# hwwang55/GraphGAN

Measured on AMD Instinct MI355X. Metric: sampled_edges_per_sec, higher is better.
Workload: dtype f32

## Files before the change

### graphgan_amd/csrc/gg_api.hip

```cpp
#include <stdarg.h>
#include <stdlib.h>
#include <string.h>
#include <sys/stat.h>
#include <unistd.h>

#include <algorithm>
#include <atomic>
#include <thread>

#include "gg_internal.h"

namespace gg {

thread_local std::string g_last_error;

int fail(gg_ctx *ctx, int code, const char *fmt, ...) {
    char buf[1024];
    va_list ap;
    va_start(ap, fmt);
    vsnprintf(buf, sizeof(buf), fmt, ap);
    va_end(ap);
    g_last_error = buf;
    if (ctx) ctx->err = buf;
    return code;
}

static void free_trees(gg_ctx *ctx) {
    discard_begun_walk(ctx);
    void *ps[] = {ctx->t_root, ctx->t_order, ctx->t_cstart, ctx->t_base, ctx->t_q3, ctx->t_q3off, ctx->t_edge};
    for (void *p : ps)
        if (p) (void)hipFree(p);
    ctx->t_root = ctx->t_order = ctx->t_cstart = ctx->t_edge = nullptr;
    ctx->t_edge_valid = false;
    ctx->t_base = ctx->t_q3off = nullptr;
    ctx->t_q3 = nullptr;
    ctx->t_cap_nodes = ctx->t_cap_roots = ctx->t_cap_q3 = 0;
    ctx->n_tree_roots = 0;
    ctx->tree_nodes = ctx->tree_entries = 0;
    ctx->tree_max_depth = ctx->tree_max_list = 0;
    ctx->t_lazy = false;
    ctx->lz_min_level = 0x7fffffff;
    ctx->h_troot.clear();
    ctx->h_tbase.clear();
    ctx->h_q3off.clear();
}

int alloc_trees(gg_ctx *ctx, const int32_t *roots, int32_t n_roots, const int64_t *node_counts, const int64_t *root_children, int64_t extra_nodes) {
    discard_begun_walk(ctx);
    (void)hipDeviceSynchronize();
    ctx->dc_valid = false;
    ctx->t_lazy = false;
    ctx->lz_min_level = 0x7fffffff;
    ctx->t_edge_valid = false;
    const int n = ctx->n_node;
    if (!node_counts && ctx->h_comp_size.empty()) component_sizes(n, ctx->h_rowptr.data(), ctx->h_col.data(), ctx->h_comp_size);
    ctx->h_tbase.assign(n_roots + 1, 0);
    ctx->h_q3off.assign(n_roots + 1, 0);
    for (int r = 0; r < n_roots; ++r) {
        ctx->h_tbase[r + 1] = ctx->h_tbase[r] + (node_counts ? node_counts[r] : ctx->h_comp_size[roots[r]]);
        const int64_t deg = root_children ? root_children[r] : ctx->h_rowptr[roots[r] + 1] - ctx->h_rowptr[roots[r]];
        ctx->h_q3off[r + 1] = ctx->h_q3off[r] + (deg + 31) / 32;
    }
    const int64_t seg_nodes = ctx->h_tbase[n_roots], q3w = ctx->h_q3off[n_roots];
    const int64_t nodes = seg_nodes + extra_nodes;
    const int nr = std::max(n_roots, 1);
    ctx->arena_next = seg_nodes;
    ctx->arena_end = nodes;
    auto regrow = [&](void **p, size_t bytes) -> hipError_t {
        if (*p) (void)hipFree(*p);
        *p = nullptr;
        return hipMalloc(p, bytes);
    };
    if (nodes > ctx->t_cap_nodes || (ctx->t_cap_nodes > (64 << 20) && nodes < ctx->t_cap_nodes / 4) || nr > ctx->t_cap_roots) {
        const int64_t cn = std::max<int64_t>(nodes, 1), cr = std::max<int64_t>(nr, ctx->t_cap_roots);
        GG_HIP(ctx, regrow((void **)&ctx->t_order, sizeof(int32_t) * (size_t)cn));
        GG_HIP(ctx, regrow((void **)&ctx->t_edge, sizeof(int32_t) * (size_t)cn));
        GG_HIP(ctx, regrow((void **)&ctx->t_cstart, sizeof(int32_t) * (size_t)(cn + 2 * cr + 2)));
        GG_HIP(ctx, regrow((void **)&ctx->t_root, sizeof(int32_t) * (size_t)cr));
        GG_HIP(ctx, regrow((void **)&ctx->t_base, sizeof(int64_t) * (size_t)(cr + 1)));
        GG_HIP(ctx, regrow((void **)&ctx->t_q3off, sizeof(int64_t) * (size_t)(cr + 1)));
        ctx->t_cap_nodes = cn;
        ctx->t_cap_roots = cr;
    }
    if (q3w > ctx->t_cap_q3 || !ctx->t_q3) {
        const int64_t cq = std::max<int64_t>(q3w + q3w / 2, 1);
        GG_HIP(ctx, regrow((void **)&ctx->t_q3, sizeof(uint32_t) * (size_t)cq));
        ctx->t_cap_q3 = cq;
    }
    ctx->tree_max_depth = ctx->tree_max_list = 0;
    GG_HIP(ctx, hipMemcpyAsync(ctx->t_root, roots, sizeof(int32_t) * n_roots, hipMemcpyHostToDevice, ctx->stream));
    GG_HIP(ctx, hipMemcpyAsync(ctx->t_base, ctx->h_tbase.data(), sizeof(int64_t) * (n_roots + 1), hipMemcpyHostToDevice, ctx->stream));
    GG_HIP(ctx, hipMemcpyAsync(ctx->t_q3off, ctx->h_q3off.data(), sizeof(int64_t) * (n_roots + 1), hipMemcpyHostToDevice, ctx->stream));
    GG_HIP(ctx, hipMemsetAsync(ctx->t_q3, 0, sizeof(uint32_t) * (size_t)std::max<int64_t>(q3w, 1), ctx->stream));
    GG_HIP(ctx, hipStreamSynchronize(ctx->stream));
    ctx->n_tree_roots = n_roots;
    ctx->tree_nodes = seg_nodes;
    ctx->tree_entries = 2 * seg_nodes - n_roots;
    ctx->h_troot.assign(roots, roots + n_roots);
    return GG_OK;
}

void generator_changed(gg_ctx *ctx) {
    ctx->dc_valid = false;
    ctx->gs_es_valid = false;
    ctx->es_tick += 256;
    ctx->es_valid_from = ctx->es_tick;
}

static int upload_table(gg_ctx *ctx, float *dst, const float *src) {
    const int n = ctx->n_node, d = ctx->n_emb, ld = ctx->ld;
    if (ld == d) {
        GG_HIP(ctx, hipMemcpy(dst, src, sizeof(float) * (size_t)n * d, hipMemcpyHostToDevice));
    } else {
        GG_HIP(ctx, hipMemset(dst, 0, sizeof(float) * (size_t)n * ld));
        GG_HIP(ctx, hipMemcpy2D(dst, sizeof(float) * ld, src, sizeof(float) * d, sizeof(float) * d, n, hipMemcpyHostToDevice));
    }
    return GG_OK;
}

__global__ __launch_bounds__(256) void table_finite_kernel(const float *E, const float *b, int64_t nE, int64_t nb, unsigned long long *bad) {
    bool any = false;
    const int64_t stride = (int64_t)gridDim.x * blockDim.x;
    for (int64_t i = (int64_t)blockIdx.x * blockDim.x + threadIdx.x; i < nE; i += stride) any |= !__builtin_isfinite(E[i]);
    for (int64_t i = (int64_t)blockIdx.x * blockDim.x + threadIdx.x; i < nb; i += stride) any |= !__builtin_isfinite(b[i]);
    if (any) *bad = 1ull;
}

int rescan_table_finite(gg_ctx *ctx, int which) {
    const Model &M = ctx->model[which];
    unsigned long long *w = ctx->table_bad.as<unsigned long long>() + which;
    GG_HIP(ctx, hipMemsetAsync(w, 0, sizeof(unsigned long long), ctx->stream));
    const int64_t nE = (int64_t)ctx->n_node * ctx->ld;
    hipLaunchKernelGGL(table_finite_kernel, dim3((unsigned)std::min<int64_t>(2048, (nE + 255) / 256)), dim3(256), 0, ctx->stream, M.E, M.b, nE, (int64_t)ctx->n_node, w);
    GG_HIP(ctx, hipGetLastError());
    if (which == 0) ctx->gen_dirty = true;
    return GG_OK;
}

}

using namespace gg;

static int launch_and_join(gg_ctx *ctx, int32_t n_slots, int64_t total, int32_t for_d, uint64_t seed, uint32_t stream, int32_t stride, bool join = true) {
    const bool side = ctx->walk_stream != ctx->stream;
    int rc = launch_walk_sample(ctx, n_slots, total, for_d, seed, stream, stride);
    if (rc != GG_OK) {
        if (side) (void)hipStreamSynchronize(ctx->walk_stream);
        return rc;
    }
    if (side) {
        GG_HIP(ctx, hipEventRecord(ctx->ev_walk_done, ctx->walk_stream));
        if (join) GG_HIP(ctx, hipStreamWaitEvent(ctx->stream, ctx->ev_walk_done, 0));
        if (!for_d) {
            rc = enqueue_path_slots(ctx);
            if (rc != GG_OK) return rc;
        }
    }
    return GG_OK;
}

void gg::discard_begun_walk(gg_ctx *ctx) {
    if (!ctx->g_begun) return;
    (void)hipStreamSynchronize(ctx->stream2);
    ctx->g_begun = false;
    ctx->dc_request = 0;
    ctx->walk_stream = ctx->stream;
    ctx->w_nslots = 0;
    ctx->w_total = 0;
    generator_changed(ctx);
}

int gg::walk_launch_async(gg_ctx *ctx, const int32_t *slots, const int32_t *n_walks, int32_t uniform_walks, int32_t n_slots,
                          int32_t for_d, uint64_t seed, uint32_t stream, int32_t stride, bool side_stream, bool defer_join) {
    discard_begun_walk(ctx);
    GG_CHECK(ctx, ctx->n_tree_roots > 0 || n_slots == 0, GG_EINVAL, "walk: no trees loaded (gg_build_trees / gg_set_trees)");
    GG_CHECK(ctx, n_slots >= 0 && (slots || n_slots == 0), GG_EINVAL, "walk: bad slots");
    GG_CHECK(ctx, stride >= 2, GG_ECAPACITY, "walk: stride %d < 2", stride);
    std::vector<int64_t> &ptr = ctx->h_ptr_new;
    ptr.assign(n_slots + 1, 0);
    for (int i = 0; i < n_slots; ++i) {
        GG_CHECK(ctx, slots[i] >= 0 && slots[i] < ctx->n_tree_roots, GG_EINVAL, "walk: slot %d out of range", slots[i]);
        int64_t nw;
        if (n_walks) nw = n_walks[i];
        else if (uniform_walks >= 0) nw = uniform_walks;
        else {
            GG_CHECK(ctx, !ctx->h_rowptr.empty(), GG_EINVAL, "walk: graph CSR needed for D-mode degrees");
            const int r = ctx->h_troot[slots[i]];
            nw = ctx->h_rowptr[r + 1] - ctx->h_rowptr[r];
        }
        GG_CHECK(ctx, nw >= 0, GG_EINVAL, "walk: negative n_walks");
        ptr[i + 1] = ptr[i] + nw;
    }
    const int64_t total = ptr[n_slots];
    GG_HIP(ctx, hipSetDevice(ctx->device));
    const int mode = for_d ? 1 : 0;
    ctx->w_mode = mode;
    GG_HIP(ctx, ctx->w_slots_m[mode].reserve(sizeof(int32_t) * (n_slots + 1)));
    GG_HIP(ctx, ctx->w_ptr_m[mode].reserve(sizeof(int64_t) * (n_slots + 1)));
    GG_HIP(ctx, ctx->w_status.reserve(sizeof(int32_t) * (n_slots + 1)));
    GG_HIP(ctx, ctx->w_abort.reserve(sizeof(int32_t) * (n_slots + 1)));
    GG_HIP(ctx, ctx->w_samples.reserve(sizeof(int32_t) * (total + 1)));
    GG_HIP(ctx, ctx->w_len.reserve(sizeof(int32_t) * (total + 1)));
    GG_HIP(ctx, ctx->w_first.reserve(sizeof(int32_t) * (total + 1)));
    GG_HIP(ctx, ctx->w_paths.reserve(sizeof(int32_t) * ((size_t)total * stride + 1)));
    ctx->walk_stream = side_stream ? ctx->stream2 : ctx->stream;
    if (side_stream && ctx->gen_dirty) {
        GG_HIP(ctx, hipEventRecord(ctx->ev_main_mark, ctx->stream));
        GG_HIP(ctx, hipStreamWaitEvent(ctx->stream2, ctx->ev_main_mark, 0));
        ctx->gen_dirty = false;
    } else if (side_stream && ctx->gen_pass_recorded) {
        GG_HIP(ctx, hipStreamWaitEvent(ctx->stream2, ctx->ev_gen_pass, 0));
    }
    std::vector<int32_t> &hs = ctx->h_slots_m[mode];
    if (hs.size() != (size_t)n_slots || (n_slots && memcmp(hs.data(), slots, sizeof(int32_t) * n_slots) != 0)) {
        hs.assign(slots, slots + n_slots);
        if (n_slots) GG_HIP(ctx, hipMemcpyAsync(ctx->w_slots_m[mode].p, hs.data(), sizeof(int32_t) * n_slots, hipMemcpyHostToDevice, ctx->walk_stream));
    }
    if (ctx->h_ptr_m[mode] != ptr) {
        ctx->h_ptr_m[mode].swap(ptr);
        GG_HIP(ctx, hipMemcpyAsync(ctx->w_ptr_m[mode].p, ctx->h_ptr_m[mode].data(), sizeof(int64_t) * (n_slots + 1), hipMemcpyHostToDevice, ctx->walk_stream));
    }
    ctx->w_total = total;
    ctx->w_stride = stride;
    ctx->w_nslots = n_slots;
    ctx->w_uniform = (!n_walks && uniform_walks >= 0) ? uniform_walks : -1;
    ctx->w_args = {for_d, seed, stream};
    ctx->g_paths_valid = false;
    if (ctx->g_slots_ready) {
        GG_HIP(ctx, hipStreamWaitEvent(ctx->stream, ctx->ev_slots_done, 0));
        ctx->g_slots_ready = false;
        ctx->g_slots_unused++;
    }
    if (n_slots == 0) {
        ctx->walk_stream = ctx->stream;
        return GG_OK;
    }
    return launch_and_join(ctx, n_slots, total, for_d, seed, stream, stride, !defer_join);
}

int gg::walk_finalize(gg_ctx *ctx, bool *retried) {
    if (retried) *retried = false;
    if (ctx->w_nslots == 0) {
        GG_HIP(ctx, hipStreamSynchronize(ctx->stream));
        return GG_OK;
    }
    const int64_t total = ctx->w_total;
    unsigned long long *c = ctx->h_pin;
    constexpr int CW = gg_ctx::CTR_WORDS;
    GG_HIP(ctx, hipMemcpyAsync(c, ctx->dev_ctr, sizeof(unsigned long long) * 2 * CW, hipMemcpyDeviceToHost, ctx->stream));
    GG_HIP(ctx, hipStreamSynchronize(ctx->stream));
    harvest_timings(ctx);
    for (int attempt = 0; c[3] == 2ull || (c[2] != 0ull && ctx->t_lazy); ++attempt) {
        GG_CHECK(ctx, attempt < 16, GG_EHIP, "walk: the launch was voided %d times in a row", attempt);
        if (c[2] != 0ull && ctx->t_lazy) {
            int rebuilt = 0;
            int rc = lazy_fallback_rebuild(ctx, &rebuilt);
            if (rc == GG_ECAPACITY) rc = lazy_rebuild_whole(ctx);
            if (rc != GG_OK) return rc;
            if (ctx->tree_max_depth + 3 > ctx->w_stride) {
                ctx->w_stride = ctx->tree_max_depth + 3;
                GG_HIP(ctx, ctx->w_paths.reserve(sizeof(int32_t) * ((size_t)total * ctx->w_stride + 1)));
            }
        } else {
            ctx->walk_force_sized = true;
        }
        ctx->ctr.walk_reruns += 1;
        generator_changed(ctx);
        int rc = launch_and_join(ctx, ctx->w_nslots, total, ctx->w_args.for_d, ctx->w_args.seed, ctx->w_args.stream, ctx->w_stride);
        ctx->walk_force_sized = false;
        if (rc != GG_OK) return rc;
        GG_HIP(ctx, hipMemcpyAsync(c, ctx->dev_ctr, sizeof(unsigned long long) * 2 * CW, hipMemcpyDeviceToHost, ctx->stream));
        GG_HIP(ctx, hipStreamSynchronize(ctx->stream));
        if (retried) *retried = true;
    }
    const int n_half = ctx->w_split ? 2 : 1;
    if (n_half == 2)
        for (int i = 8; i < CW; ++i) c[i] += c[CW + i];
    {
        int64_t *prof = ctx->alive_prof[ctx->w_args.for_d ? 1 : 0];
        const int run = ctx->w_levels_run;
        for (int i = 0; i < 64; ++i) prof[i] = i < run ? (int64_t)c[8 + i] : -1;
        if (run > 0 && run < 64 && ctx->w_fin_follows) prof[run] = (int64_t)c[7];
        if (ctx->w_net && c[7] > 2048ull && ctx->lv_levels_learned < ctx->tree_max_depth + 2) ctx->lv_levels_learned += 1;
    }
    unsigned long long hops = c[0], reads = c[1], rows = c[5];
    unsigned long long gathers = 0, nodes = 0;
    for (int i = 0; i < 64; ++i) { hops += c[264 + i]; reads += c[328 + i]; rows += c[200 + i]; gathers += c[520 + i]; nodes += c[584 + i]; }
    ctx->ctr.es_gathers += (int64_t)gathers;
    ctx->ctr.es_nodes += (int64_t)nodes;
    ctx->ctr.hops += (int64_t)hops;
    ctx->ctr.nbr_reads += (int64_t)reads;
    ctx->ctr.rows_scored += (int64_t)rows;
    ctx->ctr.walks += total;
    if (total && ctx->walk_timed) {
        float ms = 0.f;
        GG_HIP(ctx, hipEventElapsedTime(&ms, ctx->ev0, ctx->ev1));
        ctx->ctr.last_kernel_ms = ms;
        ctx->ctr.walk_kernel_ms += ms;
        ctx->ctr.walk_launches += 1;
        for (int i = 0; i < ctx->lv_ev_used; ++i) {
            float lms = 0.f;
            for (int k = 0; k < n_half; ++k) {
                float e = 0.f;
                GG_HIP(ctx, hipEventElapsedTime(&e, ctx->lv_ev[4 * i + 2 * k], ctx->lv_ev[4 * i + 2 * k + 1]));
                lms += e;
            }
            ctx->ctr.score_kernel_ms += lms;
            ctx->ctr.score_launches += n_half;
            ctx->ctr.score_chunks += (int64_t)(c[136 + i] >> 32);
            if (getenv("GG_WALK_DEBUG"))
                fprintf(stderr, "[walk] for_d=%d level %d alive %llu score chunks %llu prefix chunks %llu big %llu small %llu rows %llu score %.1f us\n", ctx->w_args.for_d, i,
                        c[8 + i], c[136 + i] >> 32, c[136 + i] & 0xffffffffull, c[72 + i] & 0xffffffffull, c[72 + i] >> 32, c[456 + i], lms * 1e3);
        }
        if (ctx->lv_ev_used) {
            ctx->ctr.score_rows += (int64_t)(rows - c[5]);
            unsigned long long dists = 0;
            for (int i = 0; i < 64; ++i) dists += c[392 + i];
            ctx->ctr.score_dists += (int64_t)dists;
            ctx->ctr.score_gathers += (int64_t)gathers;
            ctx->ctr.score_nodes += (int64_t)nodes;
        }
    }
    if (c[3] || c[6]) generator_changed(ctx);
    if (c[3]) return fail(ctx, GG_ECAPACITY, "walk: a path needed more than stride=%d entries", ctx->w_stride);
    if (c[6]) return fail(ctx, GG_EINVAL, "walk: non-finite generator scores (a softmax had total weight 0, or the generator's tables hold a non-finite value)");
    return GG_OK;
}

int gg::walk_resident(gg_ctx *ctx, const int32_t *slots, const int32_t *n_walks, int32_t uniform_walks, int32_t n_slots,
                      int32_t for_d, uint64_t seed, uint32_t stream, int32_t stride) {
    int rc = walk_launch_async(ctx, slots, n_walks, uniform_walks, n_slots, for_d, seed, stream, stride);
    if (rc != GG_OK) return rc;
    return walk_finalize(ctx, nullptr);
}

extern "C" {

int gg_abi_version(void) { return GG_ABI_VERSION; }

const char *gg_last_error(const gg_ctx *ctx) { return ctx ? ctx->err.c_str() : g_last_error.c_str(); }

int gg_create(int32_t n_node, int32_t n_emb, const float *emb_gen, const float *emb_dis, const gg_config *cfg,
              gg_ctx **out) {
    if (!out) return fail(nullptr, GG_EINVAL, "gg_create: out is NULL");
    *out = nullptr;
    if (n_node <= 0 || n_emb <= 0 || n_emb > 512 || !emb_gen || !emb_dis || !cfg)
        return fail(nullptr, GG_EINVAL, "gg_create: bad argument (n_node=%d n_emb=%d)", n_node, n_emb);
    int ndev = 0;
    hipError_t e = hipGetDeviceCount(&ndev);
    if (e != hipSuccess || ndev <= 0)
        return fail(nullptr, GG_EHIP, "gg_create: no HIP device (%s); this engine has no CPU fallback",
                    e == hipSuccess ? "count = 0" : hipGetErrorString(e));
    if (cfg->device < 0 || cfg->device >= ndev) return fail(nullptr, GG_EINVAL, "gg_create: device %d of %d", cfg->device, ndev);
    hipDeviceProp_t prop;
    GG_HIP(nullptr, hipGetDeviceProperties(&prop, cfg->device));
    if (strncmp(prop.gcnArchName, "gfx950", 6) != 0)
        return fail(nullptr, GG_EHIP, "gg_create: device %d is %s; kernels are built for gfx950 only", cfg->device, prop.gcnArchName);
    GG_HIP(nullptr, hipSetDevice(cfg->device));

    gg_ctx *ctx = new gg_ctx();
    ctx->n_node = n_node;
    ctx->n_emb = n_emb;
    ctx->ld = (n_emb + 3) / 4 * 4;
    ctx->cfg = *cfg;
    ctx->device = cfg->device;
    ctx->n_cus = prop.multiProcessorCount > 0 ? prop.multiProcessorCount : 256;
    if (const char *lv = getenv("GG_WALK_LEVELS")) ctx->walk_levels = atoi(lv);
    if (const char *pe = getenv("GG_PROFILE_EVERY")) ctx->profile_every = std::max(0, atoi(pe));
    if (const char *fw = getenv("GG_COMM_FAKE_WORLD")) ctx->fake_world = atoi(fw);
    if (const char *ow = getenv("GG_COMM_OWNER")) ctx->owner_exchange = atoi(ow);
    if (const char *bf = getenv("GG_COMM_BF16")) ctx->comm_bf16 = atoi(bf) != 0;
    if (const char *om = getenv("GG_COMM_OWNER_MIN")) ctx->owner_min_bound = atoll(om);
    if (const char *dt = getenv("GG_DETERMINISTIC")) ctx->deterministic = atoi(dt) != 0;
    if (const char *nc = getenv("GG_NO_DIST_CACHE")) ctx->dc_enabled = atoi(nc) == 0;
    if (const char *ft = getenv("GG_FIN_THRESHOLD")) ctx->fin_threshold = std::max(0, atoi(ft));
    if (const char *st = getenv("GG_STAGE_T")) ctx->sg_threshold = std::max(0, atoi(st));
    if (const char *ws = getenv("GG_WALK_SPLIT")) ctx->split_enabled = atoi(ws) != 0;
    if (const char *em = getenv("GG_ES_MODE")) ctx->es_mode = std::min(2, std::max(0, atoi(em)));
    if (const char *er = getenv("GG_ES_RATIO")) ctx->es_ratio_num = std::max(1, atoi(er));
    if (const char *eh = getenv("GG_ES_HUB")) ctx->es_hub = std::max(0, atoi(eh));
    if (const char *wm = getenv("GG_WALK_SPLIT_MIN")) ctx->split_min_walks = std::max(512, atoi(wm));
    for (auto &m : ctx->alive_prof) for (auto &v : m) v = -1;
    if (const char *dr = getenv("GG_COMM_DENSE_RATIO")) ctx->dense_exchange_ratio = (float)atof(dr);
#define GG_TRY(call)                        \
    do {                                    \
        int rc__ = (call);                  \
        if (rc__ != GG_OK) {                \
            g_last_error = ctx->err;        \
            gg_destroy(ctx);                \
            return rc__;                    \
        }                                   \
    } while (0)
    auto body = [&]() -> int {
        GG_HIP(ctx, hipStreamCreateWithFlags(&ctx->stream, hipStreamNonBlocking));
        {
            int lo = 0, hi = 0;
            const char *wp = getenv("GG_WALK_PRIORITY");
            if (wp && atoi(wp) != 0 && hipDeviceGetStreamPriorityRange(&lo, &hi) == hipSuccess && hi != lo)
                GG_HIP(ctx, hipStreamCreateWithPriority(&ctx->stream2, hipStreamNonBlocking, atoi(wp) > 0 ? hi : lo));
            else
                GG_HIP(ctx, hipStreamCreateWithFlags(&ctx->stream2, hipStreamNonBlocking));
        }
        GG_HIP(ctx, hipStreamCreateWithFlags(&ctx->stream3, hipStreamNonBlocking));
        GG_HIP(ctx, hipEventCreateWithFlags(&ctx->ev_fork, hipEventDisableTiming));
        GG_HIP(ctx, hipEventCreateWithFlags(&ctx->ev_join, hipEventDisableTiming));
        GG_HIP(ctx, hipEventCreateWithFlags(&ctx->ev_score[0], hipEventDisableTiming));
        GG_HIP(ctx, hipEventCreateWithFlags(&ctx->ev_score[1], hipEventDisableTiming));
        ctx->walk_stream = ctx->stream;
        GG_HIP(ctx, hipEventCreate(&ctx->ev0));
        GG_HIP(ctx, hipEventCreate(&ctx->ev1));
        GG_HIP(ctx, hipEventCreateWithFlags(&ctx->ev_walk_done, hipEventDisableTiming));
        GG_HIP(ctx, hipEventCreateWithFlags(&ctx->ev_gen_pass, hipEventDisableTiming));
        GG_HIP(ctx, hipEventCreateWithFlags(&ctx->ev_main_mark, hipEventDisableTiming));
        GG_HIP(ctx, hipHostMalloc((void **)&ctx->h_pin, sizeof(unsigned long long) * gg_ctx::PIN_WORDS, hipHostMallocDefault));
        memset(ctx->h_pin, 0, sizeof(unsigned long long) * gg_ctx::PIN_WORDS);
        const size_t tb = sizeof(float) * (size_t)n_node * ctx->ld, vb = sizeof(float) * (size_t)n_node;
        for (int m = 0; m < 2; ++m) {
            Model &M = ctx->model[m];
            GG_HIP(ctx, hipMalloc((void **)&M.E, tb));
            GG_HIP(ctx, hipMalloc((void **)&M.b, vb));
            GG_HIP(ctx, hipMemset(M.b, 0, vb));
            if (cfg->optimizer != GG_OPT_SGD) {
                GG_HIP(ctx, hipMalloc((void **)&M.mE, tb));
                GG_HIP(ctx, hipMalloc((void **)&M.vE, tb));
                GG_HIP(ctx, hipMalloc((void **)&M.mb, vb));
                GG_HIP(ctx, hipMalloc((void **)&M.vb, vb));
                GG_HIP(ctx, hipMemset(M.mE, 0, tb));
                GG_HIP(ctx, hipMemset(M.vE, 0, tb));
                GG_HIP(ctx, hipMemset(M.mb, 0, vb));
                GG_HIP(ctx, hipMemset(M.vb, 0, vb));
            }
            M.b1p = cfg->adam_beta1;
            M.b2p = cfg->adam_beta2;
            M.lr = m == 0 ? cfg->lr_gen : cfg->lr_dis;
            M.lambda = m == 0 ? cfg->lambda_gen : cfg->lambda_dis;
            int rc = upload_table(ctx, M.E, m == 0 ? emb_gen : emb_dis);
            if (rc != GG_OK) return rc;
        }
        GG_HIP(ctx, hipMalloc((void **)&ctx->gradE, tb));
        GG_HIP(ctx, hipMalloc((void **)&ctx->gradb, vb));
        GG_HIP(ctx, hipMemset(ctx->gradE, 0, tb));
        ctx->grad_elems_padded = (size_t)n_node * ctx->ld;
        GG_HIP(ctx, hipMemset(ctx->gradb, 0, vb));
        GG_HIP(ctx, hipMalloc((void **)&ctx->touched, sizeof(int32_t) * n_node));
        GG_HIP(ctx, hipMalloc((void **)&ctx->touched_list, sizeof(int32_t) * n_node));
        GG_HIP(ctx, hipMalloc((void **)&ctx->touched_cnt, sizeof(int32_t) * 4));
        GG_HIP(ctx, hipMemset(ctx->touched, 0, sizeof(int32_t) * n_node));
        GG_HIP(ctx, hipMemset(ctx->touched_cnt, 0, sizeof(int32_t) * 4));
        GG_HIP(ctx, hipMalloc((void **)&ctx->dev_ctr, sizeof(unsigned long long) * gg_ctx::PIN_WORDS));
        GG_HIP(ctx, hipMemset(ctx->dev_ctr, 0, sizeof(unsigned long long) * gg_ctx::PIN_WORDS));
        GG_HIP(ctx, ctx->table_bad.reserve(sizeof(unsigned long long) * 2));
        for (int m = 0; m < 2; ++m) {
            int rc = rescan_table_finite(ctx, m);
            if (rc != GG_OK) return rc;
        }
        GG_HIP(ctx, hipDeviceSynchronize());
        return GG_OK;
    };
    GG_TRY(body());
#undef GG_TRY
    *out = ctx;
    return GG_OK;
}

int gg_destroy(gg_ctx *ctx) {
    if (!ctx) return GG_OK;
    (void)hipSetDevice(ctx->device);
    if (ctx->stream) (void)hipStreamSynchronize(ctx->stream);
    if (ctx->stream2) (void)hipStreamSynchronize(ctx->stream2);
    comm_destroy(ctx);
    for (int m = 0; m < 2; ++m) {
        Model &M = ctx->model[m];
        float *ps[] = {M.E, M.b, M.mE, M.vE, M.mb, M.vb};
        for (float *p : ps)
            if (p) (void)hipFree(p);
    }
    void *ps[] = {ctx->gradE, ctx->gradb, ctx->touched, ctx->touched_list, ctx->touched_cnt, ctx->g_rowptr, ctx->g_col, ctx->dev_ctr,
                  ctx->es, ctx->es_stamp, ctx->g_rev};
    for (void *p : ps)
        if (p) (void)hipFree(p);
    free_trees(ctx);
    DevBuf *bufs[] = {&ctx->w_slots_m[0], &ctx->w_slots_m[1], &ctx->w_ptr_m[0], &ctx->w_ptr_m[1], &ctx->w_samples, &ctx->w_paths, &ctx->w_len, &ctx->w_status,
                      &ctx->w_first, &ctx->w_abort, &ctx->w_scratch, &ctx->d_center, &ctx->d_neighbor, &ctx->d_label, &ctx->d_cnt,
                      &ctx->d_ptr, &ctx->g_node1, &ctx->g_node2, &ctx->g_reward, &ctx->g_cnt, &ctx->g_ptr, &ctx->scan_tmp,
                      &ctx->step_u, &ctx->step_v, &ctx->step_x, &ctx->sg_cnt, &ctx->sg_off, &ctx->sg_slot, &ctx->sg_list, &ctx->sg_rows, &ctx->sg_bias, &ctx->sg_tot, &ctx->sg_key, &ctx->touched_ptr, &ctx->x_cnt, &ctx->x_send_ids, &ctx->x_send_rows,
                      &ctx->x_recv_ids, &ctx->x_recv_rows, &ctx->x_nglob, &ctx->x_own, &ctx->st_item, &ctx->st_item2, &ctx->st_cur, &ctx->st_prev, &ctx->st_len,
                      &ctx->st_alive, &ctx->st_rank, &ctx->bfs_key, &ctx->bfs_bm, &ctx->bfs_misc, &ctx->bfs_sparse, &ctx->bfs_rowptr32, &ctx->lv_pfx, &ctx->dc_keys, &ctx->dc_vals, &ctx->dc_words, &ctx->lv_beg, &ctx->lv_k, &ctx->lv_chunks, &ctx->lv_coff, &ctx->lv_scores, &ctx->lv_chunk_owner, &ctx->lv_prefix, &ctx->lv_big, &ctx->lv_fe, &ctx->fin_list, &ctx->table_bad, &ctx->sgp_cnt, &ctx->sgp_off, &ctx->sgp_slot, &ctx->sgp_list, &ctx->sgp_tot, &ctx->sgp_key, &ctx->sgp_scan, &ctx->sgp_hub, &ctx->sg_hub, &ctx->hub_acc,
                      &ctx->q3_store, &ctx->q3s_off, &ctx->ep_center, &ctx->ep_neighbor, &ctx->ep_label, &ctx->ep_node1, &ctx->ep_node2, &ctx->ep_reward, &ctx->topk_adj,
                      &ctx->gs_es, &ctx->gs_cpre, &ctx->pt_starts, &ctx->pt_paths, &ctx->pt_len, &ctx->pt_cnt, &ctx->pt_ptr, &ctx->pt_noise, &ctx->pt_sample};
    for (DevBuf *b : bufs) b->release();
    for (hipEvent_t e : ctx->lv_ev)
        if (e) (void)hipEventDestroy(e);
    for (auto &tr : ctx->tm_ev)
        for (hipEvent_t e : tr)
            if (e) (void)hipEventDestroy(e);
    for (hipEvent_t e : ctx->pt_ev)
        if (e) (void)hipEventDestroy(e);
    if (ctx->h_pin) (void)hipHostFree(ctx->h_pin);
    for (hipEvent_t e : {ctx->ev_walk_done, ctx->ev_slots_done, ctx->ev_gen_pass, ctx->ev_main_mark, ctx->ev_fork, ctx->ev_join, ctx->ev_score[0], ctx->ev_score[1]})
        if (e) (void)hipEventDestroy(e);
    if (ctx->stream3) {
        (void)hipStreamSynchronize(ctx->stream3);
        (void)hipStreamDestroy(ctx->stream3);
    }
    if (ctx->stream2) {
        (void)hipStreamSynchronize(ctx->stream2);
        (void)hipStreamDestroy(ctx->stream2);
    }
    if (ctx->ev0) (void)hipEventDestroy(ctx->ev0);
    if (ctx->ev1) (void)hipEventDestroy(ctx->ev1);
    if (ctx->stream) (void)hipStreamDestroy(ctx->stream);
    delete ctx;
    return GG_OK;
}

int gg_set_graph_csr(gg_ctx *ctx, const int64_t *rowptr, const int32_t *col) {
    if (!ctx) return fail(nullptr, GG_EINVAL, "ctx is NULL");
    GG_CHECK(ctx, rowptr && rowptr[0] == 0, GG_EINVAL, "gg_set_graph_csr: rowptr[0] must be 0");
    discard_begun_walk(ctx);
    const int n = ctx->n_node;
    const int64_t nnz = rowptr[n];
    GG_CHECK(ctx, nnz >= 0 && (col || nnz == 0), GG_EINVAL, "gg_set_graph_csr: col is NULL");
    for (int v = 0; v < n; ++v) GG_CHECK(ctx, rowptr[v + 1] >= rowptr[v], GG_EINVAL, "gg_set_graph_csr: rowptr not monotone at %d", v);
    for (int64_t e = 0; e < nnz; ++e) GG_CHECK(ctx, col[e] >= 0 && col[e] < n, GG_EINVAL, "gg_set_graph_csr: col[%lld]=%d out of range", (long long)e, col[e]);
    GG_HIP(ctx, hipSetDevice(ctx->device));
    (void)hipDeviceSynchronize();
    for (void *p : {(void *)ctx->g_rowptr, (void *)ctx->g_col, (void *)ctx->es, (void *)ctx->es_stamp, (void *)ctx->g_rev})
        if (p) (void)hipFree(p);
    ctx->g_rowptr = nullptr;
    ctx->g_col = nullptr;
    ctx->es = nullptr;
    ctx->es_stamp = nullptr;
    ctx->g_rev = nullptr;
    ctx->t_edge_valid = false;
    ctx->q3_store_ready = false;
    ctx->bfs_rowptr32_valid = false;
    ctx->topk_adj.release();
    ctx->topk_adj_valid = false;
    ctx->gs_es_valid = ctx->gs_cpre_valid = false;
    ctx->pt_noise_set = false;
    GG_HIP(ctx, hipMalloc((void **)&ctx->g_rowptr, sizeof(int64_t) * (n + 1)));
    GG_HIP(ctx, hipMalloc((void **)&ctx->g_col, sizeof(int32_t) * (std::max<int64_t>(nnz, 1) + 4)));
    GG_HIP(ctx, hipMemcpy(ctx->g_rowptr, rowptr, sizeof(int64_t) * (n + 1), hipMemcpyHostToDevice));
    if (nnz) GG_HIP(ctx, hipMemcpy(ctx->g_col, col, sizeof(int32_t) * nnz, hipMemcpyHostToDevice));
    ctx->g_nnz = nnz;
    ctx->g_max_deg = 0;
    for (int v = 0; v < n; ++v) ctx->g_max_deg = (int32_t)std::min<int64_t>(std::max<int64_t>(ctx->g_max_deg, rowptr[v + 1] - rowptr[v]), 0x7fffffff);
    ctx->g_multi = true;
    ctx->h_rowptr.assign(rowptr, rowptr + n + 1);
    ctx->h_col.assign(col, col + nnz);
    ctx->h_comp_size.clear();
    uint64_t h = 1469598103934665603ull;
    for (int v = 0; v <= n; ++v) h = (h ^ (uint64_t)rowptr[v]) * 1099511628211ull;
    for (int64_t e = 0; e + 1 < nnz; e += 2) h = (h ^ ((uint64_t)(uint32_t)col[e] | ((uint64_t)(uint32_t)col[e + 1] << 32))) * 1099511628211ull;
    if (nnz & 1) h = (h ^ (uint64_t)(uint32_t)col[nnz - 1]) * 1099511628211ull;
    ctx->g_hash = h;
    if (nnz > 0 && nnz < (1ll << 31)) {
        hipError_t e = hipMalloc((void **)&ctx->es, sizeof(float) * (size_t)nnz);
        if (e == hipSuccess) e = hipMalloc((void **)&ctx->es_stamp, sizeof(long long) * (size_t)n);
        if (e == hipSuccess) e = hipMalloc((void **)&ctx->g_rev, sizeof(int32_t) * (size_t)nnz);
        if (e == hipSuccess) e = hipMemset(ctx->es_stamp, 0, sizeof(long long) * (size_t)n);
        generator_changed(ctx);
        int rc = e == hipSuccess ? compute_reverse_edges(ctx) : GG_ENOMEM;
        if (rc != GG_OK) {
            (void)hipGetLastError();
            for (void *p : {(void *)ctx->es, (void *)ctx->es_stamp, (void *)ctx->g_rev})
                if (p) (void)hipFree(p);
            ctx->es = nullptr;
            ctx->es_stamp = nullptr;
            ctx->g_rev = nullptr;
            if (getenv("GG_WALK_DEBUG")) fprintf(stderr, "[graph] edge-score cache not allocated (%s): walks score privately\n", e == hipSuccess ? ctx->err.c_str() : hipGetErrorString(e));
        }
    }
    return GG_OK;
}

int gg_build_trees(gg_ctx *ctx, const int32_t *roots, int32_t n_roots, int32_t n_threads) {
    if (!ctx) return fail(nullptr, GG_EINVAL, "ctx is NULL");
    GG_CHECK(ctx, !ctx->h_rowptr.empty(), GG_EINVAL, "gg_build_trees: call gg_set_graph_csr first");
    GG_CHECK(ctx, n_roots >= 0 && (roots || n_roots == 0), GG_EINVAL, "gg_build_trees: bad roots");
    const int n = ctx->n_node;
    for (int r = 0; r < n_roots; ++r) GG_CHECK(ctx, roots[r] >= 0 && roots[r] < n, GG_EINVAL, "gg_build_trees: root %d out of range", roots[r]);
    GG_HIP(ctx, hipSetDevice(ctx->device));
    if (n_threads <= 0) n_threads = (int)std::max(1u, std::thread::hardware_concurrency());
    int rc = alloc_trees(ctx, roots, n_roots, nullptr, nullptr);
    if (rc != GG_OK) return rc;
    const int64_t budget = 256ll << 20;
    const std::vector<int64_t> &base = ctx->h_tbase;
    int32_t md = 0, ml = 0;
    std::vector<int32_t> order_h, cstart_h;
    for (int r0 = 0; r0 < n_roots;) {
        int r1 = r0 + 1;
        while (r1 < n_roots && base[r1 + 1] - base[r0] <= budget) ++r1;
        order_h.resize((size_t)(base[r1] - base[r0]));
        cstart_h.resize((size_t)(base[r1] - base[r0]) + (r1 - r0));
        const int nt = std::max(1, std::min(n_threads, r1 - r0));
        std::atomic<int> next(r0);
        std::vector<int32_t> tmd(nt, 0), tml(nt, 0);
        auto work = [&](int tid) {
            std::vector<uint32_t> stamp(n, 0u);
            uint32_t epoch = 0;
            for (;;) {
                const int r = next.fetch_add(1);
                if (r >= r1) break;
                int32_t depth = 0, mc = 0;
                (void)host_bfs_order(ctx->h_rowptr.data(), ctx->h_col.data(), roots[r], order_h.data() + (base[r] - base[r0]),
                                     cstart_h.data() + (base[r] - base[r0]) + (r - r0), stamp, epoch, &depth, &mc);
                tmd[tid] = std::max(tmd[tid], depth);
                tml[tid] = std::max(tml[tid], mc + 1);
            }
        };
        std::vector<std::thread> th;
        for (int t = 1; t < nt; ++t) th.emplace_back(work, t);
        work(0);
        for (auto &t : th) t.join();
        for (int t = 0; t < nt; ++t) { md = std::max(md, tmd[t]); ml = std::max(ml, tml[t]); }
        if (!order_h.empty()) GG_HIP(ctx, hipMemcpy(ctx->t_order + base[r0], order_h.data(), sizeof(int32_t) * order_h.size(), hipMemcpyHostToDevice));
        GG_HIP(ctx, hipMemcpy(ctx->t_cstart + base[r0] + r0, cstart_h.data(), sizeof(int32_t) * cstart_h.size(), hipMemcpyHostToDevice));
        r0 = r1;
    }
    ctx->tree_max_depth = md;
    ctx->tree_max_list = ml;
    return derive_tree_edges(ctx);
}

int gg_set_trees(gg_ctx *ctx, const int32_t *roots, int32_t n_roots, const int32_t *off, const int32_t *nbr,
                 const int64_t *nbr_base, int32_t max_depth) {
    if (!ctx) return fail(nullptr, GG_EINVAL, "ctx is NULL");
    GG_CHECK(ctx, n_roots >= 0 && roots && off && nbr_base && (nbr || nbr_base[n_roots] == 0), GG_EINVAL, "gg_set_trees: bad argument");
    const int n = ctx->n_node;
    GG_HIP(ctx, hipSetDevice(ctx->device));
    std::vector<int64_t> counts(n_roots), kids(n_roots);
    for (int r = 0; r < n_roots; ++r) {
        GG_CHECK(ctx, roots[r] >= 0 && roots[r] < n, GG_EINVAL, "gg_set_trees: root out of range");
        const int32_t *o = off + (size_t)r * (n + 1);
        GG_CHECK(ctx, o[0] == 0 && o[n] == nbr_base[r + 1] - nbr_base[r] && o[n] >= 1 && (o[n] & 1), GG_EINVAL,
                 "gg_set_trees: offsets of slot %d inconsistent (a tree over C nodes has 2C - 1 entries)", r);
        for (int v = 0; v < n; ++v) GG_CHECK(ctx, o[v + 1] >= o[v], GG_EINVAL, "gg_set_trees: offsets not monotone");
        counts[r] = (o[n] + 1) / 2;
        kids[r] = o[roots[r] + 1] - o[roots[r]];
    }
    int rc = alloc_trees(ctx, roots, n_roots, counts.data(), kids.data());
    if (rc != GG_OK) return rc;
    const std::vector<int64_t> &base = ctx->h_tbase;
    std::vector<int32_t> order_h((size_t)base[n_roots]), cstart_h((size_t)base[n_roots] + n_roots);
    std::vector<uint32_t> q3_h((size_t)std::max<int64_t>(ctx->h_q3off[n_roots], 1), 0u);
    int32_t md = 0, ml = 0;
    for (int r = 0; r < n_roots; ++r) {
        const int64_t C_expect = base[r + 1] - base[r];
        GG_CHECK(ctx, nbr_base[r + 1] - nbr_base[r] == 2 * C_expect - 1, GG_EINVAL,
                 "gg_set_trees: slot %d has %lld entries, the component of root %d needs %lld", r, (long long)(nbr_base[r + 1] - nbr_base[r]),
                 roots[r], (long long)(2 * C_expect - 1));
// ... 231 lines not shown
        GG_HIP(ctx, hipMemcpy(len.data(), ctx->w_len.p, sizeof(int32_t) * total, hipMemcpyDeviceToHost));
        for (int64_t w = 0; w < total; ++w)
            GG_CHECK(ctx, len[w] <= stride, GG_ECAPACITY, "walk: a path needed %d entries, stride is %d (gg_tree_info reports the depth of the trees as rebuilt)", len[w], stride);
        if (paths) GG_HIP(ctx, hipMemcpy2D(paths, sizeof(int32_t) * (size_t)stride, ctx->w_paths.p, sizeof(int32_t) * (size_t)ctx->w_stride, sizeof(int32_t) * (size_t)stride, (size_t)total, hipMemcpyDeviceToHost));
    }
    if (root_status && n_slots) GG_HIP(ctx, hipMemcpy(root_status, ctx->w_status.p, sizeof(int32_t) * n_slots, hipMemcpyDeviceToHost));
    return GG_OK;
}

int gg_debug_words(gg_ctx *ctx, int32_t first, int32_t n, uint64_t *out) {
    if (!ctx || !out || first < 0 || n < 0 || first + n > gg_ctx::PIN_WORDS) return fail(ctx, GG_EINVAL, "gg_debug_words: bad argument");
    GG_HIP(ctx, hipSetDevice(ctx->device));
    hipStream_t s;
    GG_HIP(ctx, hipStreamCreateWithFlags(&s, hipStreamNonBlocking));
    hipError_t e = hipMemcpyAsync(out, ctx->dev_ctr + first, sizeof(uint64_t) * (size_t)n, hipMemcpyDeviceToHost, s);
    if (e == hipSuccess) e = hipStreamSynchronize(s);
    (void)hipStreamDestroy(s);
    GG_HIP(ctx, e);
    return GG_OK;
}

int gg_set_tree_mode(gg_ctx *ctx, int32_t mode, int64_t node_cap) {
    if (!ctx) return fail(nullptr, GG_EINVAL, "ctx is NULL");
    GG_CHECK(ctx, mode >= -1 && mode <= 1 && node_cap >= 0, GG_EINVAL, "gg_set_tree_mode: mode must be -1 (auto), 0 (whole trees) or 1 (lazy), node_cap >= 0");
    ctx->tree_mode = mode;
    ctx->lz_cap = node_cap;
    return GG_OK;
}

int gg_lazy_stats(gg_ctx *ctx, int64_t *out8) {
    if (!ctx || !out8) return fail(ctx, GG_EINVAL, "gg_lazy_stats: NULL argument");
    GG_HIP(ctx, hipSetDevice(ctx->device));
    for (int i = 0; i < 24; ++i) out8[i] = 0;
    out8[0] = ctx->t_lazy ? 1 : 0;
    out8[1] = ctx->t_lazy ? ctx->lz_min_level : 0;
    out8[2] = ctx->lz_fallback_roots;
    out8[3] = ctx->lz_fallback_rounds;
    if (ctx->t_lazy && ctx->n_tree_roots > 0) {
        GG_HIP(ctx, hipStreamSynchronize(ctx->stream));
        const int R = ctx->n_tree_roots;
        std::vector<int4> info((size_t)R);
        std::vector<int32_t> cur((size_t)R);
        GG_HIP(ctx, hipMemcpy(info.data(), ctx->lz_info.p, sizeof(int4) * (size_t)R, hipMemcpyDeviceToHost));
        GG_HIP(ctx, hipMemcpy(cur.data(), ctx->lz_cursor.p, sizeof(int32_t) * (size_t)R, hipMemcpyDeviceToHost));
        for (int r = 0; r < R; ++r) {
            out8[4] += info[r].y;
            out8[5] += std::max(0, cur[r] - info[r].y);
            out8[6] += info[r].x < info[r].y ? 1 : 0;
            out8[7] = std::max<int64_t>(out8[7], info[r].z);
            if (info[r].x < info[r].y && info[r].z >= 0 && info[r].z < 8) out8[16 + info[r].z] += 1;
        }
        unsigned long long c[8];
        GG_HIP(ctx, hipMemcpy(c, ctx->dev_ctr + 1500, sizeof(c), hipMemcpyDeviceToHost));
        for (int i = 0; i < 8; ++i) out8[8 + i] = (int64_t)c[i];
    }
    return GG_OK;
}

int gg_get_lazy_trees(gg_ctx *ctx, int64_t *n_entries, int32_t *info4, int64_t *base, int32_t *order, int32_t *cstart, int32_t *edge, uint64_t *pair) {
    if (!ctx) return fail(nullptr, GG_EINVAL, "ctx is NULL");
    GG_CHECK(ctx, ctx->t_lazy, GG_EINVAL, "gg_get_lazy_trees: the resident trees are not lazy");
    GG_HIP(ctx, hipSetDevice(ctx->device));
    GG_HIP(ctx, hipDeviceSynchronize());
    const size_t R = (size_t)ctx->n_tree_roots, nodes = (size_t)ctx->arena_end;
    if (n_entries) *n_entries = (int64_t)nodes;
    if (info4) GG_HIP(ctx, hipMemcpy(info4, ctx->lz_info.p, sizeof(int4) * R, hipMemcpyDeviceToHost));
    if (base) GG_HIP(ctx, hipMemcpy(base, ctx->t_base, sizeof(int64_t) * R, hipMemcpyDeviceToHost));
    if (order) GG_HIP(ctx, hipMemcpy(order, ctx->t_order, sizeof(int32_t) * nodes, hipMemcpyDeviceToHost));
    if (cstart) GG_HIP(ctx, hipMemcpy(cstart, ctx->t_cstart, sizeof(int32_t) * (nodes + R), hipMemcpyDeviceToHost));
    if (edge) GG_HIP(ctx, hipMemcpy(edge, ctx->t_edge, sizeof(int32_t) * nodes, hipMemcpyDeviceToHost));
    if (pair) GG_HIP(ctx, hipMemcpy(pair, ctx->lz_pair.p, sizeof(uint64_t) * std::min(nodes, ctx->lz_pair.bytes / sizeof(uint64_t)), hipMemcpyDeviceToHost));
    return GG_OK;
}

int gg_walk_info(const gg_ctx *ctx, int64_t *total_walks, int32_t *stride, int32_t *n_slots) {
    if (!ctx) return fail(nullptr, GG_EINVAL, "ctx is NULL");
    if (total_walks) *total_walks = ctx->w_total;
    if (stride) *stride = ctx->w_stride;
    if (n_slots) *n_slots = ctx->w_nslots;
    return GG_OK;
}

int gg_get_walks(gg_ctx *ctx, int32_t *samples, int32_t *paths, int32_t *path_len, int32_t *root_status) {
    if (!ctx) return fail(nullptr, GG_EINVAL, "ctx is NULL");
    GG_HIP(ctx, hipSetDevice(ctx->device));
    const bool begun = ctx->g_begun;
    discard_begun_walk(ctx);
    GG_CHECK(ctx, !begun, GG_EINVAL, "gg_get_walks: the walks of the last completed launch were overwritten by gg_prepare_g_begin (fetch them before it, or after the gg_prepare_g that adopts it)");
    GG_HIP(ctx, hipStreamSynchronize(ctx->stream));
    const int64_t total = ctx->w_total;
    if (samples && total) GG_HIP(ctx, hipMemcpy(samples, ctx->w_samples.p, sizeof(int32_t) * total, hipMemcpyDeviceToHost));
    if (path_len && total) GG_HIP(ctx, hipMemcpy(path_len, ctx->w_len.p, sizeof(int32_t) * total, hipMemcpyDeviceToHost));
    if (paths && total) GG_HIP(ctx, hipMemcpy(paths, ctx->w_paths.p, sizeof(int32_t) * (size_t)total * ctx->w_stride, hipMemcpyDeviceToHost));
    if (root_status && ctx->w_nslots) GG_HIP(ctx, hipMemcpy(root_status, ctx->w_status.p, sizeof(int32_t) * ctx->w_nslots, hipMemcpyDeviceToHost));
    return GG_OK;
}

static int table_io(gg_ctx *ctx, int32_t which, float *out, const float *in, bool bias) {
    if (!ctx) return fail(nullptr, GG_EINVAL, "ctx is NULL");
    GG_CHECK(ctx, which == 0 || which == 1, GG_EINVAL, "which must be 0 (gen) or 1 (dis)");
    GG_CHECK(ctx, out || in, GG_EINVAL, "buffer is NULL");
    GG_HIP(ctx, hipSetDevice(ctx->device));
    GG_HIP(ctx, hipStreamSynchronize(ctx->stream));
    Model &M = ctx->model[which];
    const int n = ctx->n_node, d = ctx->n_emb, ld = ctx->ld;
    if (in && which == 0) { discard_begun_walk(ctx); generator_changed(ctx); }
    if (bias) {
        if (out) GG_HIP(ctx, hipMemcpy(out, M.b, sizeof(float) * n, hipMemcpyDeviceToHost));
        else GG_HIP(ctx, hipMemcpy(M.b, in, sizeof(float) * n, hipMemcpyHostToDevice));
    } else if (out) {
        GG_HIP(ctx, hipMemcpy2D(out, sizeof(float) * d, M.E, sizeof(float) * ld, sizeof(float) * d, n, hipMemcpyDeviceToHost));
    } else {
        int rc = upload_table(ctx, M.E, in);
        if (rc != GG_OK) return rc;
    }
    if (in) return rescan_table_finite(ctx, which);
    return GG_OK;
}

int gg_get_embeddings(gg_ctx *ctx, int32_t which, float *out) { return table_io(ctx, which, out, nullptr, false); }
int gg_get_bias(gg_ctx *ctx, int32_t which, float *out) { return table_io(ctx, which, out, nullptr, true); }
int gg_set_embeddings(gg_ctx *ctx, int32_t which, const float *emb) { return table_io(ctx, which, nullptr, emb, false); }
int gg_set_bias(gg_ctx *ctx, int32_t which, const float *bias) { return table_io(ctx, which, nullptr, bias, true); }

int gg_get_counters(gg_ctx *ctx, gg_counters *out) {
    if (!ctx || !out) return fail(ctx, GG_EINVAL, "gg_get_counters: NULL argument");
    if (!ctx->tm_pending.empty()) {
        GG_HIP(ctx, hipSetDevice(ctx->device));
        GG_HIP(ctx, hipStreamSynchronize(ctx->stream));
        harvest_timings(ctx);
    }
    *out = ctx->ctr;
    return GG_OK;
}

int gg_set_profiling_solo(gg_ctx *ctx, int32_t solo) {
    if (!ctx) return fail(nullptr, GG_EINVAL, "ctx is NULL");
    ctx->profile_solo = solo != 0;
    return GG_OK;
}

int gg_set_profiling(gg_ctx *ctx, int32_t every_n) {
    if (!ctx) return fail(nullptr, GG_EINVAL, "ctx is NULL");
    GG_CHECK(ctx, every_n >= 0, GG_EINVAL, "gg_set_profiling: every_n < 0");
    ctx->profile_every = every_n;
    ctx->walk_call_index = 0;
    return GG_OK;
}

int gg_synchronize(gg_ctx *ctx) {
    if (!ctx) return fail(nullptr, GG_EINVAL, "ctx is NULL");
    GG_HIP(ctx, hipSetDevice(ctx->device));
    GG_HIP(ctx, hipStreamSynchronize(ctx->stream));
    if (ctx->g_begun) GG_HIP(ctx, hipStreamSynchronize(ctx->stream2));
    harvest_timings(ctx);
    return check_exchange_flag(ctx);
}

}

int gg::check_exchange_flag(gg_ctx *ctx) {
    if (!ctx->comm && ctx->fake_world <= 1) return GG_OK;
    int32_t flag = 0;
    GG_HIP(ctx, hipMemcpy(&flag, ctx->touched_cnt + 2, sizeof(int32_t), hipMemcpyDeviceToHost));
    if (flag) return fail(ctx, GG_ECOMM, "replica exchange: a rank touched more rows than the pack capacity of its step");
    return GG_OK;
}

void gg::harvest_timings(gg_ctx *ctx) {
    size_t keep = 0;
    for (size_t i = 0; i < ctx->tm_pending.size(); ++i) {
        const gg_ctx::PendingTiming t = ctx->tm_pending[i];
        hipEvent_t *ev = ctx->tm_ev[t.slot];
        if (hipEventQuery(ev[2]) != hipSuccess) {
            ctx->tm_pending[keep++] = t;
            continue;
        }
        float a = 0.f, b = 0.f;
        (void)hipEventElapsedTime(&a, ev[0], ev[1]);
        (void)hipEventElapsedTime(&b, ev[1], ev[2]);
        const int64_t rows = t.has_rows ? (int64_t)ctx->h_pin[gg_ctx::H_ROWS + t.slot] : (int64_t)ctx->n_node;
        if (t.kind == 0) {
            ctx->ctr.reward_kernel_ms += a + b;
            ctx->ctr.reward_pairs_timed += t.units;
        } else if (t.kind == 1) {
            ctx->ctr.d_grad_ms += a; ctx->ctr.d_opt_ms += b;
            ctx->ctr.d_pairs_timed += t.units; ctx->ctr.d_rows_timed += rows; ctx->ctr.d_passes_timed += 1;
        } else {
            ctx->ctr.g_grad_ms += a; ctx->ctr.g_opt_ms += b;
            ctx->ctr.g_pairs_timed += t.units; ctx->ctr.g_rows_timed += rows; ctx->ctr.g_passes_timed += 1;
        }
    }
    ctx->tm_pending.resize(keep);
}

int gg::timing_slot(gg_ctx *ctx) {
    for (int s = 0; s < 8; ++s) {
        bool busy = false;
        for (const auto &t : ctx->tm_pending) busy |= t.slot == s;
        if (busy) continue;
        for (int k = 0; k < 3; ++k)
            if (!ctx->tm_ev[s][k] && hipEventCreate(&ctx->tm_ev[s][k]) != hipSuccess) return -1;
        return s;
    }
    return -1;
}

namespace {
struct StateHeader {
    char magic[4];
    int32_t version, n_node, n_emb, ld, optimizer;
};

int io_dev(gg_ctx *ctx, FILE *f, float *dev, size_t count, bool save, std::vector<float> &tmp) {
    tmp.resize(count);
    if (save) {
        GG_HIP(ctx, hipMemcpy(tmp.data(), dev, sizeof(float) * count, hipMemcpyDeviceToHost));
        if (fwrite(tmp.data(), sizeof(float), count, f) != count) return gg::fail(ctx, GG_EIO, "state: short write");
    } else {
        if (fread(tmp.data(), sizeof(float), count, f) != count) return gg::fail(ctx, GG_EIO, "state: short read");
        GG_HIP(ctx, hipMemcpy(dev, tmp.data(), sizeof(float) * count, hipMemcpyHostToDevice));
    }
    return GG_OK;
}

int state_io(gg_ctx *ctx, const char *path, bool save) {
    if (!ctx) return gg::fail(nullptr, GG_EINVAL, "ctx is NULL");
    GG_CHECK(ctx, path, GG_EINVAL, "state: path is NULL");
    GG_HIP(ctx, hipSetDevice(ctx->device));
    GG_HIP(ctx, hipStreamSynchronize(ctx->stream));
    if (!save) discard_begun_walk(ctx);
    const bool slots = ctx->cfg.optimizer != GG_OPT_SGD;
    const size_t ne = (size_t)ctx->n_node * ctx->ld, nb = (size_t)ctx->n_node;
    struct Scalars { int64_t t; float b1p, b2p; };
    const size_t per_model = sizeof(Scalars) + sizeof(float) * (ne + nb) * (slots ? 3 : 1);
    const size_t expect = sizeof(StateHeader) + 2 * per_model;
    const std::string tmp_path = std::string(path) + ".tmp";
    FILE *f = fopen(save ? tmp_path.c_str() : path, save ? "wb" : "rb");
    if (!f) return gg::fail(ctx, GG_EIO, "state: cannot open %s", save ? tmp_path.c_str() : path);
    StateHeader h{{'G', 'G', 'S', 'T'}, 1, ctx->n_node, ctx->n_emb, ctx->ld, ctx->cfg.optimizer};
    int rc = GG_OK;
    if (save) {
        if (fwrite(&h, sizeof(h), 1, f) != 1) rc = gg::fail(ctx, GG_EIO, "state: short write");
    } else {
        StateHeader g;
        if (fread(&g, sizeof(g), 1, f) != 1 || memcmp(g.magic, "GGST", 4) != 0 || g.version != 1)
            rc = gg::fail(ctx, GG_EIO, "state: %s is not a GGST v1 file", path);
        else if (g.n_node != h.n_node || g.n_emb != h.n_emb || g.ld != h.ld || (g.optimizer == GG_OPT_SGD) != (h.optimizer == GG_OPT_SGD))
            rc = gg::fail(ctx, GG_EINVAL, "state: shape/optimizer mismatch (file %dx%d opt %d)", g.n_node, g.n_emb, g.optimizer);
        if (rc == GG_OK) {
            struct stat st;
            if (fstat(fileno(f), &st) != 0 || (size_t)st.st_size != expect)
                rc = gg::fail(ctx, GG_EIO, "state: %s is truncated or has trailing bytes (%lld bytes, expected %zu); nothing was loaded", path,
                              (long long)st.st_size, expect);
        }
    }
    std::vector<float> tmp;
    Scalars loaded[2] = {};
    for (int m = 0; m < 2 && rc == GG_OK; ++m) {
        gg::Model &M = ctx->model[m];
        Scalars sc{M.t, M.b1p, M.b2p};
        if (save) {
            if (fwrite(&sc, sizeof(sc), 1, f) != 1) rc = gg::fail(ctx, GG_EIO, "state: short write");
        } else {
            if (fread(&sc, sizeof(sc), 1, f) != 1) rc = gg::fail(ctx, GG_EIO, "state: short read");
            else loaded[m] = sc;
        }
        if (rc == GG_OK) rc = io_dev(ctx, f, M.E, ne, save, tmp);
        if (rc == GG_OK) rc = io_dev(ctx, f, M.b, nb, save, tmp);
        if (slots) {
            if (rc == GG_OK) rc = io_dev(ctx, f, M.mE, ne, save, tmp);
            if (rc == GG_OK) rc = io_dev(ctx, f, M.vE, ne, save, tmp);
            if (rc == GG_OK) rc = io_dev(ctx, f, M.mb, nb, save, tmp);
            if (rc == GG_OK) rc = io_dev(ctx, f, M.vb, nb, save, tmp);
        }
    }
    if (save) {
        if (rc == GG_OK && (fflush(f) != 0 || fsync(fileno(f)) != 0)) rc = gg::fail(ctx, GG_EIO, "state: cannot flush %s", tmp_path.c_str());
        fclose(f);
        if (rc == GG_OK && rename(tmp_path.c_str(), path) != 0) rc = gg::fail(ctx, GG_EIO, "state: cannot rename %s to %s", tmp_path.c_str(), path);
        if (rc != GG_OK) (void)remove(tmp_path.c_str());
        return rc;
    }
    fclose(f);
    generator_changed(ctx);
    for (int m = 0; m < 2; ++m) {
        const int rs = gg::rescan_table_finite(ctx, m);
        if (rc == GG_OK) rc = rs;
    }
    if (rc == GG_OK)
        for (int m = 0; m < 2; ++m) { ctx->model[m].t = loaded[m].t; ctx->model[m].b1p = loaded[m].b1p; ctx->model[m].b2p = loaded[m].b2p; }
    return rc;
}
}

extern "C" int gg_save_state(gg_ctx *ctx, const char *path) { return state_io(ctx, path, true); }
extern "C" int gg_load_state(gg_ctx *ctx, const char *path) { return state_io(ctx, path, false); }
```

### graphgan_amd/csrc/gg_internal.h

```cpp
#pragma once
#include <hip/hip_runtime.h>
#include <stdint.h>
#include <stdio.h>
#include <string>
#include <vector>

#include "../../include/graphgan_hip.h"

namespace gg {

struct DevBuf {
    void *p = nullptr;
    size_t bytes = 0;
    hipError_t reserve(size_t need) {
        if (need <= bytes) return hipSuccess;
        if (p) {
            (void)hipDeviceSynchronize();
            (void)hipFree(p);
        }
        p = nullptr;
        bytes = 0;
        size_t want = need + need / 4 + 256;
        hipError_t e = hipMalloc(&p, want);
        if (e == hipSuccess) bytes = want;
        return e;
    }
    void release() {
        if (p) (void)hipFree(p);
        p = nullptr;
        bytes = 0;
    }
    template <class T> T *as() const { return (T *)p; }
};

struct Model {
    float *E = nullptr, *b = nullptr;
    float *mE = nullptr, *vE = nullptr;
    float *mb = nullptr, *vb = nullptr;
    float b1p = 0.9f, b2p = 0.999f;
    int64_t t = 0;
    float lr = 1e-3f, lambda = 1e-5f;
};

}

struct gg_ctx {
    int32_t n_node = 0, n_emb = 0, ld = 0;
    gg_config cfg{};
    int device = 0;
    hipStream_t stream = nullptr;
    hipEvent_t ev0 = nullptr, ev1 = nullptr;
    hipStream_t stream2 = nullptr;
    hipStream_t walk_stream = nullptr;
    hipEvent_t ev_walk_done = nullptr;
    hipEvent_t ev_gen_pass = nullptr;
    hipEvent_t ev_main_mark = nullptr;
    bool gen_pass_recorded = false;
    bool gen_dirty = false;
    hipEvent_t lv_ev[256] = {};
    hipStream_t stream3 = nullptr;
    hipEvent_t ev_fork = nullptr, ev_join = nullptr, ev_score[2] = {nullptr, nullptr};
    bool split_enabled = false;
    int64_t split_min_walks = 32768;
    bool w_split = false;
    gg::DevBuf fin_list;
    gg::DevBuf table_bad;
    int lv_ev_used = 0;
    gg::Model model[2];

    float *gradE = nullptr, *gradb = nullptr;
    int32_t *touched = nullptr;
    int32_t *touched_list = nullptr;
    int32_t *touched_cnt = nullptr;

    int64_t *g_rowptr = nullptr;
    int32_t *g_col = nullptr;
    int64_t g_nnz = 0;
    uint64_t g_hash = 0;
    std::vector<int64_t> h_rowptr;
    std::vector<int32_t> h_col;
    float *es = nullptr;
    long long *es_stamp = nullptr;
    int32_t *g_rev = nullptr;
    long long es_tick = 256;
    long long es_valid_from = 256;
    int32_t es_mode = 1;
    int32_t es_ratio_num = 2;
    int32_t es_hub = 0;

    int32_t n_tree_roots = 0, tree_max_depth = 0, tree_max_list = 0;
    int64_t tree_nodes = 0;
    int64_t t_cap_nodes = 0, t_cap_roots = 0, t_cap_q3 = 0;
    int64_t tree_entries = 0;
    int32_t *t_root = nullptr;
    int32_t *t_order = nullptr;
    int32_t *t_cstart = nullptr;
    int32_t *t_edge = nullptr;
    bool t_edge_valid = false;
    int64_t *t_base = nullptr;
    uint32_t *t_q3 = nullptr;
    int64_t *t_q3off = nullptr;
    std::vector<int32_t> h_troot;
    std::vector<int64_t> h_tbase, h_q3off;
    std::vector<int32_t> h_comp_size;

    int32_t tree_mode = -1;
    int64_t lz_cap = 0;
    bool t_lazy = false;
    bool lz_force_whole = false;
    int32_t lz_min_level = 0x7fffffff;
    uint32_t lz_stamp = 0;
    gg::DevBuf lz_info, lz_pair, lz_rank, lz_bm, lz_cursor, lz_flag, lz_limit, lz_expect, lz_list, lz_scratch, lz_fb_scratch;
    int64_t arena_next = 0, arena_end = 0;
    int64_t lz_fallback_roots = 0, lz_fallback_rounds = 0, lz_resolved = 0;
    bool g_multi = true;
    int32_t g_max_deg = 0;

    gg::DevBuf w_slots_m[2], w_ptr_m[2];
    std::vector<int32_t> h_slots_m[2];
    std::vector<int64_t> h_ptr_m[2], h_ptr_new;
    int w_mode = 0;
    int64_t alive_prof[2][64];
    int64_t fin_threshold = 0;
    int w_levels_run = 0;
    bool w_fin_follows = false;
    bool w_net = false;
    const gg::DevBuf &w_slots_buf() const { return w_slots_m[w_mode]; }
    const gg::DevBuf &w_ptr_buf() const { return w_ptr_m[w_mode]; }
    gg::DevBuf w_samples, w_paths, w_len, w_status, w_first, w_abort, w_scratch;
    gg::DevBuf st_cur, st_prev, st_len, st_alive, st_rank, st_item, st_item2, lv_beg, lv_k, lv_chunks, lv_coff, lv_scores, lv_chunk_owner, lv_prefix, lv_big, lv_fe;
    gg::DevBuf lv_pfx, dc_keys, dc_vals, dc_words;
    size_t dc_size = 0;
    int32_t dc_request = 0;
    bool dc_valid = false;
    bool dc_enabled = true;
    int64_t lv_cap_total = 0;
    int32_t lv_levels_learned = 0;
    int64_t lv_cap_chunks = 0;
    bool walk_force_sized = false;
    bool walk_used_speculation = false;
    int32_t walk_levels = 64;
    int64_t w_total = 0;
    int32_t w_stride = 0, w_nslots = 0;
    int32_t w_uniform = -1;
    struct { int32_t for_d; uint64_t seed; uint32_t stream; } w_args{};

    static constexpr int CTR_WORDS = 720;
    static constexpr int PIN_WORDS = 2048;
    static constexpr int H_TOTAL = 1960;
    static constexpr int H_ROWS = 1940;
    unsigned long long *h_pin = nullptr;
    int32_t profile_every = 1;
    int64_t walk_call_index = 0;
    bool walk_timed = false;
    bool profile_solo = true;
    struct PendingTiming { int kind; int64_t units; int slot; bool has_rows; };
    hipEvent_t tm_ev[8][3] = {};
    std::vector<PendingTiming> tm_pending;
    int64_t pass_call_index[2] = {0, 0};
    int tm_cur = -1;

    gg::DevBuf d_center, d_neighbor, d_label, d_cnt, d_ptr;
    int64_t d_rows = 0;
    gg::DevBuf g_node1, g_node2, g_reward, g_cnt, g_ptr;
    int64_t g_pairs = 0;
    bool g_paths_valid = false;
    bool g_begun = false;
    struct { int32_t n_slots = 0, n_sample = 0; uint64_t seed = 0; uint32_t stream = 0; } g_begun_args;
    gg::DevBuf touched_ptr;
    gg::DevBuf bfs_key, bfs_bm, bfs_misc, bfs_sparse, bfs_rowptr32;
    bool bfs_rowptr32_valid = false;
    gg::DevBuf q3_store, q3s_off;
    int64_t q3_words = 0;
    bool q3_store_ready = false;
    gg::DevBuf ep_center, ep_neighbor, ep_label, ep_node1, ep_node2, ep_reward;
    int64_t ep_rows = 0, ep_pairs = 0;
    std::vector<int32_t> ep_slots;
    bool in_epoch_add = false;
    int n_cus = 256;
    gg::DevBuf scan_tmp, step_u, step_v, step_x;
    gg::DevBuf sg_cnt, sg_off, sg_slot, sg_list, sg_rows, sg_bias, sg_tot, sg_key;
    bool g_pairs_filled = false;
    bool sg_cnt_dirty = false;
    gg::DevBuf sgp_cnt, sgp_off, sgp_slot, sgp_list, sgp_tot, sgp_key, sgp_scan, sgp_hub;
    gg::DevBuf sg_hub, hub_acc;
    int64_t hub_cap = 0;
    hipEvent_t ev_slots_done = nullptr;
    bool g_slots_ready = false;
    bool sgp_cnt_clean = false;
    int g_slots_unused = 0;
    int64_t g_slots_walks = 0;
    int32_t g_slots_stride = 0;
    int32_t *sg_cnt_active = nullptr;
    bool sg_active = false;
    int sg_threshold = 64;

    unsigned long long *dev_ctr = nullptr;
    gg_counters ctr{};

    void *comm = nullptr;
    bool comm_rsag = true;
    size_t grad_elems_padded = 0;
    int64_t d_rows_max = 0, g_pairs_max = 0;
    int64_t step_bound = 0;
    int64_t comm_steps_sparse = 0, comm_steps_dense = 0, comm_bytes_sent = 0;
    int32_t rank = 0, world = 1;
    bool deterministic = true;
    float dense_exchange_ratio = 1.5f;
    int32_t fake_world = 0;
    gg::DevBuf x_cnt, x_send_ids, x_send_rows, x_recv_ids, x_recv_rows;
    gg::DevBuf x_nglob;
    gg::DevBuf x_own;
    int32_t owner_exchange = 1;
    bool comm_bf16 = false;
    int64_t owner_min_bound = 4096;
    int64_t comm_steps_owner = 0;

    gg::DevBuf topk_adj;
    bool topk_adj_valid = false;

    gg::DevBuf gs_es, gs_cpre;
    int64_t gs_chunks = 0;
    bool gs_es_valid = false, gs_cpre_valid = false;

    gg::DevBuf pt_starts, pt_paths, pt_len, pt_cnt, pt_ptr, pt_noise, pt_sample;
    bool pt_noise_set = false;
    uint64_t pt_noise_total = 0;
    int32_t pt_sample_n = 0, pt_sample_stride = 1;
    hipEvent_t pt_ev[4] = {};
    bool ep_d_open = false;

    std::string err;
};

namespace gg {

extern thread_local std::string g_last_error;

int fail(gg_ctx *ctx, int code, const char *fmt, ...);

#define GG_HIP(ctx, call)                                                                      \
    do {                                                                                       \
        hipError_t e__ = (call);                                                               \
        if (e__ != hipSuccess)                                                                 \
            return gg::fail(ctx, GG_EHIP, "%s:%d %s -> %s", __FILE__, __LINE__, #call,         \
                            hipGetErrorString(e__));                                           \
    } while (0)

#define GG_CHECK(ctx, cond, code, ...)                        \
    do {                                                      \
        if (!(cond)) return gg::fail(ctx, code, __VA_ARGS__); \
    } while (0)

int device_exclusive_scan(gg_ctx *ctx, const int32_t *cnt, int64_t *ptr, int64_t n);
int ensure_g_pairs(gg_ctx *ctx);
int device_compact_flags(gg_ctx *ctx, const int32_t *flag, int64_t n, int32_t *list, int64_t *total_out);
int device_segment_rows(gg_ctx *ctx, const int32_t *cnt, int64_t n, int T, int32_t *off, int4 *list, int64_t *totals, hipStream_t stream = nullptr,
                        DevBuf *scratch = nullptr);

int alloc_trees(gg_ctx *ctx, const int32_t *roots, int32_t n_roots, const int64_t *node_counts, const int64_t *root_children, int64_t extra_nodes = 0);
bool lazy_build_wanted(const gg_ctx *ctx);
int lazy_rebuild_whole(gg_ctx *ctx);
int lazy_fallback_rebuild(gg_ctx *ctx, int *n_out);
void component_sizes(int n, const int64_t *rowptr, const int32_t *col, std::vector<int32_t> &comp_size);
int32_t host_bfs_order(const int64_t *rowptr, const int32_t *col, int32_t root, int32_t *order, int32_t *cstart,
                       std::vector<uint32_t> &stamp, uint32_t &epoch, int32_t *depth_out, int32_t *max_children_out);
void order_to_lists(int32_t n, int32_t C, const int32_t *order, const int32_t *cstart, const uint32_t *q3, int32_t *off, int32_t *nbr);
int32_t lists_to_order(int32_t n, int32_t root, const int32_t *off, const int32_t *nbr, int32_t *order, int32_t *cstart,
                       uint32_t *q3, int32_t q3_words, int32_t *depth_out, int32_t *max_children_out);

int walk_launch_async(gg_ctx *ctx, const int32_t *slots, const int32_t *n_walks, int32_t uniform_walks, int32_t n_slots,
                      int32_t for_d, uint64_t seed, uint32_t stream, int32_t stride, bool side_stream = false, bool defer_join = false);
void discard_begun_walk(gg_ctx *ctx);
int walk_finalize(gg_ctx *ctx, bool *retried);
int timing_slot(gg_ctx *ctx);
int check_exchange_flag(gg_ctx *ctx);
void harvest_timings(gg_ctx *ctx);
int derive_tree_edges(gg_ctx *ctx);
int compute_reverse_edges(gg_ctx *ctx);
int rescan_table_finite(gg_ctx *ctx, int which);
int enqueue_path_slots(gg_ctx *ctx);
void generator_changed(gg_ctx *ctx);
int walk_resident(gg_ctx *ctx, const int32_t *slots, const int32_t *n_walks, int32_t uniform_walks, int32_t n_slots,
                  int32_t for_d, uint64_t seed, uint32_t stream, int32_t stride);
int launch_walk_sample(gg_ctx *ctx, int32_t n_slots, int64_t total_walks, int for_d, uint64_t seed, uint32_t stream,
                       int32_t stride);
int run_step(gg_ctx *ctx, int which, const int32_t *d_u, const int32_t *d_v, const float *d_x, int32_t n);
int comm_allreduce_grads(gg_ctx *ctx);
int comm_allreduce_flags(gg_ctx *ctx);
int comm_allreduce_i64(gg_ctx *ctx, int64_t *buf, size_t count);
int comm_allreduce_max_i64(gg_ctx *ctx, int64_t *buf, size_t count);
size_t comm_dense_bytes(const gg_ctx *ctx);
int exchange_count_max(gg_ctx *ctx, int64_t local, int64_t *max_out);
int comm_allgather(gg_ctx *ctx, const void *send, void *recv, size_t count, int elem_bytes);
bool comm_has_p2p(const gg_ctx *ctx);
int comm_exchange_v(gg_ctx *ctx, const float *send, const int64_t *send_off, const int64_t *send_cnt, float *recv, const int64_t *recv_off,
                    const int64_t *recv_cnt);
void comm_destroy(gg_ctx *ctx);

static inline int cdiv(int64_t a, int64_t b) { return (int)((a + b - 1) / b); }

}
```

### graphgan_amd/csrc/prepare.hip

```cpp
#include <algorithm>

#include <cstring>

#include "gg_internal.h"

namespace gg {

constexpr int SCAN_THREADS = 256;
constexpr int SCAN_ITEMS = 8;
constexpr int SCAN_TILE = SCAN_THREADS * SCAN_ITEMS;

__device__ __forceinline__ int64_t block_excl_scan(int64_t v, int64_t *total, int64_t *sh ) {
    const int lane = threadIdx.x & 63, wv = threadIdx.x >> 6;
    int64_t inc = v;
#pragma unroll
    for (int off = 1; off < 64; off <<= 1) {
        const int64_t o = __shfl_up(inc, off, 64);
        if (lane >= off) inc += o;
    }
    if (lane == 63) sh[wv] = inc;
    __syncthreads();
    int64_t base = 0, tot = 0;
#pragma unroll
    for (int i = 0; i < SCAN_THREADS / 64; ++i) {
        if (i < wv) base += sh[i];
        tot += sh[i];
    }
    __syncthreads();
    *total = tot;
    return base + inc - v;
}

__global__ __launch_bounds__(SCAN_THREADS) void scan_tile_sums(const int32_t *cnt, int64_t n, int64_t *tile_sum) {
    __shared__ int64_t sh[SCAN_THREADS / 64];
    const int64_t base = (int64_t)blockIdx.x * SCAN_TILE + (int64_t)threadIdx.x * SCAN_ITEMS;
    int64_t s = 0;
#pragma unroll
    for (int i = 0; i < SCAN_ITEMS; ++i)
        if (base + i < n) s += cnt[base + i];
    int64_t tot;
    (void)block_excl_scan(s, &tot, sh);
    if (threadIdx.x == 0) tile_sum[blockIdx.x] = tot;
}

__global__ __launch_bounds__(SCAN_THREADS) void scan_tile_offsets(int64_t *tile_sum, int64_t n_tiles, int64_t *total_out) {
    __shared__ int64_t sh[SCAN_THREADS / 64];
    int64_t carry = 0;
    for (int64_t t0 = 0; t0 < n_tiles; t0 += SCAN_THREADS) {
        const int64_t i = t0 + threadIdx.x;
        const int64_t v = i < n_tiles ? tile_sum[i] : 0;
        int64_t tot;
        const int64_t ex = block_excl_scan(v, &tot, sh);
        if (i < n_tiles) tile_sum[i] = carry + ex;
        carry += tot;
    }
    if (threadIdx.x == 0) *total_out = carry;
}

__global__ __launch_bounds__(SCAN_THREADS) void scan_tile_offsets2(int64_t *tile_sum_a, int64_t *tile_sum_b, int64_t n_tiles, int64_t *total_a, int64_t *total_b) {
    __shared__ int64_t sh[SCAN_THREADS / 64];
    int64_t *const tile_sum = blockIdx.x == 0 ? tile_sum_a : tile_sum_b;
    int64_t carry = 0;
    for (int64_t t0 = 0; t0 < n_tiles; t0 += SCAN_THREADS) {
        const int64_t i = t0 + threadIdx.x;
        const int64_t v = i < n_tiles ? tile_sum[i] : 0;
        int64_t tot;
        const int64_t ex = block_excl_scan(v, &tot, sh);
        if (i < n_tiles) tile_sum[i] = carry + ex;
        carry += tot;
    }
    if (threadIdx.x == 0) *(blockIdx.x == 0 ? total_a : total_b) = carry;
}

__global__ __launch_bounds__(SCAN_THREADS) void scan_apply(const int32_t *cnt, int64_t n, const int64_t *tile_off, int64_t *ptr) {
    __shared__ int64_t sh[SCAN_THREADS / 64];
    const int64_t base = (int64_t)blockIdx.x * SCAN_TILE + (int64_t)threadIdx.x * SCAN_ITEMS;
    int64_t v[SCAN_ITEMS], s = 0;
#pragma unroll
    for (int i = 0; i < SCAN_ITEMS; ++i) {
        v[i] = base + i < n ? cnt[base + i] : 0;
        s += v[i];
    }
    int64_t tot;
    int64_t run = tile_off[blockIdx.x] + block_excl_scan(s, &tot, sh);
#pragma unroll
    for (int i = 0; i < SCAN_ITEMS; ++i) {
        if (base + i < n) ptr[base + i] = run;
        run += v[i];
    }
}

int device_exclusive_scan(gg_ctx *ctx, const int32_t *cnt, int64_t *ptr, int64_t n) {
    const int64_t tiles = (n + SCAN_TILE - 1) / SCAN_TILE;
    GG_HIP(ctx, ctx->scan_tmp.reserve(sizeof(int64_t) * (tiles + 2)));
    int64_t *ts = ctx->scan_tmp.as<int64_t>();
    if (n == 0) {
        GG_HIP(ctx, hipMemsetAsync(ptr, 0, sizeof(int64_t), ctx->stream));
        return GG_OK;
    }
    hipLaunchKernelGGL(scan_tile_sums, dim3((unsigned)tiles), dim3(SCAN_THREADS), 0, ctx->stream, cnt, n, ts);
    hipLaunchKernelGGL(scan_tile_offsets, dim3(1), dim3(SCAN_THREADS), 0, ctx->stream, ts, tiles, ptr + n);
    hipLaunchKernelGGL(scan_apply, dim3((unsigned)tiles), dim3(SCAN_THREADS), 0, ctx->stream, cnt, n, ts, ptr);
    GG_HIP(ctx, hipGetLastError());
    return GG_OK;
}

__global__ __launch_bounds__(SCAN_THREADS) void flag_tile_sums(const int32_t *flag, int64_t n, int64_t *tile_sum) {
    __shared__ int64_t sh[SCAN_THREADS / 64];
    const int64_t base = (int64_t)blockIdx.x * SCAN_TILE + (int64_t)threadIdx.x * SCAN_ITEMS;
    int64_t s = 0;
#pragma unroll
    for (int i = 0; i < SCAN_ITEMS; ++i)
        if (base + i < n) s += flag[base + i] > 0 ? 1 : 0;
    int64_t tot;
    (void)block_excl_scan(s, &tot, sh);
    if (threadIdx.x == 0) tile_sum[blockIdx.x] = tot;
}

__global__ __launch_bounds__(SCAN_THREADS) void flag_compact(const int32_t *flag, int64_t n, const int64_t *tile_off, int32_t *list) {
    __shared__ int64_t sh[SCAN_THREADS / 64];
    const int64_t base = (int64_t)blockIdx.x * SCAN_TILE + (int64_t)threadIdx.x * SCAN_ITEMS;
    bool v[SCAN_ITEMS];
    int64_t s = 0;
#pragma unroll
    for (int i = 0; i < SCAN_ITEMS; ++i) {
        v[i] = base + i < n && flag[base + i] > 0;
        s += v[i] ? 1 : 0;
    }
    int64_t tot;
    int64_t run = tile_off[blockIdx.x] + block_excl_scan(s, &tot, sh);
#pragma unroll
    for (int i = 0; i < SCAN_ITEMS; ++i)
        if (v[i]) list[run++] = (int32_t)(base + i);
}

int device_compact_flags(gg_ctx *ctx, const int32_t *flag, int64_t n, int32_t *list, int64_t *total_out) {
    const int64_t tiles = (n + SCAN_TILE - 1) / SCAN_TILE;
    GG_HIP(ctx, ctx->scan_tmp.reserve(sizeof(int64_t) * (tiles + 2)));
    int64_t *ts = ctx->scan_tmp.as<int64_t>();
    if (n == 0) {
        GG_HIP(ctx, hipMemsetAsync(total_out, 0, sizeof(int64_t), ctx->stream));
        return GG_OK;
    }
    hipLaunchKernelGGL(flag_tile_sums, dim3((unsigned)tiles), dim3(SCAN_THREADS), 0, ctx->stream, flag, n, ts);
    hipLaunchKernelGGL(scan_tile_offsets, dim3(1), dim3(SCAN_THREADS), 0, ctx->stream, ts, tiles, total_out);
    hipLaunchKernelGGL(flag_compact, dim3((unsigned)tiles), dim3(SCAN_THREADS), 0, ctx->stream, flag, n, ts, list);
    GG_HIP(ctx, hipGetLastError());
    return GG_OK;
}

__global__ __launch_bounds__(SCAN_THREADS) void seg_tile_sums(const int32_t *cnt, int64_t n, int T, int64_t *tile_rows, int64_t *tile_occ) {
    __shared__ int64_t sh[SCAN_THREADS / 64];
    const int64_t base = (int64_t)blockIdx.x * SCAN_TILE + (int64_t)threadIdx.x * SCAN_ITEMS;
    int64_t rows = 0, occ = 0;
#pragma unroll
    for (int i = 0; i < SCAN_ITEMS; ++i)
        if (base + i < n) {
            const int c = cnt[base + i];
            if (c > 0 && c <= T) { rows += 1; occ += c; }
        }
    int64_t tot;
    (void)block_excl_scan(rows, &tot, sh);
    if (threadIdx.x == 0) tile_rows[blockIdx.x] = tot;
    (void)block_excl_scan(occ, &tot, sh);
    if (threadIdx.x == 0) tile_occ[blockIdx.x] = tot;
}

__global__ __launch_bounds__(SCAN_THREADS) void seg_apply(const int32_t *cnt, int64_t n, int T, const int64_t *tile_rows, const int64_t *tile_occ,
                                                          int32_t *off, int4 *list) {
    __shared__ int64_t sh[SCAN_THREADS / 64];
    const int64_t base = (int64_t)blockIdx.x * SCAN_TILE + (int64_t)threadIdx.x * SCAN_ITEMS;
    int c[SCAN_ITEMS];
    int64_t rows = 0, occ = 0;
#pragma unroll
    for (int i = 0; i < SCAN_ITEMS; ++i) {
        const int v = base + i < n ? cnt[base + i] : 0;
        c[i] = (v > 0 && v <= T) ? v : 0;
        rows += c[i] ? 1 : 0;
        occ += c[i];
    }
    int64_t tot;
    int64_t rrun = tile_rows[blockIdx.x] + block_excl_scan(rows, &tot, sh);
    int64_t orun = tile_occ[blockIdx.x] + block_excl_scan(occ, &tot, sh);
#pragma unroll
    for (int i = 0; i < SCAN_ITEMS; ++i)
        if (c[i]) {
            list[rrun++] = make_int4((int32_t)(base + i), (int32_t)orun, c[i], 0);
            off[base + i] = (int32_t)orun;
            orun += c[i];
        }
}

int device_segment_rows(gg_ctx *ctx, const int32_t *cnt, int64_t n, int T, int32_t *off, int4 *list, int64_t *totals, hipStream_t stream, DevBuf *scratch) {
    const int64_t tiles = (n + SCAN_TILE - 1) / SCAN_TILE;
    if (!scratch) scratch = &ctx->scan_tmp;
    if (!stream) stream = ctx->stream;
    GG_HIP(ctx, scratch->reserve(sizeof(int64_t) * (2 * tiles + 4)));
    int64_t *tr = scratch->as<int64_t>(), *to = tr + tiles + 1;
    hipLaunchKernelGGL(seg_tile_sums, dim3((unsigned)tiles), dim3(SCAN_THREADS), 0, stream, cnt, n, T, tr, to);
    hipLaunchKernelGGL(scan_tile_offsets2, dim3(2), dim3(SCAN_THREADS), 0, stream, tr, to, tiles, totals, totals + 1);
    hipLaunchKernelGGL(seg_apply, dim3((unsigned)tiles), dim3(SCAN_THREADS), 0, stream, cnt, n, T, tr, to, off, list);
    GG_HIP(ctx, hipGetLastError());
    return GG_OK;
}

__global__ void pair_count_kernel(const int32_t *path_len, int64_t n_walks, int window, int32_t *cnt, const unsigned long long *flag) {
    const int64_t w = (int64_t)blockIdx.x * blockDim.x + threadIdx.x;
    if (w >= n_walks) return;
    if (*flag == 2ull) { cnt[w] = 0; return; }
    const int L = path_len[w] - 1;
    int c = 0;
    for (int i = 0; i < L; ++i) {
        const int lo = max(i - window, 0), hi = min(i + window + 1, L);
        c += hi - lo - 1;
    }
    cnt[w] = L > 0 ? c : 0;
}

__global__ void pair_fill_kernel(const int32_t *paths, const int32_t *path_len, int stride, int64_t n_walks, int window,
                                 const int64_t *ptr, int32_t *node1, int32_t *node2, const unsigned long long *flag) {
    const int64_t w = (int64_t)blockIdx.x * blockDim.x + threadIdx.x;
    if (w >= n_walks || *flag == 2ull) return;
    const int L = path_len[w] - 1;
    const int32_t *p = paths + w * (int64_t)stride;
    int64_t o = ptr[w];
    for (int i = 0; i < L; ++i) {
        const int lo = max(i - window, 0), hi = min(i + window + 1, L);
        const int c = p[i];
        for (int j = lo; j < hi; ++j) {
            if (j == i) continue;
            node1[o] = c;
            node2[o] = p[j];
            ++o;
        }
    }
}

__global__ __launch_bounds__(256) void pair_reward_kernel(const float *E, const float *bias, int ld, const int32_t *u,
                                                          const int32_t *v, int64_t n_host, const int64_t *n_dev, float *out) {
    const int64_t n = n_dev ? *n_dev : n_host;
    const int t = threadIdx.x & 15;
    const int64_t g0 = ((int64_t)blockIdx.x * blockDim.x + threadIdx.x) >> 4;
    const int64_t ng = ((int64_t)gridDim.x * blockDim.x) >> 4;
    const int nchunk = ld >> 2;
    for (int64_t p = g0; p < n; p += ng) {
        const int a = u[p], b = v[p];
        const float4 *ra = (const float4 *)(E + (int64_t)a * ld);
        const float4 *rb = (const float4 *)(E + (int64_t)b * ld);
        float acc = 0.f;
        for (int c = t; c < nchunk; c += 16) {
            const float4 x = ra[c], y = rb[c];
            acc = __builtin_fmaf(x.x, y.x, acc);
            acc = __builtin_fmaf(x.y, y.y, acc);
            acc = __builtin_fmaf(x.z, y.z, acc);
            acc = __builtin_fmaf(x.w, y.w, acc);
        }
        acc += __shfl_xor(acc, 8, 64);
        acc += __shfl_xor(acc, 4, 64);
        acc += __shfl_xor(acc, 2, 64);
        acc += __shfl_xor(acc, 1, 64);
        if (t == 0) {
            float s = acc + bias[b];
            s = fminf(fmaxf(s, -10.0f), 10.0f);
            out[p] = logf(1.0f + expf(s));
        }
    }
}

template <int NCH>
__global__ __launch_bounds__(256) void path_reward_kernel(const float *E, const float *bias, int ld, const int32_t *paths,
                                                          const int32_t *path_len, int stride, int64_t n_walks, int window,
                                                          const int64_t *ptr, float *out, const unsigned long long *flag) {
    const int t = threadIdx.x & 15;
    const int64_t w = ((int64_t)blockIdx.x * blockDim.x + threadIdx.x) >> 4;
    if (w >= n_walks || *flag == 2ull) return;
    const int L = path_len[w] - 1;
    if (L <= 1) return;
    const int32_t *p = paths + w * (int64_t)stride;
    const int nchunk = ld >> 2;
    const int64_t pi0 = ptr[w];
    float4 R[3][NCH];
    float bv[3];
    bool have[3];
    auto fetch = [&](int pos, float4 (&row)[NCH], float &b, bool &ok) {
        ok = pos >= 0 && pos < L;
        const int nd = ok ? p[pos] : 0;
        b = ok ? bias[nd] : 0.f;
        const float4 *r = (const float4 *)(E + (int64_t)nd * ld);
#pragma unroll
        for (int i = 0; i < NCH; ++i) {
            const int c = t + 16 * i;
            row[i] = (ok && c < nchunk) ? r[c] : make_float4(0.f, 0.f, 0.f, 0.f);
        }
    };
    fetch(0, R[0], bv[0], have[0]);
    fetch(1, R[1], bv[1], have[1]);
    fetch(2, R[2], bv[2], have[2]);
    auto n_pairs_of = [&](int i) { return min(i, window) + min(L - 1 - i, window); };
    int base = 0;
    for (int c = 0; c < L; ++c) {
        float4 Rn[NCH];
        float nb;
        bool nh;
        fetch(c + 3, Rn, nb, nh);
        const int back_c = min(c, window);
        int base_d = base + n_pairs_of(c);
        float myval = 0.f;
        int myidx = -1;
#pragma unroll
        for (int d = 1; d <= 2; ++d) {
            if (d <= window && have[d]) {
                float acc = 0.f;
#pragma unroll
                for (int i = 0; i < NCH; ++i) {
                    acc = __builtin_fmaf(R[0][i].x, R[d][i].x, acc);
                    acc = __builtin_fmaf(R[0][i].y, R[d][i].y, acc);
                    acc = __builtin_fmaf(R[0][i].z, R[d][i].z, acc);
                    acc = __builtin_fmaf(R[0][i].w, R[d][i].w, acc);
                }
                acc += __shfl_xor(acc, 8, 64);
                acc += __shfl_xor(acc, 4, 64);
                acc += __shfl_xor(acc, 2, 64);
                acc += __shfl_xor(acc, 1, 64);
                if (t == 2 * d - 2) { myval = acc + bv[d]; myidx = base + back_c + (d - 1); }
                if (t == 2 * d - 1) { myval = acc + bv[0]; myidx = base_d + (c - max(c + d - window, 0)); }
            }
            base_d += n_pairs_of(c + d);
        }
        if (myidx >= 0) {
            const float sc = fminf(fmaxf(myval, -10.0f), 10.0f);
            out[pi0 + myidx] = logf(1.0f + expf(sc));
        }
        base += n_pairs_of(c);
#pragma unroll
        for (int i = 0; i < NCH; ++i) { R[0][i] = R[1][i]; R[1][i] = R[2][i]; R[2][i] = Rn[i]; }
        have[0] = have[1]; have[1] = have[2]; have[2] = nh;
        bv[0] = bv[1]; bv[1] = bv[2]; bv[2] = nb;
    }
}

__global__ __launch_bounds__(256) void edge_dot_f64_kernel(const float *E, int ld, const int32_t *u, const int32_t *v, int64_t n, double *out) {
    const int t = threadIdx.x & 15;
    const int64_t g0 = ((int64_t)blockIdx.x * blockDim.x + threadIdx.x) >> 4, ng = ((int64_t)gridDim.x * blockDim.x) >> 4;
    for (int64_t p = g0; p < n; p += ng) {
        const float *ra = E + (int64_t)u[p] * ld, *rb = E + (int64_t)v[p] * ld;
        double acc = 0.0;
        for (int k = t; k < ld; k += 16) acc = fma((double)ra[k], (double)rb[k], acc);
        acc += __shfl_xor(acc, 8, 64);
        acc += __shfl_xor(acc, 4, 64);
        acc += __shfl_xor(acc, 2, 64);
        acc += __shfl_xor(acc, 1, 64);
        if (t == 0) out[p] = acc;
    }
}

int launch_pair_reward(gg_ctx *ctx, const int32_t *d_u, const int32_t *d_v, int64_t n, float *d_out) {
    if (n == 0) return GG_OK;
    const Model &D = ctx->model[1];
    int64_t blocks = (n * 16 + 255) / 256;
    if (blocks > 256 * 16) blocks = 256 * 16;
    hipLaunchKernelGGL(pair_reward_kernel, dim3((unsigned)blocks), dim3(256), 0, ctx->stream, D.E, D.b, ctx->ld, d_u, d_v, n,
                       (const int64_t *)nullptr, d_out);
    GG_HIP(ctx, hipGetLastError());
    ctx->ctr.reward_pairs += n;
    return GG_OK;
}

__global__ void d_count_kernel(const int32_t *status, const int64_t *walk_ptr, int n_slots, int32_t *cnt, const unsigned long long *flag) {
    const int i = blockIdx.x * blockDim.x + threadIdx.x;
    if (i >= n_slots) return;
    if (*flag == 2ull) { cnt[i] = 0; return; }
    const int64_t deg = walk_ptr[i + 1] - walk_ptr[i];
    cnt[i] = (status[i] == GG_ROOT_OK && deg > 0) ? (int32_t)(2 * deg) : 0;
}

__global__ __launch_bounds__(256) void d_fill_kernel(const int32_t *slots, const int32_t *t_root, const int64_t *g_rowptr,
                                                     const int32_t *g_col, const int32_t *samples, const int64_t *walk_ptr,
                                                     const int64_t *row_ptr, int n_slots, int32_t *center, int32_t *neighbor,
                                                     float *label, const unsigned long long *flag) {
    const int lane = threadIdx.x & 63;
    const int i = (blockIdx.x * blockDim.x + threadIdx.x) >> 6;
    if (i >= n_slots || *flag == 2ull) return;
    const int64_t o = row_ptr[i], rows = row_ptr[i + 1] - o;
    if (rows == 0) return;
    const int64_t deg = rows / 2;
    const int root = t_root[slots[i]];
    const int64_t e0 = g_rowptr[root], w0 = walk_ptr[i];
    for (int64_t e = lane; e < deg; e += 64) {
        center[o + e] = root;
        neighbor[o + e] = g_col[e0 + e];
        label[o + e] = 1.0f;
        center[o + deg + e] = root;
        neighbor[o + deg + e] = samples[w0 + e];
        label[o + deg + e] = 0.0f;
    }
}

static int fill_g_pairs(gg_ctx *ctx) {
    const int64_t nw = ctx->w_total;
    hipLaunchKernelGGL(pair_fill_kernel, dim3(cdiv(nw, 256)), dim3(256), 0, ctx->stream, ctx->w_paths.as<int32_t>(),
                       ctx->w_len.as<int32_t>(), ctx->w_stride, nw, ctx->cfg.window_size, ctx->g_ptr.as<int64_t>(),
                       ctx->g_node1.as<int32_t>(), ctx->g_node2.as<int32_t>(), ctx->dev_ctr + 3);
    GG_HIP(ctx, hipGetLastError());
    ctx->g_pairs_filled = true;
    return GG_OK;
}

int ensure_g_pairs(gg_ctx *ctx) {
    if (ctx->g_pairs_filled || ctx->g_pairs == 0) return GG_OK;
    GG_CHECK(ctx, ctx->g_paths_valid, GG_EINVAL,
             "the walks of the last gg_prepare_g were overwritten by a later walk launch before its pairs were read: fetch the pairs "
             "(gg_get_g_data) or run the minibatch passes before the next prepare call");
    return fill_g_pairs(ctx);
}

}

using namespace gg;

extern "C" {

static int enqueue_d_rows(gg_ctx *ctx, int32_t n_slots) {
    hipLaunchKernelGGL(d_count_kernel, dim3(cdiv(n_slots, 256)), dim3(256), 0, ctx->stream, ctx->w_status.as<int32_t>(),
                       ctx->w_ptr_buf().as<int64_t>(), n_slots, ctx->d_cnt.as<int32_t>(), ctx->dev_ctr + 3);
    int rc = device_exclusive_scan(ctx, ctx->d_cnt.as<int32_t>(), ctx->d_ptr.as<int64_t>(), n_slots);
    if (rc != GG_OK) return rc;
    hipLaunchKernelGGL(d_fill_kernel, dim3(cdiv((int64_t)n_slots * 64, 256)), dim3(256), 0, ctx->stream,
                       ctx->w_slots_buf().as<int32_t>(), ctx->t_root, ctx->g_rowptr, ctx->g_col, ctx->w_samples.as<int32_t>(),
                       ctx->w_ptr_buf().as<int64_t>(), ctx->d_ptr.as<int64_t>(), n_slots, ctx->d_center.as<int32_t>(),
                       ctx->d_neighbor.as<int32_t>(), ctx->d_label.as<float>(), ctx->dev_ctr + 3);
    GG_HIP(ctx, hipMemcpyAsync(ctx->h_pin + gg_ctx::H_TOTAL, ctx->d_ptr.as<int64_t>() + n_slots, sizeof(int64_t), hipMemcpyDeviceToHost, ctx->stream));
    GG_HIP(ctx, hipGetLastError());
    return GG_OK;
}

int gg_prepare_d(gg_ctx *ctx, const int32_t *slots, int32_t n_slots, uint64_t seed, uint32_t stream, int64_t *n_rows_out,
                 int32_t *root_status) {
    if (!ctx) return fail(nullptr, GG_EINVAL, "ctx is NULL");
    GG_CHECK(ctx, ctx->g_rowptr, GG_EINVAL, "gg_prepare_d: call gg_set_graph_csr first");
    const int stride = ctx->tree_max_depth + 3;
    ctx->d_rows = 0;
    ctx->dc_valid = false;
    discard_begun_walk(ctx);
    ctx->dc_request = ctx->dc_enabled ? 1 : 0;
    int rc = walk_launch_async(ctx, slots, nullptr, -1, n_slots, 1, seed, stream, stride);
    if (rc != GG_OK) { ctx->dc_request = 0; return rc; }
    if (n_slots > 0) {
        const int64_t cap = 2 * ctx->w_total;
        GG_HIP(ctx, ctx->d_cnt.reserve(sizeof(int32_t) * n_slots));
        GG_HIP(ctx, ctx->d_ptr.reserve(sizeof(int64_t) * (n_slots + 1)));
        GG_HIP(ctx, ctx->d_center.reserve(sizeof(int32_t) * (cap + 1)));
        GG_HIP(ctx, ctx->d_neighbor.reserve(sizeof(int32_t) * (cap + 1)));
        GG_HIP(ctx, ctx->d_label.reserve(sizeof(float) * (cap + 1)));
        rc = enqueue_d_rows(ctx, n_slots);
        if (rc != GG_OK) return rc;
    }
    bool retried = false;
    rc = walk_finalize(ctx, &retried);
    ctx->dc_request = 0;
    if (rc != GG_OK) return rc;
    if (n_slots > 0) {
        if (retried) {
            rc = enqueue_d_rows(ctx, n_slots);
            if (rc != GG_OK) return rc;
            GG_HIP(ctx, hipStreamSynchronize(ctx->stream));
        }
        ctx->d_rows = (int64_t)ctx->h_pin[gg_ctx::H_TOTAL];
        ctx->dc_valid = ctx->dc_enabled && ctx->walk_levels > 0;
        if (root_status) GG_HIP(ctx, hipMemcpy(root_status, ctx->w_status.p, sizeof(int32_t) * n_slots, hipMemcpyDeviceToHost));
    }
    if (!ctx->in_epoch_add) {
        rc = exchange_count_max(ctx, ctx->d_rows, &ctx->d_rows_max);
        if (rc != GG_OK) return rc;
    }
    if (n_rows_out) *n_rows_out = ctx->d_rows;
    return GG_OK;
}

int gg_get_d_data(gg_ctx *ctx, int32_t *center, int32_t *neighbor, float *label) {
    if (!ctx) return fail(nullptr, GG_EINVAL, "ctx is NULL");
    const int64_t n = ctx->d_rows;
    if (n == 0) return GG_OK;
    GG_HIP(ctx, hipSetDevice(ctx->device));
    GG_HIP(ctx, hipStreamSynchronize(ctx->stream));
    if (center) GG_HIP(ctx, hipMemcpy(center, ctx->d_center.p, sizeof(int32_t) * n, hipMemcpyDeviceToHost));
    if (neighbor) GG_HIP(ctx, hipMemcpy(neighbor, ctx->d_neighbor.p, sizeof(int32_t) * n, hipMemcpyDeviceToHost));
    if (label) GG_HIP(ctx, hipMemcpy(label, ctx->d_label.p, sizeof(float) * n, hipMemcpyDeviceToHost));
    return GG_OK;
}

static int enqueue_g_pairs(gg_ctx *ctx, int64_t nw, int64_t cap) {
    const int window = ctx->cfg.window_size;
    hipLaunchKernelGGL(pair_count_kernel, dim3(cdiv(nw, 256)), dim3(256), 0, ctx->stream, ctx->w_len.as<int32_t>(), nw, window,
                       ctx->g_cnt.as<int32_t>(), ctx->dev_ctr + 3);
    int rc = device_exclusive_scan(ctx, ctx->g_cnt.as<int32_t>(), ctx->g_ptr.as<int64_t>(), nw);
    if (rc != GG_OK) return rc;
    const int nch = (ctx->ld / 4 + 15) / 16;
    const bool path_reward = window <= 2 && nch <= 4 && ctx->ld % 4 == 0 && !getenv("GG_NO_PATH_REWARD");
    ctx->g_pairs_filled = false;
    if (!path_reward) {
        rc = fill_g_pairs(ctx);
        if (rc != GG_OK) return rc;
    }
    const Model &D = ctx->model[1];
    const int ts = ctx->walk_timed ? timing_slot(ctx) : -1;
    if (ts >= 0) GG_HIP(ctx, hipEventRecord(ctx->tm_ev[ts][0], ctx->stream));
    if (path_reward) {
        const dim3 grid(cdiv(nw * 16, 256)), blk(256);
#define GG_PATH_REWARD(N)                                                                                                              \
    hipLaunchKernelGGL(path_reward_kernel<N>, grid, blk, 0, ctx->stream, D.E, D.b, ctx->ld, ctx->w_paths.as<int32_t>(),                 \
                       ctx->w_len.as<int32_t>(), ctx->w_stride, nw, window, ctx->g_ptr.as<int64_t>(), ctx->g_reward.as<float>(), ctx->dev_ctr + 3)
        if (nch <= 1) GG_PATH_REWARD(1);
        else if (nch == 2) GG_PATH_REWARD(2);
        else GG_PATH_REWARD(4);
#undef GG_PATH_REWARD
    } else {
        hipLaunchKernelGGL(pair_reward_kernel, dim3(256 * 16), dim3(256), 0, ctx->stream, D.E, D.b, ctx->ld, ctx->g_node1.as<int32_t>(),
                           ctx->g_node2.as<int32_t>(), (int64_t)-1, ctx->g_ptr.as<int64_t>() + nw, ctx->g_reward.as<float>());
    }
    if (ts >= 0) {
        GG_HIP(ctx, hipEventRecord(ctx->tm_ev[ts][1], ctx->stream));
        GG_HIP(ctx, hipEventRecord(ctx->tm_ev[ts][2], ctx->stream));
        ctx->tm_pending.push_back({0, 0, ts, false});
    }
    GG_HIP(ctx, hipMemcpyAsync(ctx->h_pin + gg_ctx::H_TOTAL, ctx->g_ptr.as<int64_t>() + nw, sizeof(int64_t), hipMemcpyDeviceToHost, ctx->stream));
    GG_HIP(ctx, hipGetLastError());
    (void)cap;
    return GG_OK;
}

int gg_prepare_g_begin(gg_ctx *ctx, const int32_t *slots, int32_t n_slots, int32_t n_sample, uint64_t seed, uint32_t stream) {
    if (!ctx) return fail(nullptr, GG_EINVAL, "ctx is NULL");
    GG_CHECK(ctx, n_sample >= 0, GG_EINVAL, "gg_prepare_g_begin: n_sample < 0");
    const int stride = ctx->tree_max_depth + 3;
    discard_begun_walk(ctx);
    ctx->dc_request = ctx->dc_valid ? 2 : 0;
    int rc = walk_launch_async(ctx, slots, nullptr, n_sample, n_slots, 0, seed, stream, stride, true, true);
    if (rc != GG_OK) { ctx->dc_request = 0; return rc; }
    if (n_slots == 0) { ctx->dc_request = 0; return GG_OK; }
    ctx->g_begun = true;
    ctx->g_begun_args.n_slots = n_slots;
    ctx->g_begun_args.n_sample = n_sample;
    ctx->g_begun_args.seed = seed;
    ctx->g_begun_args.stream = stream;
    return GG_OK;
}

int gg_prepare_g(gg_ctx *ctx, const int32_t *slots, int32_t n_slots, int32_t n_sample, uint64_t seed, uint32_t stream,
                 int64_t *n_pairs_out, int32_t *root_status) {
    if (!ctx) return fail(nullptr, GG_EINVAL, "ctx is NULL");
    GG_CHECK(ctx, n_sample >= 0, GG_EINVAL, "gg_prepare_g: n_sample < 0");
    const int stride = ctx->tree_max_depth + 3;
    ctx->g_pairs = 0;
    int rc;
    const bool adopt = ctx->g_begun && ctx->g_begun_args.n_slots == n_slots && ctx->g_begun_args.n_sample == n_sample &&
                       ctx->g_begun_args.seed == seed && ctx->g_begun_args.stream == stream && slots &&
                       ctx->h_slots_m[0].size() == (size_t)n_slots && memcmp(ctx->h_slots_m[0].data(), slots, sizeof(int32_t) * n_slots) == 0;
    if (adopt) {
        ctx->g_begun = false;
        GG_HIP(ctx, hipSetDevice(ctx->device));
        GG_HIP(ctx, hipStreamWaitEvent(ctx->stream, ctx->ev_walk_done, 0));
    } else {
        discard_begun_walk(ctx);
        ctx->dc_request = ctx->dc_valid ? 2 : 0;
        rc = walk_launch_async(ctx, slots, nullptr, n_sample, n_slots, 0, seed, stream, stride, true);
        if (rc != GG_OK) { ctx->dc_request = 0; return rc; }
    }
    const int64_t nw = ctx->w_total;
    const int64_t cap = nw * 2 * ctx->cfg.window_size * (stride - 1);
    if (nw > 0) {
        GG_HIP(ctx, ctx->g_cnt.reserve(sizeof(int32_t) * nw));
        GG_HIP(ctx, ctx->g_ptr.reserve(sizeof(int64_t) * (nw + 1)));
        GG_HIP(ctx, ctx->g_node1.reserve(sizeof(int32_t) * (cap + 1)));
        GG_HIP(ctx, ctx->g_node2.reserve(sizeof(int32_t) * (cap + 1)));
        GG_HIP(ctx, ctx->g_reward.reserve(sizeof(float) * (cap + 1)));
        rc = enqueue_g_pairs(ctx, nw, cap);
        if (rc != GG_OK) return rc;
    }
    bool retried = false;
    const int64_t hops_before = ctx->ctr.hops;
    rc = walk_finalize(ctx, &retried);
    ctx->dc_request = 0;
    if (rc != GG_OK) return rc;
    if (nw > 0) {
        if (retried) {
            const int64_t cap2 = std::max<int64_t>(cap, nw * 2 * ctx->cfg.window_size * (ctx->w_stride - 1));
            GG_HIP(ctx, ctx->g_node1.reserve(sizeof(int32_t) * (cap2 + 1)));
            GG_HIP(ctx, ctx->g_node2.reserve(sizeof(int32_t) * (cap2 + 1)));
            GG_HIP(ctx, ctx->g_reward.reserve(sizeof(float) * (cap2 + 1)));
            rc = enqueue_g_pairs(ctx, nw, cap2);
            if (rc != GG_OK) return rc;
            GG_HIP(ctx, hipStreamSynchronize(ctx->stream));
        }
        ctx->g_pairs = (int64_t)ctx->h_pin[gg_ctx::H_TOTAL];
        ctx->ctr.reward_pairs += ctx->g_pairs;
        if (ctx->walk_timed) {
            ctx->ctr.reward_pairs_timed += ctx->g_pairs;
            ctx->ctr.g_walk_nodes_timed += ctx->ctr.hops - hops_before;
        }
        ctx->g_paths_valid = true;
    }
    if (root_status && n_slots) GG_HIP(ctx, hipMemcpy(root_status, ctx->w_status.p, sizeof(int32_t) * n_slots, hipMemcpyDeviceToHost));
    if (!ctx->in_epoch_add) {
        rc = exchange_count_max(ctx, ctx->g_pairs, &ctx->g_pairs_max);
        if (rc != GG_OK) return rc;
    }
    if (n_pairs_out) *n_pairs_out = ctx->g_pairs;
    return GG_OK;
}

int gg_get_g_data(gg_ctx *ctx, int32_t *node_1, int32_t *node_2, float *reward) {
    if (!ctx) return fail(nullptr, GG_EINVAL, "ctx is NULL");
    discard_begun_walk(ctx);
    const int64_t n = ctx->g_pairs;
    if (n == 0) return GG_OK;
    GG_HIP(ctx, hipSetDevice(ctx->device));
    if (node_1 || node_2) {
        int rc = ensure_g_pairs(ctx);
        if (rc != GG_OK) return rc;
    }
    GG_HIP(ctx, hipStreamSynchronize(ctx->stream));
    if (node_1) GG_HIP(ctx, hipMemcpy(node_1, ctx->g_node1.p, sizeof(int32_t) * n, hipMemcpyDeviceToHost));
    if (node_2) GG_HIP(ctx, hipMemcpy(node_2, ctx->g_node2.p, sizeof(int32_t) * n, hipMemcpyDeviceToHost));
    if (reward) GG_HIP(ctx, hipMemcpy(reward, ctx->g_reward.p, sizeof(float) * n, hipMemcpyDeviceToHost));
    return GG_OK;
}

int gg_pair_reward(gg_ctx *ctx, const int32_t *u, const int32_t *v, int64_t n, float *out) {
    if (!ctx) return fail(nullptr, GG_EINVAL, "ctx is NULL");
    GG_CHECK(ctx, n >= 0 && (n == 0 || (u && v && out)), GG_EINVAL, "gg_pair_reward: bad argument");
    if (n == 0) return GG_OK;
    for (int64_t i = 0; i < n; ++i)
        GG_CHECK(ctx, u[i] >= 0 && u[i] < ctx->n_node && v[i] >= 0 && v[i] < ctx->n_node, GG_EINVAL, "gg_pair_reward: id out of range at %lld", (long long)i);
    GG_HIP(ctx, hipSetDevice(ctx->device));
    GG_HIP(ctx, ctx->step_u.reserve(sizeof(int32_t) * n));
    GG_HIP(ctx, ctx->step_v.reserve(sizeof(int32_t) * n));
    GG_HIP(ctx, ctx->step_x.reserve(sizeof(float) * n));
    GG_HIP(ctx, hipMemcpyAsync(ctx->step_u.p, u, sizeof(int32_t) * n, hipMemcpyHostToDevice, ctx->stream));
    GG_HIP(ctx, hipMemcpyAsync(ctx->step_v.p, v, sizeof(int32_t) * n, hipMemcpyHostToDevice, ctx->stream));
    int rc = launch_pair_reward(ctx, ctx->step_u.as<int32_t>(), ctx->step_v.as<int32_t>(), n, ctx->step_x.as<float>());
    if (rc != GG_OK) return rc;
    GG_HIP(ctx, hipMemcpyAsync(out, ctx->step_x.p, sizeof(float) * n, hipMemcpyDeviceToHost, ctx->stream));
    GG_HIP(ctx, hipStreamSynchronize(ctx->stream));
    return GG_OK;
}

}

extern "C" int gg_edge_scores(gg_ctx *ctx, int32_t which, const int32_t *u, const int32_t *v, int64_t n, double *out) {
    if (!ctx) return fail(nullptr, GG_EINVAL, "ctx is NULL");
    GG_CHECK(ctx, (which == 0 || which == 1) && n >= 0 && (n == 0 || (u && v && out)), GG_EINVAL, "gg_edge_scores: bad argument");
    if (n == 0) return GG_OK;
    for (int64_t i = 0; i < n; ++i)
        GG_CHECK(ctx, u[i] >= 0 && u[i] < ctx->n_node && v[i] >= 0 && v[i] < ctx->n_node, GG_EINVAL, "gg_edge_scores: id out of range at %lld", (long long)i);
    GG_HIP(ctx, hipSetDevice(ctx->device));
    GG_HIP(ctx, ctx->step_u.reserve(sizeof(int32_t) * n));
    GG_HIP(ctx, ctx->step_v.reserve(sizeof(int32_t) * n));
    GG_HIP(ctx, ctx->step_x.reserve(sizeof(double) * n));
    GG_HIP(ctx, hipMemcpyAsync(ctx->step_u.p, u, sizeof(int32_t) * n, hipMemcpyHostToDevice, ctx->stream));
    GG_HIP(ctx, hipMemcpyAsync(ctx->step_v.p, v, sizeof(int32_t) * n, hipMemcpyHostToDevice, ctx->stream));
    int64_t blocks = std::min<int64_t>((n * 16 + 255) / 256, 4096);
    hipLaunchKernelGGL(edge_dot_f64_kernel, dim3((unsigned)blocks), dim3(256), 0, ctx->stream, ctx->model[which].E, ctx->ld,
                       ctx->step_u.as<int32_t>(), ctx->step_v.as<int32_t>(), n, ctx->step_x.as<double>());
    GG_HIP(ctx, hipGetLastError());
    GG_HIP(ctx, hipMemcpyAsync(out, ctx->step_x.p, sizeof(double) * n, hipMemcpyDeviceToHost, ctx->stream));
    GG_HIP(ctx, hipStreamSynchronize(ctx->stream));
    return GG_OK;
}
```

### graphgan_amd/csrc/steps.hip

```cpp
#include <stdlib.h>

#include <algorithm>
#include <cmath>
#include <vector>

#include "gg_internal.h"

namespace gg {

struct HubAcc {
    unsigned long long *acc;
    int64_t cap;
    float scale;
};
__device__ __forceinline__ unsigned long long *hub_row(const HubAcc &h, int slot, int ld) {
    const int64_t k = -3 - (int64_t)slot;
    return (slot <= -3 && k < h.cap) ? h.acc + k * (ld + 1) : nullptr;
}
__device__ __forceinline__ void hub_add(unsigned long long *p, float x, float scale) {
    atomicAdd(p, (unsigned long long)__float2ll_rn(x * scale));
}

struct StepArgs {
    float *E, *b;
// ... 1624 lines not shown
            if (bf16) hipLaunchKernelGGL(set_rows_kernel<true>, dim3(nbg), dim3(256), 0, ctx->stream, ctx->gradE, ctx->gradb, ctx->touched, ctx->x_recv_ids.as<int32_t>() + (size_t)r * cap,
                                         ctx->x_recv_rows.as<float>() + (size_t)r * cap * row_f, (int64_t)cap, ld);
            else hipLaunchKernelGGL(set_rows_kernel<false>, dim3(nbg), dim3(256), 0, ctx->stream, ctx->gradE, ctx->gradb, ctx->touched, ctx->x_recv_ids.as<int32_t>() + (size_t)r * cap,
                                    ctx->x_recv_rows.as<float>() + (size_t)r * cap * row_f, (int64_t)cap, ld);
        }
        bytes += (long long)(world - 1) * (long long)cap * (long long)(row_f + 1) * 4;
    } else {
        hipLaunchKernelGGL(owner_count_owned_kernel, dim3(256), dim3(256), 0, ctx->stream, ctx->touched_list, o.touched_total, bf16 ? 1 : world, 0, own);
        GG_HIP(ctx, hipMemcpyAsync(&umax, own, sizeof(long long), hipMemcpyDeviceToHost, ctx->stream));
        GG_HIP(ctx, hipStreamSynchronize(ctx->stream));
        const size_t cap = (size_t)std::max<long long>(umax, 1);
        GG_HIP(ctx, ctx->x_send_ids.reserve(sizeof(int32_t) * cap));
        GG_HIP(ctx, ctx->x_send_rows.reserve(sizeof(float) * cap * row_f));
        hipLaunchKernelGGL(fill_ids_kernel, dim3(256), dim3(256), 0, ctx->stream, ctx->x_send_ids.as<int32_t>(), (int64_t)cap, -1);
        GG_HIP(ctx, hipMemsetAsync(own + 1, 0, sizeof(long long), ctx->stream));
        int nbg = cdiv((int64_t)cap * 16, 256);
        if (nbg > 4096) nbg = 4096;
        const int wsim = bf16 ? 1 : world;
        if (bf16) {
            hipLaunchKernelGGL(owner_gather_pack_kernel<true>, dim3(nbg), dim3(256), 0, ctx->stream, ctx->gradE, ctx->gradb, ctx->touched_list, o.touched_total, wsim, 0, own + 1,
                               (int64_t)cap, ld, ctx->x_send_ids.as<int32_t>(), ctx->x_send_rows.as<float>());
            hipLaunchKernelGGL(set_rows_kernel<true>, dim3(nbg), dim3(256), 0, ctx->stream, ctx->gradE, ctx->gradb, ctx->touched, ctx->x_send_ids.as<int32_t>(),
                               ctx->x_send_rows.as<float>(), (int64_t)cap, ld);
        } else {
            hipLaunchKernelGGL(owner_gather_pack_kernel<false>, dim3(nbg), dim3(256), 0, ctx->stream, ctx->gradE, ctx->gradb, ctx->touched_list, o.touched_total, wsim, 0, own + 1,
                               (int64_t)cap, ld, ctx->x_send_ids.as<int32_t>(), ctx->x_send_rows.as<float>());
            hipLaunchKernelGGL(set_rows_kernel<false>, dim3(nbg), dim3(256), 0, ctx->stream, ctx->gradE, ctx->gradb, ctx->touched, ctx->x_send_ids.as<int32_t>(),
                               ctx->x_send_rows.as<float>(), (int64_t)cap, ld);
        }
    }
    GG_HIP(ctx, hipGetLastError());
    ctx->comm_steps_sparse += 1;
    ctx->comm_steps_owner += 1;
    if (ctx->comm) ctx->comm_bytes_sent += bytes;
    *taken = true;
    return GG_OK;
}

static int exchange_sparse(gg_ctx *ctx, OptArgs &o, int world, int64_t bound) {
    const int n = ctx->n_node, ld = ctx->ld;
    const int64_t cap = std::min<int64_t>(n, 2 * std::max<int64_t>(bound, 0));
    if (cap == 0) return GG_OK;
    if ((double)world * (double)cap >= (double)ctx->dense_exchange_ratio * n) {
        if (bound >= ctx->owner_min_bound) {
            bool taken = false;
            int rc = exchange_owner(ctx, o, world, &taken);
            if (rc != GG_OK) return rc;
            if (taken) return GG_OK;
        }
        if (ctx->comm) {
            int rc = comm_allreduce_grads(ctx);
            if (rc == GG_OK) rc = comm_allreduce_flags(ctx);
            if (rc != GG_OK) return rc;
            ctx->comm_bytes_sent += (int64_t)comm_dense_bytes(ctx) + (int64_t)(2.0 * 4.0 * n * (world - 1) / world);
        } else {
            hipLaunchKernelGGL(scale_grads_kernel, dim3(2048), dim3(256), 0, ctx->stream, ctx->gradE, ctx->gradb, (int64_t)n * ld, n, (float)world);
        }
        hipLaunchKernelGGL(normalize_flags_kernel, dim3(cdiv(n, 256)), dim3(256), 0, ctx->stream, ctx->touched, n);
        GG_HIP(ctx, hipGetLastError());
        ctx->comm_steps_dense += 1;
        return GG_OK;
    }
    int rc = device_compact_flags(ctx, ctx->touched, n, ctx->touched_list, ctx->touched_ptr.as<int64_t>() + n);
    if (rc != GG_OK) return rc;
    const size_t row_f = (size_t)ld + 1;
    GG_HIP(ctx, ctx->x_send_ids.reserve(sizeof(int32_t) * cap));
    GG_HIP(ctx, ctx->x_send_rows.reserve(sizeof(float) * cap * row_f));
    GG_HIP(ctx, ctx->x_recv_ids.reserve(sizeof(int32_t) * cap * world));
    GG_HIP(ctx, ctx->x_recv_rows.reserve(sizeof(float) * cap * row_f * world));
    int nb = cdiv(cap * 16, 256);
    if (nb > 4096) nb = 4096;
    hipLaunchKernelGGL(pack_rows_kernel, dim3(nb), dim3(256), 0, ctx->stream, ctx->gradE, ctx->gradb, ctx->touched, ctx->touched_list,
                       o.touched_total, cap, ld, ctx->x_send_ids.as<int32_t>(), ctx->x_send_rows.as<float>(), ctx->touched_cnt + 2);
    rc = comm_allgather(ctx, ctx->x_send_ids.p, ctx->x_recv_ids.p, (size_t)cap, 4);
    if (rc != GG_OK) return rc;
    rc = comm_allgather(ctx, ctx->x_send_rows.p, ctx->x_recv_rows.p, (size_t)cap * row_f, 4);
    if (rc != GG_OK) return rc;
    for (int r = 0; r < world; ++r)
        hipLaunchKernelGGL(add_rows_kernel<false>, dim3(nb), dim3(256), 0, ctx->stream, ctx->gradE, ctx->gradb, ctx->touched,
                           ctx->x_recv_ids.as<int32_t>() + (size_t)r * cap, ctx->x_recv_rows.as<float>() + (size_t)r * cap * row_f, cap, ld);
    GG_HIP(ctx, hipGetLastError());
    ctx->comm_steps_sparse += 1;
    if (ctx->comm) ctx->comm_bytes_sent += (int64_t)((world - 1) * cap * (row_f + 1) * 4);
    return GG_OK;
}

int exchange_count_max(gg_ctx *ctx, int64_t local, int64_t *max_out) {
    *max_out = local;
    if (!ctx->comm || ctx->world <= 1) return GG_OK;
    GG_HIP(ctx, ctx->x_nglob.reserve(sizeof(int64_t) * 4));
    int64_t *w = ctx->x_nglob.as<int64_t>() + 2;
    ctx->h_pin[gg_ctx::H_TOTAL + 2] = (unsigned long long)local;
    GG_HIP(ctx, hipMemcpyAsync(w, ctx->h_pin + gg_ctx::H_TOTAL + 2, sizeof(int64_t), hipMemcpyHostToDevice, ctx->stream));
    int rc = comm_allreduce_max_i64(ctx, w, 1);
    if (rc != GG_OK) return rc;
    GG_HIP(ctx, hipMemcpyAsync(ctx->h_pin + gg_ctx::H_TOTAL + 1, w, sizeof(int64_t), hipMemcpyDeviceToHost, ctx->stream));
    GG_HIP(ctx, hipStreamSynchronize(ctx->stream));
    *max_out = (int64_t)ctx->h_pin[gg_ctx::H_TOTAL + 1];
    return GG_OK;
}

int apply_optimizer(gg_ctx *ctx, int which, int64_t n) {
    const int opt = ctx->cfg.optimizer;
    int rc = GG_OK;
    if (opt == GG_OPT_ADAM_DENSE) {
        rc = comm_allreduce_grads(ctx);
        if (ctx->comm && ctx->world > 1) { ctx->comm_steps_dense += 1; ctx->comm_bytes_sent += (int64_t)comm_dense_bytes(ctx); }
    }
    if (rc != GG_OK) return rc;

    OptArgs o = make_opt_args(ctx, which);
    if (ctx->sg_active) o.sg_cnt = ctx->sg_cnt_active;
    if (opt == GG_OPT_ADAM_DENSE) {
        int64_t nb = (o.nE / 4 + 255) / 256;
        if (nb > 2048) nb = 2048;
        if (nb < 1) nb = 1;
        hipLaunchKernelGGL(adam_dense_kernel, dim3((unsigned)nb), dim3(256), 0, ctx->stream, o);
    } else {
        GG_HIP(ctx, ctx->touched_ptr.reserve(sizeof(int64_t) * ((size_t)ctx->n_node + 1)));
        o.touched_ptr = ctx->touched_ptr.as<int64_t>();
        o.touched_total = o.touched_ptr + ctx->n_node;
        const int world = ctx->comm ? ctx->world : ctx->fake_world;
        if (world > 1 || (ctx->comm && ctx->world == 1)) {
            rc = exchange_sparse(ctx, o, world < 1 ? 1 : world, ctx->step_bound > 0 ? ctx->step_bound : n);
            if (rc != GG_OK) return rc;
        }
        rc = device_compact_flags(ctx, ctx->touched, ctx->n_node, ctx->touched_list, ctx->touched_ptr.as<int64_t>() + ctx->n_node);
        if (rc != GG_OK) return rc;
        int nb = cdiv((int64_t)std::min<int64_t>(2ll * n * ctx->world, ctx->n_node) * 16, 256);
        if (nb > 4096) nb = 4096;
        if (nb < 1) nb = 1;
        if (opt == GG_OPT_SGD) hipLaunchKernelGGL(sparse_opt_kernel<1>, dim3(nb), dim3(256), 0, ctx->stream, o);
        else hipLaunchKernelGGL(sparse_opt_kernel<0>, dim3(nb), dim3(256), 0, ctx->stream, o);
    }
    GG_HIP(ctx, hipGetLastError());
    step_done(ctx, which, n);
    return GG_OK;
}

void step_done(gg_ctx *ctx, int which, int64_t n) {
    Model &M = ctx->model[which];
    if (which == 0) { ctx->gen_dirty = true; generator_changed(ctx); }
    M.t += 1;
    M.b1p = M.b1p * ctx->cfg.adam_beta1;
    M.b2p = M.b2p * ctx->cfg.adam_beta2;
    if (which == 1) { ctx->ctr.d_pairs += n; ctx->ctr.d_steps += 1; }
    else { ctx->ctr.g_pairs += n; ctx->ctr.g_steps += 1; }
}

}

using namespace gg;

static int host_step(gg_ctx *ctx, int which, const int32_t *u, const int32_t *v, const float *x, int32_t n) {
    if (!ctx) return fail(nullptr, GG_EINVAL, "ctx is NULL");
    if (which == 0) discard_begun_walk(ctx);
    GG_CHECK(ctx, n >= 0 && (n == 0 || (u && v && x)), GG_EINVAL, "step: bad argument");
    if (n == 0) return GG_OK;
    for (int i = 0; i < n; ++i)
        GG_CHECK(ctx, u[i] >= 0 && u[i] < ctx->n_node && v[i] >= 0 && v[i] < ctx->n_node, GG_EINVAL, "step: id out of range at %d", i);
    GG_HIP(ctx, hipSetDevice(ctx->device));
    GG_HIP(ctx, ctx->step_u.reserve(sizeof(int32_t) * n));
    GG_HIP(ctx, ctx->step_v.reserve(sizeof(int32_t) * n));
    GG_HIP(ctx, ctx->step_x.reserve(sizeof(float) * n));
    GG_HIP(ctx, hipMemcpyAsync(ctx->step_u.p, u, sizeof(int32_t) * n, hipMemcpyHostToDevice, ctx->stream));
    GG_HIP(ctx, hipMemcpyAsync(ctx->step_v.p, v, sizeof(int32_t) * n, hipMemcpyHostToDevice, ctx->stream));
    GG_HIP(ctx, hipMemcpyAsync(ctx->step_x.p, x, sizeof(float) * n, hipMemcpyHostToDevice, ctx->stream));
    ctx->step_bound = n;
    if (ctx->comm && ctx->world > 1 && ctx->cfg.optimizer != GG_OPT_ADAM_DENSE) {
        GG_HIP(ctx, ctx->x_nglob.reserve(sizeof(int64_t) * 4));
        int64_t *w = ctx->x_nglob.as<int64_t>() + 3;
        const int64_t mine = n;
        GG_HIP(ctx, hipMemcpyAsync(w, &mine, sizeof(int64_t), hipMemcpyHostToDevice, ctx->stream));
        int rc0 = comm_allreduce_max_i64(ctx, w, 1);
        if (rc0 != GG_OK) return rc0;
        int64_t mx = n;
        GG_HIP(ctx, hipMemcpyAsync(&mx, w, sizeof(int64_t), hipMemcpyDeviceToHost, ctx->stream));
        GG_HIP(ctx, hipStreamSynchronize(ctx->stream));
        ctx->step_bound = mx;
    }
    int rc = run_step(ctx, which, ctx->step_u.as<int32_t>(), ctx->step_v.as<int32_t>(), ctx->step_x.as<float>(), n);
    if (rc != GG_OK) return rc;
    GG_HIP(ctx, hipStreamSynchronize(ctx->stream));
    return GG_OK;
}

static int run_pass(gg_ctx *ctx, int which, const int64_t *starts, int64_t n_batches, int32_t batch_size) {
    if (!ctx) return fail(nullptr, GG_EINVAL, "ctx is NULL");
    if (which == 0) discard_begun_walk(ctx);
    GG_CHECK(ctx, batch_size > 0 && n_batches >= 0 && (starts || n_batches == 0), GG_EINVAL, "pass: bad argument");
    const int64_t rows = which == 1 ? ctx->d_rows : ctx->g_pairs;
    const int32_t *u = which == 1 ? ctx->d_center.as<int32_t>() : ctx->g_node1.as<int32_t>();
    const int32_t *v = which == 1 ? ctx->d_neighbor.as<int32_t>() : ctx->g_node2.as<int32_t>();
    const float *x = which == 1 ? ctx->d_label.as<float>() : ctx->g_reward.as<float>();
    GG_HIP(ctx, hipSetDevice(ctx->device));
    const int64_t rows_max = std::max(rows, which == 1 ? ctx->d_rows_max : ctx->g_pairs_max);
    auto empty_step = [&]() -> int {
        if (!ctx->comm) return GG_OK;
        if (which == 0) {
            const int64_t *unused = nullptr;
            int rc = global_pair_count(ctx, 0, &unused);
            if (rc != GG_OK) return rc;
        }
        return apply_optimizer(ctx, which, 0);
    };
    if (rows == 0) {
        ctx->step_bound = std::min<int64_t>(batch_size, rows_max);
        for (int64_t k = 0; k < n_batches; ++k) {
            int rc = empty_step();
            if (rc != GG_OK) return rc;
        }
        if (ctx->comm && n_batches > 0) GG_HIP(ctx, hipStreamSynchronize(ctx->stream));
        return GG_OK;
    }
    const bool timed = ctx->profile_every == 1;
    if (timed) GG_HIP(ctx, hipEventRecord(ctx->ev0, ctx->stream));
    const bool whole = n_batches == 1 && starts[0] == 0 && batch_size >= rows && rows > 0;
    ctx->tm_cur = -1;
    if (whole && ctx->profile_every > 0 && (ctx->pass_call_index[which]++ % ctx->profile_every) == 0 && !(ctx->deterministic && rows <= DET_MAX_PAIRS)) {
        ctx->tm_cur = timing_slot(ctx);
        if (ctx->tm_cur >= 0) GG_HIP(ctx, hipEventRecord(ctx->tm_ev[ctx->tm_cur][0], ctx->stream));
    }
    ctx->step_bound = std::min<int64_t>(batch_size, rows_max);
    if (which == 0 && whole && ctx->g_paths_valid && ctx->cfg.window_size <= 2 && ctx->ld <= 256 && !getenv("GG_NO_PATH_GRAD")) {
        int rc = run_path_step(ctx);
        if (rc != GG_OK) { ctx->tm_cur = -1; return rc; }
    } else {
        if (which == 0) {
            int rc = ensure_g_pairs(ctx);
            if (rc != GG_OK) { ctx->tm_cur = -1; return rc; }
        }
        for (int64_t k = 0; k < n_batches; ++k) {
            const int64_t s = starts[k];
            if (s < 0) {
                int rc = empty_step();
                if (rc != GG_OK) return rc;
                continue;
            }
            GG_CHECK(ctx, s < rows, GG_EINVAL, "pass: start %lld outside the %lld prepared rows", (long long)s, (long long)rows);
            const int32_t n = (int32_t)std::min<int64_t>(batch_size, rows - s);
            int rc = run_step(ctx, which, u + s, v + s, x + s, n);
            if (rc != GG_OK) return rc;
        }
    }
    if (ctx->tm_cur >= 0) {
        const int ts = ctx->tm_cur;
        ctx->tm_cur = -1;
        GG_HIP(ctx, hipEventRecord(ctx->tm_ev[ts][2], ctx->stream));
        const bool has_rows = ctx->cfg.optimizer != GG_OPT_ADAM_DENSE;
        if (has_rows)
            GG_HIP(ctx, hipMemcpyAsync(ctx->h_pin + gg_ctx::H_ROWS + ts, ctx->touched_ptr.as<int64_t>() + ctx->n_node, sizeof(int64_t),
                                       hipMemcpyDeviceToHost, ctx->stream));
        ctx->tm_pending.push_back({which == 1 ? 1 : 2, rows, ts, has_rows});
    }
    if (which == 0) {
        GG_HIP(ctx, hipEventRecord(ctx->ev_gen_pass, ctx->stream));
        ctx->gen_pass_recorded = true;
        ctx->gen_dirty = false;
    }
    if (timed) {
        GG_HIP(ctx, hipEventRecord(ctx->ev1, ctx->stream));
        GG_HIP(ctx, hipStreamSynchronize(ctx->stream));
        harvest_timings(ctx);
        float ms = 0.f;
        GG_HIP(ctx, hipEventElapsedTime(&ms, ctx->ev0, ctx->ev1));
        ctx->ctr.last_kernel_ms = ms;
    }
    return GG_OK;
}

extern "C" {

int gg_d_step(gg_ctx *ctx, const int32_t *u, const int32_t *v, const float *label, int32_t n) { return host_step(ctx, 1, u, v, label, n); }
int gg_g_step(gg_ctx *ctx, const int32_t *u, const int32_t *v, const float *reward, int32_t n) { return host_step(ctx, 0, u, v, reward, n); }
int gg_d_pass(gg_ctx *ctx, const int64_t *starts, int64_t n_batches, int32_t batch_size) { return run_pass(ctx, 1, starts, n_batches, batch_size); }
int gg_g_pass(gg_ctx *ctx, const int64_t *starts, int64_t n_batches, int32_t batch_size) { return run_pass(ctx, 0, starts, n_batches, batch_size); }

}
```

### graphgan_amd/csrc/walk_sample.hip

```cpp
#include <algorithm>

#include "gg_arith.h"
#include "gg_internal.h"

namespace gg {

constexpr int WAVES_PER_BLOCK = 4;
constexpr int SCORE_CAP = 1024;
constexpr int CHUNK = 16;

struct WalkArgs {
    const float *E;
    const float *bias;
    int32_t n_node, ld, nchunk;
    const int32_t *t_root;
    const int32_t *t_order;
    const int32_t *t_cstart;
    const int64_t *t_base;
    uint32_t *t_q3;
    const int64_t *t_q3off;
    const int32_t *slots;
    const int64_t *walk_ptr;
    int32_t n_slots;
    int64_t total_walks;
// ... 1422 lines not shown

                const uint64_t m53 = uniform53(a.seed, a.stream, (uint32_t)root, j, hop);
                int idx = sample_index([&](int jj) { return sbuf[jj]; }, k, mx, m53, lane);
                __builtin_amdgcn_wave_barrier();
                if (idx < 0) {
                    if (lane == 0) a.ctr[CTR_NONFINITE] = 1ull;
                    idx = 0;
                }
                const bool back = hf && idx == 0;
                const int nxt = back ? prev : ids[idx];
                my_hops += 1;
                my_reads += (unsigned long long)k;
                if (len >= a.stride) { overflow = true; break; }
                if (lane == 0) path[len] = nxt;
                len += 1;
                hop += 1;
                if (back) break;
                prev = cur;
                cur = nxt;
                rank = cbeg + idx - hf;
            }

            if (lane == 0) {
                if (overflow) {
                    a.ctr[3] = 1ull;
                    a.path_len[w] = 0;
                    a.samples[w] = -1;
                } else if (aborted) {
                    a.path_len[w] = 0;
                    a.samples[w] = -1;
                    if (!a.for_d) a.status[item] = GG_ROOT_ABORTED;
                    else if (hop == 0) atomicMin(&a.abort_walk[item], 0);
                } else {
                    a.path_len[w] = len;
                    a.samples[w] = cur;
                }
            }
        }
        unsigned long long nw = 0;
        if (lane == 0) nw = atomicAdd(&a.ctr[4], 1ull);
        it = n_waves + (int64_t)__shfl(nw, 0, 64);
    }

    if (lane == 0) {
        atomicAdd(&blk_ctr[0], my_hops);
        atomicAdd(&blk_ctr[1], my_reads);
    }
    __syncthreads();
    if (threadIdx.x == 0) {
        if (blk_ctr[0]) atomicAdd(&a.ctr[0], blk_ctr[0]);
        if (blk_ctr[1]) {
            atomicAdd(&a.ctr[1], blk_ctr[1]);
            atomicAdd(&a.ctr[5], blk_ctr[1]);
        }
    }
}

__global__ void walk_d_postpass_kernel(const WalkArgs a) {
    const int64_t w = (int64_t)blockIdx.x * blockDim.x + threadIdx.x;
    if (w >= a.total_walks || a.ctr[3] == 2ull || a.ctr[CTR_LZ_FB] != 0ull) return;
    const int item = find_item(a.walk_ptr, a.n_slots, w);
    const int j = (int)(w - a.walk_ptr[item]);
    const int ab = a.abort_walk[item];
    const int slot = a.slots[item];
    if (j < ab) {
        const int c = a.first_child[w];
        if (c >= 1) atomicOr(&a.t_q3[a.t_q3off[slot] + ((c - 1) >> 5)], 1u << ((c - 1) & 31));
    }
    if (ab != 0x7fffffff) {
        a.samples[w] = -1;
        a.path_len[w] = 0;
        if (j == 0) a.status[item] = GG_ROOT_ABORTED;
    }
}

__global__ void walk_reset_kernel(unsigned long long *ctr, int n_words, int64_t *dc_words, int append, int split, int64_t S, const unsigned long long *gen_bad) {
    const int i = blockIdx.x * blockDim.x + threadIdx.x;
    if (i < n_words && i != CTR_BASE && i != CTR_WORDS + CTR_BASE) ctr[i] = (i == CTR_NONFINITE) ? (*gen_bad ? 1ull : 0ull) : 0ull;
    if (i == 0) {
        if (!append) dc_words[1] = dc_words[3] = 0;
        const int64_t e0 = dc_words[1], e1 = dc_words[3];
        if (split) {
            dc_words[0] = append ? e0 : 0;
            dc_words[2] = (append && e1 > S) ? e1 : S;
        } else {
            dc_words[0] = append ? (e0 > e1 ? e0 : e1) : 0;
        }
        ctr[CTR_BASE] = (unsigned long long)dc_words[0];
        ctr[CTR_WORDS + CTR_BASE] = (unsigned long long)(split ? dc_words[2] : 0);
    }
}

__global__ void walk_init_status_kernel(const WalkArgs a) {
    const int i = blockIdx.x * blockDim.x + threadIdx.x;
    if (i >= a.n_slots) return;
    a.status[i] = (a.walk_ptr[i + 1] == a.walk_ptr[i]) ? GG_ROOT_EMPTY : GG_ROOT_OK;
    a.abort_walk[i] = 0x7fffffff;
}

static int reserve_level_buffers(gg_ctx *ctx, WalkArgs &a, int64_t chunks) {
    GG_HIP(ctx, ctx->lv_scores.reserve(sizeof(float) * CHUNK * (size_t)chunks + 256));
    GG_HIP(ctx, ctx->lv_chunk_owner.reserve(sizeof(int4) * 2 * (size_t)chunks + 256));
    a.lv_scores = ctx->lv_scores.as<float>();
    a.lv_chunk_desc = ctx->lv_chunk_owner.as<int4>();
    return GG_OK;
}

static int reserve_prefix(gg_ctx *ctx, WalkArgs &a, int64_t chunks, bool keep) {
    const size_t need = sizeof(uint64_t) * CHUNK * (size_t)chunks + 256;
    if (need > ctx->lv_prefix.bytes) {
        if (keep && ctx->lv_prefix.p) {
            DevBuf bigger;
            GG_HIP(ctx, bigger.reserve(need));
            GG_HIP(ctx, hipMemcpyAsync(bigger.p, ctx->lv_prefix.p, ctx->lv_prefix.bytes, hipMemcpyDeviceToDevice, ctx->walk_stream));
            GG_HIP(ctx, hipStreamSynchronize(ctx->walk_stream));
            ctx->lv_prefix.release();
            ctx->lv_prefix = bigger;
        } else {
            GG_HIP(ctx, ctx->lv_prefix.reserve(need));
        }
    }
    a.lv_prefix = ctx->lv_prefix.as<uint64_t>();
    a.cap_total = (int64_t)((ctx->lv_prefix.bytes - 256) / (sizeof(uint64_t) * CHUNK));
    return GG_OK;
}

__global__ __launch_bounds__(256) void fill_ones_kernel(uint4 *p, int64_t n16) {
    const uint4 v = make_uint4(~0u, ~0u, ~0u, ~0u);
    for (int64_t i = (int64_t)blockIdx.x * 256 + threadIdx.x; i < n16; i += (int64_t)gridDim.x * 256) p[i] = v;
}

__global__ void dc_finish_kernel(const WalkArgs a, int64_t *words, int n_levels) {
    if (a.ctr[3] == 2ull || a.ctr[CTR_LZ_FB] != 0ull) { words[1] = 0; return; }
    words[1] = (int64_t)a.lc[CTR_BASE + n_levels];
}


static void launch_lazy_resolve(gg_ctx *ctx, const WalkArgs &x, hipStream_t st) {
    const size_t lds = sizeof(uint32_t) * (size_t)x.lz_words;
    const bool no_lds = getenv("GG_LZ_NO_LDS") != nullptr;
    const size_t lds_static = sizeof(LzWork) * (LZ_T / 64) + 2 * sizeof(int32_t) * LZ_LIST + sizeof(LzCoop) + 256;
    if (!no_lds && lds + lds_static <= 160 * 1024) {
        static bool attr_set = false;
        if (!attr_set) {
            if (hipFuncSetAttribute((const void *)lazy_resolve_kernel<true>, hipFuncAttributeMaxDynamicSharedMemorySize, (int)(160 * 1024 - lds_static)) != hipSuccess) (void)hipGetLastError();
            attr_set = true;
        }
        hipLaunchKernelGGL(lazy_resolve_kernel<true>, dim3((unsigned)std::min<int64_t>(x.n_slots, ctx->n_cus)), dim3(LZ_T), lds, st, x);
    } else {
        hipLaunchKernelGGL(lazy_resolve_kernel<false>, dim3((unsigned)std::min<int64_t>(x.n_slots, 2 * ctx->n_cus)), dim3(LZ_T), 0, st, x);
    }
}

template <int NCH>
static int run_levels(gg_ctx *ctx, WalkArgs &a, int64_t total_walks, int n_levels, bool sized, bool finisher_follows, bool *any_alive) {
    const dim3 blk(WAVES_PER_BLOCK * 64);
    int64_t cap = sized ? 0 : ctx->lv_cap_chunks;
    const bool keep = a.dc_mode != 0;
    int64_t base_host = 0, cum = 0;
    const bool split = ctx->w_split;
    const int n_half = split ? 2 : 1;
    const int64_t S = ctx->lv_cap_total;
    if (!sized) {
        int rc = reserve_level_buffers(ctx, a, cap * n_half);
        if (rc == GG_OK) rc = reserve_prefix(ctx, a, std::max<int64_t>(S, cap) * n_half, keep);
        if (rc != GG_OK) return rc;
    } else {
        if (a.dc_mode == 2) {
            GG_HIP(ctx, hipMemcpyAsync(&base_host, a.dc_words, sizeof(int64_t), hipMemcpyDeviceToHost, ctx->walk_stream));
            GG_HIP(ctx, hipStreamSynchronize(ctx->walk_stream));
        }
        int rc = reserve_prefix(ctx, a, std::max<int64_t>(base_host, 1), keep);
        if (rc != GG_OK) return rc;
    }
    WalkArgs h[2] = {a, a};
    hipStream_t hs[2] = {ctx->walk_stream, ctx->stream3};
    if (split) {
        const int64_t mid = ((total_walks / 2 + 255) / 256) * 256;
        h[0].w0 = 0; h[0].w_end = mid;
        h[1].w0 = mid; h[1].w_end = total_walks;
        for (int k = 0; k < 2; ++k) {
            h[k].lc = ctx->dev_ctr + (size_t)k * CTR_WORDS;
            h[k].lv_big = a.lv_big + h[k].w0;
            h[k].lv_big_cap = h[k].w_end - h[k].w0;
            h[k].lv_scores = a.lv_scores + (size_t)k * cap * CHUNK;
            h[k].lv_chunk_desc = a.lv_chunk_desc + (size_t)2 * k * cap;
            h[k].dc_words = a.dc_words + 2 * k;
            h[k].cap_total = std::min<int64_t>((k + 1) * S, a.cap_total);
        }
        GG_HIP(ctx, hipEventRecord(ctx->ev_fork, hs[0]));
        GG_HIP(ctx, hipStreamWaitEvent(hs[1], ctx->ev_fork, 0));
    }
    const bool all_levels = n_levels >= ctx->tree_max_depth + 2;
    if (!sized && all_levels && !finisher_follows && ctx->lv_levels_learned > 0) n_levels = std::min(n_levels, ctx->lv_levels_learned);
    *any_alive = true;
    ctx->lv_ev_used = 0;
    int level = 0;
    for (; level < n_levels; ++level) {
        for (int k = 0; k < n_half; ++k) {
            WalkArgs &x = h[k];
            x.level = level;
            x.es_now = a.es_now + 2 * level + k;
            const unsigned wblocks = (unsigned)cdiv(x.w_end - x.w0, 256);
            if (!a.lazy) {
                hipLaunchKernelGGL(level_advance_kernel<false>, dim3(wblocks), dim3(256), 0, hs[k], x, level > 0 ? 1 : 0, 1, sized ? 0 : 1, cap);
            } else if (level == 0 || level < ctx->lz_min_level) {
                hipLaunchKernelGGL(level_advance_kernel<true>, dim3(wblocks), dim3(256), 0, hs[k], x, level > 0 ? 1 : 0, 1, sized ? 0 : 1, cap);
            } else {
                hipLaunchKernelGGL(level_advance_kernel<true>, dim3(wblocks), dim3(256), 0, hs[k], x, 1, 0, 0, cap);
                launch_lazy_resolve(ctx, x, hs[k]);
                hipLaunchKernelGGL(level_advance_kernel<true>, dim3(wblocks), dim3(256), 0, hs[k], x, 2, 1, sized ? 0 : 1, cap);
            }
            if (sized) {
                unsigned long long total_chunks = 0, alive = 0;
                GG_HIP(ctx, hipMemcpyAsync(&total_chunks, ctx->dev_ctr + CTR_CHUNKS + level, sizeof(total_chunks), hipMemcpyDeviceToHost, ctx->walk_stream));
                GG_HIP(ctx, hipMemcpyAsync(&alive, ctx->dev_ctr + CTR_ALIVE + level, sizeof(alive), hipMemcpyDeviceToHost, ctx->walk_stream));
                GG_HIP(ctx, hipStreamSynchronize(ctx->walk_stream));
                if (alive == 0) {
                    *any_alive = false;
                    ctx->w_levels_run = level + 1;
                    if (a.dc_mode == 1) hipLaunchKernelGGL(dc_finish_kernel, dim3(1), dim3(1), 0, ctx->walk_stream, x, ctx->dc_words.as<int64_t>(), level);
                    return GG_OK;
                }
                if (level + 1 > ctx->lv_levels_learned) ctx->lv_levels_learned = level + 1;
                const int64_t pch = (int64_t)(total_chunks & 0xffffffffull);
                cap = (int64_t)(total_chunks >> 32);
                const int64_t need = std::max(cap, pch);
                if (need + need / 2 + 4096 > ctx->lv_cap_chunks) ctx->lv_cap_chunks = need + need / 2 + 4096;
                int rc = reserve_level_buffers(ctx, x, cap);
                if (rc == GG_OK) rc = reserve_prefix(ctx, x, base_host + cum + pch, true);
                if (rc != GG_OK) return rc;
                cum += pch;
                if (base_host + cum + (base_host + cum) / 4 + 4096 > ctx->lv_cap_total) ctx->lv_cap_total = base_host + cum + (base_host + cum) / 4 + 4096;
                hipLaunchKernelGGL(level_expand_kernel, dim3(wblocks), dim3(256), 0, ctx->walk_stream, x);
            }
            int64_t blocks = sized ? (cap + WAVES_PER_BLOCK * 4 - 1) / (WAVES_PER_BLOCK * 4) : score_blocks();
            if (blocks > score_blocks()) blocks = score_blocks();
            if (blocks >= 8) blocks -= blocks % 8;
            if (blocks < 1) blocks = 1;
            if (split && (level > 0 || k == 1)) GG_HIP(ctx, hipStreamWaitEvent(hs[k], ctx->ev_score[1 - k], 0));
            hipEvent_t *ev = ctx->lv_ev + 4 * level + 2 * k;
            if (ctx->walk_timed) {
                if (!ev[0]) {
                    GG_HIP(ctx, hipEventCreate(&ev[0]));
                    GG_HIP(ctx, hipEventCreate(&ev[1]));
                }
                GG_HIP(ctx, hipEventRecord(ev[0], hs[k]));
            }
            hipLaunchKernelGGL(level_score_kernel<NCH>, dim3((unsigned)blocks), blk, 0, hs[k], x, cap);
            if (ctx->walk_timed) {
                GG_HIP(ctx, hipEventRecord(ev[1], hs[k]));
                ctx->lv_ev_used = level + 1;
            }
            if (split) GG_HIP(ctx, hipEventRecord(ctx->ev_score[k], hs[k]));
            const int64_t half_walks = x.w_end - x.w0;
            hipLaunchKernelGGL(level_weights_kernel, dim3((unsigned)(BIG_BLOCKS + std::min<int64_t>(SMALL_BLOCKS, cdiv(half_walks * 16, 256)))), dim3(256), 0, hs[k], x, cap);
        }
    }
    for (int k = 0; k < n_half; ++k) {
        WalkArgs &x = h[k];
        x.level = level;
        const unsigned wblocks = (unsigned)cdiv(x.w_end - x.w0, 256);
        const int wd_last = (!sized && all_levels && !finisher_follows) ? 2 : 0;
        if (!a.lazy) {
            hipLaunchKernelGGL(level_advance_kernel<false>, dim3(wblocks), dim3(256), 0, hs[k], x, 1, 2, wd_last, 0);
        } else if (level < ctx->lz_min_level) {
            hipLaunchKernelGGL(level_advance_kernel<true>, dim3(wblocks), dim3(256), 0, hs[k], x, 1, 2, wd_last, 0);
        } else {
            hipLaunchKernelGGL(level_advance_kernel<true>, dim3(wblocks), dim3(256), 0, hs[k], x, 1, 0, 0, 0);
            launch_lazy_resolve(ctx, x, hs[k]);
            hipLaunchKernelGGL(level_advance_kernel<true>, dim3(wblocks), dim3(256), 0, hs[k], x, 2, 2, wd_last, 0);
        }
        if (a.dc_mode == 1) hipLaunchKernelGGL(dc_finish_kernel, dim3(1), dim3(1), 0, hs[k], x, ctx->dc_words.as<int64_t>() + 2 * k, level);
    }
    if (split) {
        GG_HIP(ctx, hipEventRecord(ctx->ev_join, hs[1]));
        GG_HIP(ctx, hipStreamWaitEvent(hs[0], ctx->ev_join, 0));
    }
    a = h[0];
    a.w0 = 0; a.w_end = total_walks;
    ctx->w_levels_run = level;
    GG_HIP(ctx, hipGetLastError());
    return GG_OK;
}

template <int NCH>
static int run_levels_and_finish(gg_ctx *ctx, WalkArgs &a, int64_t total_walks) {
    const dim3 blk(WAVES_PER_BLOCK * 64);
    int n_levels = ctx->walk_levels < 0 ? 0 : ctx->walk_levels;
    const bool all_levels = n_levels >= ctx->tree_max_depth + 2;
    if (all_levels) n_levels = ctx->tree_max_depth + 2;
    if (n_levels > MAX_LEVELS) n_levels = MAX_LEVELS;
    bool any_alive = true, small_finisher = false;
    ctx->lv_ev_used = 0;
    ctx->w_levels_run = 0;
    ctx->w_fin_follows = true;
    ctx->w_net = false;
    if (n_levels > 0) {
        GG_HIP(ctx, ctx->st_cur.reserve(sizeof(int32_t) * total_walks));
        GG_HIP(ctx, ctx->st_prev.reserve(sizeof(int32_t) * total_walks));
        GG_HIP(ctx, ctx->st_len.reserve(sizeof(int32_t) * total_walks));
        GG_HIP(ctx, ctx->st_alive.reserve(sizeof(int32_t) * total_walks));
        GG_HIP(ctx, ctx->st_rank.reserve(sizeof(int32_t) * total_walks));
        GG_HIP(ctx, ctx->lv_beg.reserve(sizeof(int64_t) * total_walks));
        GG_HIP(ctx, ctx->lv_k.reserve(sizeof(int32_t) * total_walks));
        GG_HIP(ctx, ctx->lv_chunks.reserve(sizeof(int32_t) * total_walks));
        GG_HIP(ctx, ctx->lv_big.reserve(sizeof(int32_t) * total_walks));
        GG_HIP(ctx, ctx->lv_fe.reserve(sizeof(int32_t) * total_walks));
        GG_HIP(ctx, ctx->lv_coff.reserve(sizeof(int64_t) * (total_walks + 1)));
        GG_HIP(ctx, ctx->lv_pfx.reserve(sizeof(int64_t) * (total_walks + 1)));
        GG_HIP(ctx, ctx->st_item.reserve(sizeof(int4) * total_walks));
        GG_HIP(ctx, ctx->st_item2.reserve(sizeof(int4) * total_walks));
        a.st_cur = ctx->st_cur.as<int32_t>();
        a.st_prev = ctx->st_prev.as<int32_t>();
        a.st_len = ctx->st_len.as<int32_t>();
        a.st_alive = ctx->st_alive.as<int32_t>();
        a.st_rank = ctx->st_rank.as<int32_t>();
        a.st_const = ctx->st_item.as<int4>();
        a.st_const2 = ctx->st_item2.as<int4>();
        a.lv_beg = ctx->lv_beg.as<int64_t>();
        a.lv_k = ctx->lv_k.as<int32_t>();
        a.lv_chunks = ctx->lv_chunks.as<int32_t>();
        a.lv_big = ctx->lv_big.as<int32_t>();
        a.lv_fe = ctx->lv_fe.as<int32_t>();
        a.lv_coff = ctx->lv_coff.as<int64_t>();
        a.lv_pfx = ctx->lv_pfx.as<int64_t>();
        const bool sized = ctx->lv_cap_chunks == 0 || ctx->walk_force_sized;
        bool early = false;
        if (all_levels && !sized && ctx->fin_threshold > 0) {
            const int64_t *prof = ctx->alive_prof[a.for_d ? 1 : 0];
            for (int l = 1; l < n_levels && l < MAX_LEVELS; ++l)
                if (prof[l] >= 0 && prof[l] < ctx->fin_threshold) { n_levels = l; early = true; break; }
        }
        bool net = false;
        if (all_levels && !sized && !early && ctx->lv_levels_learned > 0 && ctx->lv_levels_learned < n_levels && !getenv("GG_WALK_NO_NET")) {
            n_levels = ctx->lv_levels_learned;
            net = true;
        }
        ctx->w_net = net;
        ctx->w_fin_follows = early || !all_levels || net;
        int rc = run_levels<NCH>(ctx, a, total_walks, n_levels, sized, early || net, &any_alive);
        if (rc != GG_OK) return rc;
        ctx->walk_used_speculation = !sized;
        if (all_levels && !early && !net) any_alive = false;
        if (net) small_finisher = true;
    }
    if (any_alive) {
        a.level = n_levels;
        int64_t blocks = (total_walks + WAVES_PER_BLOCK - 1) / WAVES_PER_BLOCK;
        const int64_t max_blocks = small_finisher ? 256 : 256 * 8;
        if (blocks > max_blocks) blocks = max_blocks;
        if (blocks >= 8) blocks -= blocks % 8;
        const int64_t need_stride = ctx->tree_max_list > SCORE_CAP ? ((ctx->tree_max_list + 63) / 64 * 64) : 0;
        GG_HIP(ctx, ctx->w_scratch.reserve((size_t)need_stride * blocks * WAVES_PER_BLOCK * sizeof(float) + 16));
        a.scratch = ctx->w_scratch.as<float>();
        a.scratch_stride = need_stride;
        if (a.lazy) hipLaunchKernelGGL((walk_sample_kernel<NCH, true>), dim3((unsigned)blocks), blk, 0, ctx->walk_stream, a);
        else hipLaunchKernelGGL((walk_sample_kernel<NCH, false>), dim3((unsigned)blocks), blk, 0, ctx->walk_stream, a);
    }
    GG_HIP(ctx, hipGetLastError());
    return GG_OK;
}

int launch_walk_sample(gg_ctx *ctx, int32_t n_slots, int64_t total_walks, int for_d, uint64_t seed, uint32_t stream,
                       int32_t stride) {
    WalkArgs a{};
    a.E = ctx->model[0].E;
    a.bias = ctx->model[0].b;
    a.n_node = ctx->n_node;
    a.ld = ctx->ld;
    a.nchunk = ctx->ld / 4;
    a.t_root = ctx->t_root;
    a.t_order = ctx->t_order;
    a.t_cstart = ctx->t_cstart;
    a.t_base = ctx->t_base;
    a.t_q3 = ctx->t_q3;
    a.t_q3off = ctx->t_q3off;
    a.slots = ctx->w_slots_buf().as<int32_t>();
    a.walk_ptr = ctx->w_ptr_buf().as<int64_t>();
    a.n_slots = n_slots;
    a.total_walks = total_walks;
    a.for_d = for_d;
    a.seed = seed;
    a.stream = stream;
    a.samples = ctx->w_samples.as<int32_t>();
    a.paths = ctx->w_paths.as<int32_t>();
    a.path_len = ctx->w_len.as<int32_t>();
    a.stride = stride;
    a.status = ctx->w_status.as<int32_t>();
    a.first_child = ctx->w_first.as<int32_t>();
    a.abort_walk = ctx->w_abort.as<int32_t>();
    a.ctr = ctx->dev_ctr;
    a.lc = ctx->dev_ctr;
    a.rowptr = ctx->g_rowptr;
    a.col = ctx->g_col;
    a.t_edge = ctx->t_edge;
    a.rev = ctx->g_rev;
    a.es = ctx->es;
    a.es_stamp = ctx->es_stamp;
    a.es_valid_from = ctx->es_valid_from;
    a.es_now = ctx->es_tick;
    ctx->es_tick += 256;
    a.es_ratio = ctx->es_ratio_num;
    a.es_hub = ctx->es_hub;
    a.es_mode = 0;
    {
        static const int exp_env = getenv("GG_WALK_EXPERIMENT") ? atoi(getenv("GG_WALK_EXPERIMENT")) : 0;
        a.exp = exp_env;
    }
    a.w0 = 0;
    a.w_end = total_walks;
    a.lv_big_cap = total_walks;
    a.lazy = ctx->t_lazy ? 1 : 0;
    a.t_order_w = ctx->t_order;
    a.t_edge_w = ctx->t_edge;
    if (a.lazy) {
        if (ctx->lz_list.bytes < sizeof(int32_t) * 2 * (size_t)n_slots) {
            GG_HIP(ctx, ctx->lz_list.reserve(sizeof(int32_t) * 2 * (size_t)n_slots));
            GG_HIP(ctx, hipMemset(ctx->lz_list.p, 0, ctx->lz_list.bytes));
        }
        a.lz_info = ctx->lz_info.as<int4>();
        a.lz_pair = ctx->lz_pair.as<unsigned long long>();
        a.lz_rank = ctx->lz_rank.as<int32_t>();
        a.lz_bm = ctx->lz_bm.as<uint2>();
        a.lz_words = (ctx->n_node + 31) / 32;
        a.lz_cursor = ctx->lz_cursor.as<int32_t>();
        a.lz_flag = ctx->lz_flag.as<int32_t>();
        a.lz_stamp = ctx->lz_stamp;
        a.g_multi = ctx->g_multi ? 1 : 0;
        a.lz_list = ctx->lz_list.as<int32_t>();
        {
            const bool stats_env = getenv("GG_LZ_STATS") != nullptr;
            a.lz_ctr = stats_env ? ctx->dev_ctr + 1500 : nullptr;
        }
        {
            static const int budget_env = getenv("GG_LZ_BUDGET") ? atoi(getenv("GG_LZ_BUDGET")) : 2048;
            a.lz_budget = budget_env > 0 ? budget_env : 0x7fffffff;
            const int coop_env = getenv("GG_LZ_COOP_MIN") ? atoi(getenv("GG_LZ_COOP_MIN")) : LZ_COOP_MIN;
            a.lz_coop_min = std::max(64, coop_env);
        }
    }
    GG_HIP(ctx, ctx->fin_list.reserve(sizeof(int32_t) * (size_t)(total_walks + 1)));
    a.fin_list = ctx->fin_list.as<int32_t>();
    GG_HIP(ctx, ctx->dc_words.reserve(sizeof(int64_t) * 8));
    a.dc_words = ctx->dc_words.as<int64_t>();
    a.dc_mode = (ctx->walk_levels > 0 && total_walks > 0) ? ctx->dc_request : 0;
    if (a.dc_mode == 1) {
        size_t want = 1u << 16;
        while (want < (size_t)total_walks * 8 && want < (1u << 24)) want <<= 1;
        if (want > ctx->dc_size) {
            GG_HIP(ctx, ctx->dc_keys.reserve(sizeof(ulonglong2) * want));
            ctx->dc_size = want;
        }
        hipLaunchKernelGGL(fill_ones_kernel, dim3(1024), dim3(256), 0, ctx->walk_stream, (uint4 *)ctx->dc_keys.p, (int64_t)ctx->dc_size);
    }
    a.dc_tab = ctx->dc_keys.as<ulonglong2>();
    a.dc_mask = (uint32_t)(ctx->dc_size ? ctx->dc_size - 1 : 0);
    const bool will_size = ctx->lv_cap_chunks == 0 || ctx->walk_force_sized;
    ctx->w_split = ctx->split_enabled && ctx->walk_levels > 0 && !will_size && total_walks >= ctx->split_min_walks && !ctx->t_lazy;
    if (ctx->es && ctx->es_stamp && ctx->g_rev && ctx->t_edge_valid && ctx->walk_levels > 0) a.es_mode = ctx->es_mode;
    hipLaunchKernelGGL(walk_reset_kernel, dim3(cdiv(2 * CTR_WORDS, 256)), dim3(256), 0, ctx->walk_stream, ctx->dev_ctr, 2 * (int)CTR_WORDS,
                       ctx->dc_words.as<int64_t>(), a.dc_mode == 2 ? 1 : 0, ctx->w_split ? 1 : 0, ctx->lv_cap_total, ctx->table_bad.as<unsigned long long>());
    if (!ctx->walk_force_sized) ctx->walk_timed = ctx->profile_every > 0 && (ctx->walk_call_index++ % ctx->profile_every) == 0;
    if (ctx->walk_timed && ctx->walk_stream != ctx->stream && ctx->profile_solo) {
        GG_HIP(ctx, hipEventRecord(ctx->ev_main_mark, ctx->stream));
        GG_HIP(ctx, hipStreamWaitEvent(ctx->walk_stream, ctx->ev_main_mark, 0));
    }
    hipLaunchKernelGGL(walk_init_status_kernel, dim3(cdiv(n_slots, 256)), dim3(256), 0, ctx->walk_stream, a);
    if (total_walks == 0) return GG_OK;

    const int nch = (a.nchunk + 15) / 16;
    if (ctx->walk_timed) GG_HIP(ctx, hipEventRecord(ctx->ev0, ctx->walk_stream));
    int rc;
    if (nch <= 1) rc = run_levels_and_finish<1>(ctx, a, total_walks);
    else if (nch == 2) rc = run_levels_and_finish<2>(ctx, a, total_walks);
    else if (nch <= 4) rc = run_levels_and_finish<4>(ctx, a, total_walks);
    else if (nch <= 8) rc = run_levels_and_finish<8>(ctx, a, total_walks);
    else return fail(ctx, GG_EINVAL, "n_emb %d not supported (max 512)", ctx->n_emb);
    if (rc != GG_OK) return rc;
    if (ctx->walk_timed) GG_HIP(ctx, hipEventRecord(ctx->ev1, ctx->walk_stream));
    if (for_d)
        hipLaunchKernelGGL(walk_d_postpass_kernel, dim3(cdiv(total_walks, 256)), dim3(256), 0, ctx->walk_stream, a);
    GG_HIP(ctx, hipGetLastError());
    return GG_OK;
}

}
```

Measured before the change: 664.0 million.

## Defer walk level launches and enqueue early counter/count readbacks on side stream

Adds a deferred-walk continuation that launches only the first few level kernels and resumes the rest after the training pass, so host launch work interleaves with the main stream. It also enqueues the counter and pair-count readbacks on the walk stream with events, letting finalize wait on events instead of a full stream sync. It adds a single-block scan kernel for small inputs and moves the generator pair count and scan onto the side stream. This cuts host-side sync and launch serialization, at the cost of more state machine complexity and possible ordering bugs.

```diff
diff --git a/graphgan_amd/csrc/gg_api.hip b/graphgan_amd/csrc/gg_api.hip
--- a/graphgan_amd/csrc/gg_api.hip
+++ b/graphgan_amd/csrc/gg_api.hip
@@ -141,28 +141,77 @@
 
 using namespace gg;
 
-static int launch_and_join(gg_ctx *ctx, int32_t n_slots, int64_t total, int32_t for_d, uint64_t seed, uint32_t stream, int32_t stride, bool join = true) {
+int gg::enqueue_ctr_readback(gg_ctx *ctx, hipStream_t stream) {
+    GG_HIP(ctx, hipMemcpyAsync(ctx->h_pin, ctx->dev_ctr, sizeof(unsigned long long) * 2 * gg_ctx::CTR_WORDS, hipMemcpyDeviceToHost, stream));
+    GG_HIP(ctx, hipEventRecord(ctx->ev_ctr, stream));
+    ctx->ctr_copied = true;
+    return GG_OK;
+}
+
+int gg::enqueue_count_readback(gg_ctx *ctx, const int64_t *count, hipStream_t stream) {
+    GG_HIP(ctx, hipMemcpyAsync(ctx->h_pin + gg_ctx::H_TOTAL, count, sizeof(int64_t), hipMemcpyDeviceToHost, stream));
+    GG_HIP(ctx, hipEventRecord(ctx->ev_count, stream));
+    ctx->count_copied = true;
+    return GG_OK;
+}
+
+static int side_launch_tail(gg_ctx *ctx, int32_t for_d, bool join, bool early_tail) {
+    hipStream_t st = ctx->walk_stream;
+    GG_HIP(ctx, hipEventRecord(ctx->ev_walk_done, st));
+    ctx->g_count_early = false;
+    if (early_tail && !for_d && ctx->w_total > 0 && !ctx->in_epoch_add) {
+        const bool early = env_on("GG_EARLY_COUNT");
+        if (early) {
+            int rc = enqueue_ctr_readback(ctx, st);
+            if (rc != GG_OK) return rc;
+        }
+        if (env_on("GG_SIDE_PAIRS")) {
+            int rc = enqueue_g_pair_count(ctx, st, &ctx->sgp_scan, early);
+            if (rc != GG_OK) return rc;
+            GG_HIP(ctx, hipEventRecord(ctx->ev_pairs_done, st));
+            ctx->g_count_early = true;
+        }
+    }
+    if (join) GG_HIP(ctx, hipStreamWaitEvent(ctx->stream, ctx->g_count_early ? ctx->ev_pairs_done : ctx->ev_walk_done, 0));
+    if (!for_d) return enqueue_path_slots(ctx);
+    return GG_OK;
+}
+
+static int launch_and_join(gg_ctx *ctx, int32_t n_slots, int64_t total, int32_t for_d, uint64_t seed, uint32_t stream, int32_t stride, bool join = true,
+                           bool early_tail = false) {
     const bool side = ctx->walk_stream != ctx->stream;
+    ctx->ctr_copied = ctx->count_copied = false;
+    ctx->g_count_early = false;
     int rc = launch_walk_sample(ctx, n_slots, total, for_d, seed, stream, stride);
     if (rc != GG_OK) {
+        ctx->walk_cont_pending = false;
         if (side) (void)hipStreamSynchronize(ctx->walk_stream);
         return rc;
     }
-    if (side) {
-        GG_HIP(ctx, hipEventRecord(ctx->ev_walk_done, ctx->walk_stream));
-        if (join) GG_HIP(ctx, hipStreamWaitEvent(ctx->stream, ctx->ev_walk_done, 0));
-        if (!for_d) {
-            rc = enqueue_path_slots(ctx);
-            if (rc != GG_OK) return rc;
-        }
-    }
-    return GG_OK;
+    if (ctx->walk_cont_pending) return GG_OK;
+    if (side) return side_launch_tail(ctx, for_d, join, early_tail);
+    return GG_OK;
+}
+
+int gg::flush_begun_walk(gg_ctx *ctx) {
+    if (!ctx->walk_cont_pending) return GG_OK;
+    ctx->walk_cont_pending = false;
+    GG_HIP(ctx, hipSetDevice(ctx->device));
+    int rc = walk_resume(ctx);
+    if (rc != GG_OK) {
+        (void)hipStreamSynchronize(ctx->walk_stream);
+        return rc;
+    }
+    return side_launch_tail(ctx, 0, false, true);
 }
 
 void gg::discard_begun_walk(gg_ctx *ctx) {
-    if (!ctx->g_begun) return;
+    if (!ctx->g_begun) { ctx->walk_cont_pending = false; return; }
+    (void)flush_begun_walk(ctx);
     (void)hipStreamSynchronize(ctx->stream2);
     ctx->g_begun = false;
+    ctx->ctr_copied = ctx->count_copied = false;
+    ctx->g_count_early = false;
     ctx->dc_request = 0;
     ctx->walk_stream = ctx->stream;
     ctx->w_nslots = 0;
@@ -211,6 +260,10 @@
     } else if (side_stream && ctx->gen_pass_recorded) {
         GG_HIP(ctx, hipStreamWaitEvent(ctx->stream2, ctx->ev_gen_pass, 0));
     }
+    if (ctx->fill_pending) {
+        if (side_stream) GG_HIP(ctx, hipStreamWaitEvent(ctx->stream2, ctx->ev_fill, 0));
+        ctx->fill_pending = false;
+    }
     std::vector<int32_t> &hs = ctx->h_slots_m[mode];
     if (hs.size() != (size_t)n_slots || (n_slots && memcmp(hs.data(), slots, sizeof(int32_t) * n_slots) != 0)) {
         hs.assign(slots, slots + n_slots);
@@ -235,20 +288,30 @@
         ctx->walk_stream = ctx->stream;
         return GG_OK;
     }
-    return launch_and_join(ctx, n_slots, total, for_d, seed, stream, stride, !defer_join);
+    ctx->walk_defer_req = defer_join && side_stream && env_on("GG_DEFER_WALK");
+    const int rc = launch_and_join(ctx, n_slots, total, for_d, seed, stream, stride, !defer_join, true);
+    ctx->walk_defer_req = false;
+    return rc;
 }
 
 int gg::walk_finalize(gg_ctx *ctx, bool *retried) {
     if (retried) *retried = false;
     if (ctx->w_nslots == 0) {
+        ctx->ctr_copied = ctx->count_copied = false;
         GG_HIP(ctx, hipStreamSynchronize(ctx->stream));
         return GG_OK;
     }
     const int64_t total = ctx->w_total;
     unsigned long long *c = ctx->h_pin;
     constexpr int CW = gg_ctx::CTR_WORDS;
-    GG_HIP(ctx, hipMemcpyAsync(c, ctx->dev_ctr, sizeof(unsigned long long) * 2 * CW, hipMemcpyDeviceToHost, ctx->stream));
-    GG_HIP(ctx, hipStreamSynchronize(ctx->stream));
+    if (ctx->ctr_copied && ctx->count_copied) {
+        GG_HIP(ctx, hipEventSynchronize(ctx->ev_ctr));
+        GG_HIP(ctx, hipEventSynchronize(ctx->ev_count));
+    } else {
+        if (!ctx->ctr_copied) GG_HIP(ctx, hipMemcpyAsync(c, ctx->dev_ctr, sizeof(unsigned long long) * 2 * CW, hipMemcpyDeviceToHost, ctx->stream));
+        GG_HIP(ctx, hipStreamSynchronize(ctx->stream));
+    }
+    ctx->ctr_copied = ctx->count_copied = false;
     harvest_timings(ctx);
     for (int attempt = 0; c[3] == 2ull || (c[2] != 0ull && ctx->t_lazy); ++attempt) {
         GG_CHECK(ctx, attempt < 16, GG_EHIP, "walk: the launch was voided %d times in a row", attempt);
@@ -410,6 +473,10 @@
         GG_HIP(ctx, hipEventCreate(&ctx->ev0));
         GG_HIP(ctx, hipEventCreate(&ctx->ev1));
         GG_HIP(ctx, hipEventCreateWithFlags(&ctx->ev_walk_done, hipEventDisableTiming));
+        GG_HIP(ctx, hipEventCreateWithFlags(&ctx->ev_ctr, hipEventDisableTiming));
+        GG_HIP(ctx, hipEventCreateWithFlags(&ctx->ev_fill, hipEventDisableTiming));
+        GG_HIP(ctx, hipEventCreateWithFlags(&ctx->ev_count, hipEventDisableTiming));
+        GG_HIP(ctx, hipEventCreateWithFlags(&ctx->ev_pairs_done, hipEventDisableTiming));
         GG_HIP(ctx, hipEventCreateWithFlags(&ctx->ev_gen_pass, hipEventDisableTiming));
         GG_HIP(ctx, hipEventCreateWithFlags(&ctx->ev_main_mark, hipEventDisableTiming));
         GG_HIP(ctx, hipHostMalloc((void **)&ctx->h_pin, sizeof(unsigned long long) * gg_ctx::PIN_WORDS, hipHostMallocDefault));
@@ -466,6 +533,8 @@
 int gg_destroy(gg_ctx *ctx) {
     if (!ctx) return GG_OK;
     (void)hipSetDevice(ctx->device);
+    (void)flush_begun_walk(ctx);
+    walk_cont_release(ctx);
     if (ctx->stream) (void)hipStreamSynchronize(ctx->stream);
     if (ctx->stream2) (void)hipStreamSynchronize(ctx->stream2);
     comm_destroy(ctx);
@@ -497,7 +566,7 @@
     for (hipEvent_t e : ctx->pt_ev)
         if (e) (void)hipEventDestroy(e);
     if (ctx->h_pin) (void)hipHostFree(ctx->h_pin);
-    for (hipEvent_t e : {ctx->ev_walk_done, ctx->ev_slots_done, ctx->ev_gen_pass, ctx->ev_main_mark, ctx->ev_fork, ctx->ev_join, ctx->ev_score[0], ctx->ev_score[1]})
+    for (hipEvent_t e : {ctx->ev_fill, ctx->ev_ctr, ctx->ev_count, ctx->ev_pairs_done, ctx->ev_walk_done, ctx->ev_slots_done, ctx->ev_gen_pass, ctx->ev_main_mark, ctx->ev_fork, ctx->ev_join, ctx->ev_score[0], ctx->ev_score[1]})
         if (e) (void)hipEventDestroy(e);
     if (ctx->stream3) {
         (void)hipStreamSynchronize(ctx->stream3);
@@ -1035,7 +1104,11 @@
     if (!ctx) return fail(nullptr, GG_EINVAL, "ctx is NULL");
     GG_HIP(ctx, hipSetDevice(ctx->device));
     GG_HIP(ctx, hipStreamSynchronize(ctx->stream));
-    if (ctx->g_begun) GG_HIP(ctx, hipStreamSynchronize(ctx->stream2));
+    if (ctx->g_begun) {
+        int rc = flush_begun_walk(ctx);
+        if (rc != GG_OK) return rc;
+        GG_HIP(ctx, hipStreamSynchronize(ctx->stream2));
+    }
     harvest_timings(ctx);
     return check_exchange_flag(ctx);
 }
diff --git a/graphgan_amd/csrc/gg_internal.h b/graphgan_amd/csrc/gg_internal.h
--- a/graphgan_amd/csrc/gg_internal.h
+++ b/graphgan_amd/csrc/gg_internal.h
@@ -2,6 +2,7 @@
 #include <hip/hip_runtime.h>
 #include <stdint.h>
 #include <stdio.h>
+#include <stdlib.h>
 #include <string>
 #include <vector>
 
@@ -167,6 +168,15 @@
     bool g_paths_valid = false;
     bool g_begun = false;
     struct { int32_t n_slots = 0, n_sample = 0; uint64_t seed = 0; uint32_t stream = 0; } g_begun_args;
+    void *walk_cont = nullptr;
+    bool walk_cont_pending = false;
+    bool walk_defer_req = false;
+    hipEvent_t ev_ctr = nullptr, ev_count = nullptr;
+    hipEvent_t ev_fill = nullptr;
+    bool fill_pending = false;
+    bool ctr_copied = false, count_copied = false;
+    hipEvent_t ev_pairs_done = nullptr;
+    bool g_count_early = false;
     gg::DevBuf touched_ptr;
     gg::DevBuf bfs_key, bfs_bm, bfs_misc, bfs_sparse, bfs_rowptr32;
     bool bfs_rowptr32_valid = false;
@@ -252,7 +262,13 @@
         if (!(cond)) return gg::fail(ctx, code, __VA_ARGS__); \
     } while (0)
 
-int device_exclusive_scan(gg_ctx *ctx, const int32_t *cnt, int64_t *ptr, int64_t n);
+static inline bool env_on(const char *name) {
+    const char *s = getenv(name);
+    return !(s && s[0] == '0');
+}
+
+int device_exclusive_scan(gg_ctx *ctx, const int32_t *cnt, int64_t *ptr, int64_t n, hipStream_t stream = nullptr, DevBuf *scratch = nullptr);
+int enqueue_g_pair_count(gg_ctx *ctx, hipStream_t stream, DevBuf *scratch, bool early);
 int ensure_g_pairs(gg_ctx *ctx);
 int device_compact_flags(gg_ctx *ctx, const int32_t *flag, int64_t n, int32_t *list, int64_t *total_out);
 int device_segment_rows(gg_ctx *ctx, const int32_t *cnt, int64_t n, int T, int32_t *off, int4 *list, int64_t *totals, hipStream_t stream = nullptr,
@@ -272,7 +288,12 @@
 int walk_launch_async(gg_ctx *ctx, const int32_t *slots, const int32_t *n_walks, int32_t uniform_walks, int32_t n_slots,
                       int32_t for_d, uint64_t seed, uint32_t stream, int32_t stride, bool side_stream = false, bool defer_join = false);
 void discard_begun_walk(gg_ctx *ctx);
+int flush_begun_walk(gg_ctx *ctx);
+int walk_resume(gg_ctx *ctx);
+void walk_cont_release(gg_ctx *ctx);
 int walk_finalize(gg_ctx *ctx, bool *retried);
+int enqueue_ctr_readback(gg_ctx *ctx, hipStream_t stream);
+int enqueue_count_readback(gg_ctx *ctx, const int64_t *count, hipStream_t stream);
 int timing_slot(gg_ctx *ctx);
 int check_exchange_flag(gg_ctx *ctx);
 void harvest_timings(gg_ctx *ctx);
diff --git a/graphgan_amd/csrc/prepare.hip b/graphgan_amd/csrc/prepare.hip
--- a/graphgan_amd/csrc/prepare.hip
+++ b/graphgan_amd/csrc/prepare.hip
@@ -90,17 +90,69 @@
     }
 }
 
-int device_exclusive_scan(gg_ctx *ctx, const int32_t *cnt, int64_t *ptr, int64_t n) {
+constexpr int SCAN1_THREADS = 1024;
+__global__ __launch_bounds__(SCAN1_THREADS) void scan_one_kernel(const int32_t *cnt, int64_t n, int64_t *ptr) {
+    __shared__ int64_t sh[SCAN1_THREADS / 64];
+    const int lane = threadIdx.x & 63, wv = threadIdx.x >> 6;
+    int64_t carry = 0;
+    for (int64_t t0 = 0; t0 < n; t0 += (int64_t)SCAN1_THREADS * SCAN_ITEMS) {
+        const int64_t base = t0 + (int64_t)threadIdx.x * SCAN_ITEMS;
+        int64_t v[SCAN_ITEMS], s = 0;
+#pragma unroll
+        for (int i = 0; i < SCAN_ITEMS; ++i) {
+            v[i] = base + i < n ? cnt[base + i] : 0;
+            s += v[i];
+        }
+        int64_t inc = s;
+#pragma unroll
+        for (int off = 1; off < 64; off <<= 1) {
+            const int64_t o = __shfl_up(inc, off, 64);
+            if (lane >= off) inc += o;
+        }
+        if (lane == 63) sh[wv] = inc;
+        __syncthreads();
+        int64_t wbase = 0, tot = 0;
+#pragma unroll
+        for (int i = 0; i < SCAN1_THREADS / 64; ++i) {
+            if (i < wv) wbase += sh[i];
+            tot += sh[i];
+        }
+        __syncthreads();
+        int64_t run = carry + wbase + inc - s;
+#pragma unroll
+        for (int i = 0; i < SCAN_ITEMS; ++i) {
+            if (base + i < n) ptr[base + i] = run;
+            run += v[i];
+        }
+        carry += tot;
+    }
+    if (threadIdx.x == 0) ptr[n] = carry;
+}
+
+static int64_t scan_one_max() {
+    if (!env_on("GG_SCAN_ONE")) return 0;
+    const char *s = getenv("GG_SCAN_ONE_MAX");
+    return s ? atoll(s) : (int64_t)4 * SCAN1_THREADS * SCAN_ITEMS;
+}
+
+int device_exclusive_scan(gg_ctx *ctx, const int32_t *cnt, int64_t *ptr, int64_t n, hipStream_t stream, DevBuf *scratch) {
+    if (!scratch) scratch = &ctx->scan_tmp;
+    if (!stream) stream = ctx->stream;
+    if (n == 0) {
+        GG_HIP(ctx, hipMemsetAsync(ptr, 0, sizeof(int64_t), stream));
+        return GG_OK;
+    }
+    if (n <= scan_one_max()) {
+        hipLaunchKernelGGL(scan_one_kernel, dim3(1), dim3(SCAN1_THREADS), 0, stream, cnt, n, ptr);
+        GG_HIP(ctx, hipGetLastError());
+        return GG_OK;
+    }
     const int64_t tiles = (n + SCAN_TILE - 1) / SCAN_TILE;
-    GG_HIP(ctx, ctx->scan_tmp.reserve(sizeof(int64_t) * (tiles + 2)));
-    int64_t *ts = ctx->scan_tmp.as<int64_t>();
-    if (n == 0) {
-        GG_HIP(ctx, hipMemsetAsync(ptr, 0, sizeof(int64_t), ctx->stream));
-        return GG_OK;
-    }
-    hipLaunchKernelGGL(scan_tile_sums, dim3((unsigned)tiles), dim3(SCAN_THREADS), 0, ctx->stream, cnt, n, ts);
-    hipLaunchKernelGGL(scan_tile_offsets, dim3(1), dim3(SCAN_THREADS), 0, ctx->stream, ts, tiles, ptr + n);
-    hipLaunchKernelGGL(scan_apply, dim3((unsigned)tiles), dim3(SCAN_THREADS), 0, ctx->stream, cnt, n, ts, ptr);
+    GG_HIP(ctx, scratch->reserve(sizeof(int64_t) * (tiles + 2)));
+    int64_t *ts = scratch->as<int64_t>();
+    hipLaunchKernelGGL(scan_tile_sums, dim3((unsigned)tiles), dim3(SCAN_THREADS), 0, stream, cnt, n, ts);
+    hipLaunchKernelGGL(scan_tile_offsets, dim3(1), dim3(SCAN_THREADS), 0, stream, ts, tiles, ptr + n);
+    hipLaunchKernelGGL(scan_apply, dim3((unsigned)tiles), dim3(SCAN_THREADS), 0, stream, cnt, n, ts, ptr);
     GG_HIP(ctx, hipGetLastError());
     return GG_OK;
 }
@@ -406,6 +458,18 @@
     return GG_OK;
 }
 
+int enqueue_g_pair_count(gg_ctx *ctx, hipStream_t stream, DevBuf *scratch, bool early) {
+    const int64_t nw = ctx->w_total;
+    GG_HIP(ctx, ctx->g_cnt.reserve(sizeof(int32_t) * nw));
+    GG_HIP(ctx, ctx->g_ptr.reserve(sizeof(int64_t) * (nw + 1)));
+    hipLaunchKernelGGL(pair_count_kernel, dim3(cdiv(nw, 256)), dim3(256), 0, stream, ctx->w_len.as<int32_t>(), nw, ctx->cfg.window_size,
+                       ctx->g_cnt.as<int32_t>(), ctx->dev_ctr + 3);
+    int rc = device_exclusive_scan(ctx, ctx->g_cnt.as<int32_t>(), ctx->g_ptr.as<int64_t>(), nw, stream, scratch);
+    if (rc != GG_OK) return rc;
+    if (early) return enqueue_count_readback(ctx, ctx->g_ptr.as<int64_t>() + nw, stream);
+    return GG_OK;
+}
+
 int ensure_g_pairs(gg_ctx *ctx) {
     if (ctx->g_pairs_filled || ctx->g_pairs == 0) return GG_OK;
     GG_CHECK(ctx, ctx->g_paths_valid, GG_EINVAL,
@@ -420,16 +484,28 @@
 
 extern "C" {
 
-static int enqueue_d_rows(gg_ctx *ctx, int32_t n_slots) {
+static int enqueue_d_rows(gg_ctx *ctx, int32_t n_slots, bool early) {
+    if (early) {
+        int rc = enqueue_ctr_readback(ctx, ctx->stream);
+        if (rc != GG_OK) return rc;
+    }
     hipLaunchKernelGGL(d_count_kernel, dim3(cdiv(n_slots, 256)), dim3(256), 0, ctx->stream, ctx->w_status.as<int32_t>(),
                        ctx->w_ptr_buf().as<int64_t>(), n_slots, ctx->d_cnt.as<int32_t>(), ctx->dev_ctr + 3);
     int rc = device_exclusive_scan(ctx, ctx->d_cnt.as<int32_t>(), ctx->d_ptr.as<int64_t>(), n_slots);
     if (rc != GG_OK) return rc;
+    if (early) {
+        rc = enqueue_count_readback(ctx, ctx->d_ptr.as<int64_t>() + n_slots, ctx->stream);
+        if (rc != GG_OK) return rc;
+    }
     hipLaunchKernelGGL(d_fill_kernel, dim3(cdiv((int64_t)n_slots * 64, 256)), dim3(256), 0, ctx->stream,
                        ctx->w_slots_buf().as<int32_t>(), ctx->t_root, ctx->g_rowptr, ctx->g_col, ctx->w_samples.as<int32_t>(),
                        ctx->w_ptr_buf().as<int64_t>(), ctx->d_ptr.as<int64_t>(), n_slots, ctx->d_center.as<int32_t>(),
                        ctx->d_neighbor.as<int32_t>(), ctx->d_label.as<float>(), ctx->dev_ctr + 3);
-    GG_HIP(ctx, hipMemcpyAsync(ctx->h_pin + gg_ctx::H_TOTAL, ctx->d_ptr.as<int64_t>() + n_slots, sizeof(int64_t), hipMemcpyDeviceToHost, ctx->stream));
+    if (!early) GG_HIP(ctx, hipMemcpyAsync(ctx->h_pin + gg_ctx::H_TOTAL, ctx->d_ptr.as<int64_t>() + n_slots, sizeof(int64_t), hipMemcpyDeviceToHost, ctx->stream));
+    if (early) {
+        GG_HIP(ctx, hipEventRecord(ctx->ev_fill, ctx->stream));
+        ctx->fill_pending = true;
+    }
     GG_HIP(ctx, hipGetLastError());
     return GG_OK;
 }
@@ -452,7 +528,7 @@
         GG_HIP(ctx, ctx->d_center.reserve(sizeof(int32_t) * (cap + 1)));
         GG_HIP(ctx, ctx->d_neighbor.reserve(sizeof(int32_t) * (cap + 1)));
         GG_HIP(ctx, ctx->d_label.reserve(sizeof(float) * (cap + 1)));
-        rc = enqueue_d_rows(ctx, n_slots);
+        rc = enqueue_d_rows(ctx, n_slots, env_on("GG_EARLY_COUNT"));
         if (rc != GG_OK) return rc;
     }
     bool retried = false;
@@ -461,13 +537,16 @@
     if (rc != GG_OK) return rc;
     if (n_slots > 0) {
         if (retried) {
-            rc = enqueue_d_rows(ctx, n_slots);
+            rc = enqueue_d_rows(ctx, n_slots, false);
             if (rc != GG_OK) return rc;
             GG_HIP(ctx, hipStreamSynchronize(ctx->stream));
         }
         ctx->d_rows = (int64_t)ctx->h_pin[gg_ctx::H_TOTAL];
         ctx->dc_valid = ctx->dc_enabled && ctx->walk_levels > 0;
-        if (root_status) GG_HIP(ctx, hipMemcpy(root_status, ctx->w_status.p, sizeof(int32_t) * n_slots, hipMemcpyDeviceToHost));
+        if (root_status) {
+            GG_HIP(ctx, hipStreamSynchronize(ctx->stream));
+            GG_HIP(ctx, hipMemcpy(root_status, ctx->w_status.p, sizeof(int32_t) * n_slots, hipMemcpyDeviceToHost));
+        }
     }
     if (!ctx->in_epoch_add) {
         rc = exchange_count_max(ctx, ctx->d_rows, &ctx->d_rows_max);
@@ -489,12 +568,15 @@
     return GG_OK;
 }
 
-static int enqueue_g_pairs(gg_ctx *ctx, int64_t nw, int64_t cap) {
+static int enqueue_g_pairs(gg_ctx *ctx, int64_t nw, int64_t cap, bool early) {
     const int window = ctx->cfg.window_size;
-    hipLaunchKernelGGL(pair_count_kernel, dim3(cdiv(nw, 256)), dim3(256), 0, ctx->stream, ctx->w_len.as<int32_t>(), nw, window,
-                       ctx->g_cnt.as<int32_t>(), ctx->dev_ctr + 3);
-    int rc = device_exclusive_scan(ctx, ctx->g_cnt.as<int32_t>(), ctx->g_ptr.as<int64_t>(), nw);
-    if (rc != GG_OK) return rc;
+    if (ctx->g_count_early) {
+        ctx->g_count_early = false;
+    } else {
+        int rc = enqueue_g_pair_count(ctx, ctx->stream, nullptr, early);
+        if (rc != GG_OK) return rc;
+    }
+    int rc;
     const int nch = (ctx->ld / 4 + 15) / 16;
     const bool path_reward = window <= 2 && nch <= 4 && ctx->ld % 4 == 0 && !getenv("GG_NO_PATH_REWARD");
     ctx->g_pairs_filled = false;
@@ -523,7 +605,7 @@
         GG_HIP(ctx, hipEventRecord(ctx->tm_ev[ts][2], ctx->stream));
         ctx->tm_pending.push_back({0, 0, ts, false});
     }
-    GG_HIP(ctx, hipMemcpyAsync(ctx->h_pin + gg_ctx::H_TOTAL, ctx->g_ptr.as<int64_t>() + nw, sizeof(int64_t), hipMemcpyDeviceToHost, ctx->stream));
+    if (!ctx->count_copied) GG_HIP(ctx, hipMemcpyAsync(ctx->h_pin + gg_ctx::H_TOTAL, ctx->g_ptr.as<int64_t>() + nw, sizeof(int64_t), hipMemcpyDeviceToHost, ctx->stream));
     GG_HIP(ctx, hipGetLastError());
     (void)cap;
     return GG_OK;
@@ -552,14 +634,15 @@
     GG_CHECK(ctx, n_sample >= 0, GG_EINVAL, "gg_prepare_g: n_sample < 0");
     const int stride = ctx->tree_max_depth + 3;
     ctx->g_pairs = 0;
-    int rc;
+    int rc = flush_begun_walk(ctx);
+    if (rc != GG_OK) { discard_begun_walk(ctx); return rc; }
     const bool adopt = ctx->g_begun && ctx->g_begun_args.n_slots == n_slots && ctx->g_begun_args.n_sample == n_sample &&
                        ctx->g_begun_args.seed == seed && ctx->g_begun_args.stream == stream && slots &&
                        ctx->h_slots_m[0].size() == (size_t)n_slots && memcmp(ctx->h_slots_m[0].data(), slots, sizeof(int32_t) * n_slots) == 0;
     if (adopt) {
         ctx->g_begun = false;
         GG_HIP(ctx, hipSetDevice(ctx->device));
-        GG_HIP(ctx, hipStreamWaitEvent(ctx->stream, ctx->ev_walk_done, 0));
+        GG_HIP(ctx, hipStreamWaitEvent(ctx->stream, ctx->g_count_early ? ctx->ev_pairs_done : ctx->ev_walk_done, 0));
     } else {
         discard_begun_walk(ctx);
         ctx->dc_request = ctx->dc_valid ? 2 : 0;
@@ -569,12 +652,10 @@
     const int64_t nw = ctx->w_total;
     const int64_t cap = nw * 2 * ctx->cfg.window_size * (stride - 1);
     if (nw > 0) {
-        GG_HIP(ctx, ctx->g_cnt.reserve(sizeof(int32_t) * nw));
-        GG_HIP(ctx, ctx->g_ptr.reserve(sizeof(int64_t) * (nw + 1)));
         GG_HIP(ctx, ctx->g_node1.reserve(sizeof(int32_t) * (cap + 1)));
         GG_HIP(ctx, ctx->g_node2.reserve(sizeof(int32_t) * (cap + 1)));
         GG_HIP(ctx, ctx->g_reward.reserve(sizeof(float) * (cap + 1)));
-        rc = enqueue_g_pairs(ctx, nw, cap);
+        rc = enqueue_g_pairs(ctx, nw, cap, env_on("GG_EARLY_COUNT"));
         if (rc != GG_OK) return rc;
     }
     bool retried = false;
@@ -588,7 +669,8 @@
             GG_HIP(ctx, ctx->g_node1.reserve(sizeof(int32_t) * (cap2 + 1)));
             GG_HIP(ctx, ctx->g_node2.reserve(sizeof(int32_t) * (cap2 + 1)));
             GG_HIP(ctx, ctx->g_reward.reserve(sizeof(float) * (cap2 + 1)));
-            rc = enqueue_g_pairs(ctx, nw, cap2);
+            ctx->g_count_early = false;
+            rc = enqueue_g_pairs(ctx, nw, cap2, false);
             if (rc != GG_OK) return rc;
             GG_HIP(ctx, hipStreamSynchronize(ctx->stream));
         }
@@ -600,7 +682,10 @@
         }
         ctx->g_paths_valid = true;
     }
-    if (root_status && n_slots) GG_HIP(ctx, hipMemcpy(root_status, ctx->w_status.p, sizeof(int32_t) * n_slots, hipMemcpyDeviceToHost));
+    if (root_status && n_slots) {
+        GG_HIP(ctx, hipStreamSynchronize(ctx->stream));
+        GG_HIP(ctx, hipMemcpy(root_status, ctx->w_status.p, sizeof(int32_t) * n_slots, hipMemcpyDeviceToHost));
+    }
     if (!ctx->in_epoch_add) {
         rc = exchange_count_max(ctx, ctx->g_pairs, &ctx->g_pairs_max);
         if (rc != GG_OK) return rc;
diff --git a/graphgan_amd/csrc/steps.hip b/graphgan_amd/csrc/steps.hip
--- a/graphgan_amd/csrc/steps.hip
+++ b/graphgan_amd/csrc/steps.hip
@@ -1800,8 +1800,7 @@
 
 using namespace gg;
 
-static int host_step(gg_ctx *ctx, int which, const int32_t *u, const int32_t *v, const float *x, int32_t n) {
-    if (!ctx) return fail(nullptr, GG_EINVAL, "ctx is NULL");
+static int host_step_impl(gg_ctx *ctx, int which, const int32_t *u, const int32_t *v, const float *x, int32_t n) {
     if (which == 0) discard_begun_walk(ctx);
     GG_CHECK(ctx, n >= 0 && (n == 0 || (u && v && x)), GG_EINVAL, "step: bad argument");
     if (n == 0) return GG_OK;
@@ -1833,8 +1832,14 @@
     return GG_OK;
 }
 
-static int run_pass(gg_ctx *ctx, int which, const int64_t *starts, int64_t n_batches, int32_t batch_size) {
+static int host_step(gg_ctx *ctx, int which, const int32_t *u, const int32_t *v, const float *x, int32_t n) {
     if (!ctx) return fail(nullptr, GG_EINVAL, "ctx is NULL");
+    const int rc = host_step_impl(ctx, which, u, v, x, n);
+    const int rc2 = flush_begun_walk(ctx);
+    return rc != GG_OK ? rc : rc2;
+}
+
+static int run_pass_impl(gg_ctx *ctx, int which, const int64_t *starts, int64_t n_batches, int32_t batch_size) {
     if (which == 0) discard_begun_walk(ctx);
     GG_CHECK(ctx, batch_size > 0 && n_batches >= 0 && (starts || n_batches == 0), GG_EINVAL, "pass: bad argument");
     const int64_t rows = which == 1 ? ctx->d_rows : ctx->g_pairs;
@@ -1908,6 +1913,8 @@
     }
     if (timed) {
         GG_HIP(ctx, hipEventRecord(ctx->ev1, ctx->stream));
+        int rc = flush_begun_walk(ctx);
+        if (rc != GG_OK) return rc;
         GG_HIP(ctx, hipStreamSynchronize(ctx->stream));
         harvest_timings(ctx);
         float ms = 0.f;
@@ -1917,6 +1924,13 @@
     return GG_OK;
 }
 
+static int run_pass(gg_ctx *ctx, int which, const int64_t *starts, int64_t n_batches, int32_t batch_size) {
+    if (!ctx) return fail(nullptr, GG_EINVAL, "ctx is NULL");
+    const int rc = run_pass_impl(ctx, which, starts, n_batches, batch_size);
+    const int rc2 = flush_begun_walk(ctx);
+    return rc != GG_OK ? rc : rc2;
+}
+
 extern "C" {
 
 int gg_d_step(gg_ctx *ctx, const int32_t *u, const int32_t *v, const float *label, int32_t n) { return host_step(ctx, 1, u, v, label, n); }
diff --git a/graphgan_amd/csrc/walk_sample.hip b/graphgan_amd/csrc/walk_sample.hip
--- a/graphgan_amd/csrc/walk_sample.hip
+++ b/graphgan_amd/csrc/walk_sample.hip
@@ -1598,16 +1598,35 @@
     }
 }
 
+struct WalkCont {
+    WalkArgs a;
+    int64_t total_walks = 0, cap = 0;
+    int nch = 0;
+    int n_levels = 0;
+    int run_levels = 0;
+    int next_level = 0;
+    bool early = false, net = false, all_levels = false;
+};
+
+static int defer_head_levels() {
+    const char *s = getenv("GG_DEFER_HEAD");
+    const int v = s ? atoi(s) : 2;
+    return v < 1 ? 1 : v;
+}
+
 template <int NCH>
-static int run_levels(gg_ctx *ctx, WalkArgs &a, int64_t total_walks, int n_levels, bool sized, bool finisher_follows, bool *any_alive) {
+static int run_levels(gg_ctx *ctx, WalkArgs &a, int64_t total_walks, int n_levels, bool sized, bool finisher_follows, bool *any_alive,
+                      WalkCont *resume = nullptr, int pause_at = -1, WalkCont *pause_out = nullptr) {
     const dim3 blk(WAVES_PER_BLOCK * 64);
     int64_t cap = sized ? 0 : ctx->lv_cap_chunks;
+    if (resume) cap = resume->cap;
     const bool keep = a.dc_mode != 0;
     int64_t base_host = 0, cum = 0;
     const bool split = ctx->w_split;
     const int n_half = split ? 2 : 1;
     const int64_t S = ctx->lv_cap_total;
-    if (!sized) {
+    if (resume) {
+    } else if (!sized) {
         int rc = reserve_level_buffers(ctx, a, cap * n_half);
         if (rc == GG_OK) rc = reserve_prefix(ctx, a, std::max<int64_t>(S, cap) * n_half, keep);
         if (rc != GG_OK) return rc;
@@ -1621,7 +1640,7 @@
     }
     WalkArgs h[2] = {a, a};
     hipStream_t hs[2] = {ctx->walk_stream, ctx->stream3};
-    if (split) {
+    if (split && !resume) {
         const int64_t mid = ((total_walks / 2 + 255) / 256) * 256;
         h[0].w0 = 0; h[0].w_end = mid;
         h[1].w0 = mid; h[1].w_end = total_walks;
@@ -1639,10 +1658,21 @@
     }
     const bool all_levels = n_levels >= ctx->tree_max_depth + 2;
     if (!sized && all_levels && !finisher_follows && ctx->lv_levels_learned > 0) n_levels = std::min(n_levels, ctx->lv_levels_learned);
+    if (resume) n_levels = resume->run_levels;
     *any_alive = true;
-    ctx->lv_ev_used = 0;
-    int level = 0;
+    if (!resume) ctx->lv_ev_used = 0;
+    int level = resume ? resume->next_level : 0;
     for (; level < n_levels; ++level) {
+        if (level == pause_at && pause_out) {
+            pause_out->a = h[0];
+            pause_out->a.es_now = a.es_now;
+            pause_out->cap = cap;
+            pause_out->run_levels = n_levels;
+            pause_out->next_level = level;
+            GG_HIP(ctx, hipGetLastError());
+            ctx->walk_cont_pending = true;
+            return GG_OK;
+        }
         for (int k = 0; k < n_half; ++k) {
             WalkArgs &x = h[k];
             x.level = level;
@@ -1731,8 +1761,34 @@
 }
 
 template <int NCH>
-static int run_levels_and_finish(gg_ctx *ctx, WalkArgs &a, int64_t total_walks) {
+static int launch_finisher(gg_ctx *ctx, WalkArgs &a, int64_t total_walks, int n_levels, bool small_finisher) {
     const dim3 blk(WAVES_PER_BLOCK * 64);
+    a.level = n_levels;
+    int64_t blocks = (total_walks + WAVES_PER_BLOCK - 1) / WAVES_PER_BLOCK;
+    const int64_t max_blocks = small_finisher ? 256 : 256 * 8;
+    if (blocks > max_blocks) blocks = max_blocks;
+    if (blocks >= 8) blocks -= blocks % 8;
+    const int64_t need_stride = ctx->tree_max_list > SCORE_CAP ? ((ctx->tree_max_list + 63) / 64 * 64) : 0;
+    GG_HIP(ctx, ctx->w_scratch.reserve((size_t)need_stride * blocks * WAVES_PER_BLOCK * sizeof(float) + 16));
+    a.scratch = ctx->w_scratch.as<float>();
+    a.scratch_stride = need_stride;
+    if (a.lazy) hipLaunchKernelGGL((walk_sample_kernel<NCH, true>), dim3((unsigned)blocks), blk, 0, ctx->walk_stream, a);
+    else hipLaunchKernelGGL((walk_sample_kernel<NCH, false>), dim3((unsigned)blocks), blk, 0, ctx->walk_stream, a);
+    GG_HIP(ctx, hipGetLastError());
+    return GG_OK;
+}
+
+template <int NCH>
+static int run_levels_and_finish(gg_ctx *ctx, WalkArgs &a, int64_t total_walks, WalkCont *resume = nullptr) {
+    if (resume) {
+        bool alive = true;
+        a = resume->a;
+        const int n_lv = resume->n_levels;
+        int rc = run_levels<NCH>(ctx, a, total_walks, n_lv, false, resume->early || resume->net, &alive, resume);
+        if (rc != GG_OK) return rc;
+        if (resume->all_levels && !resume->early && !resume->net) alive = false;
+        return alive ? launch_finisher<NCH>(ctx, a, total_walks, n_lv, resume->net) : GG_OK;
+    }
     int n_levels = ctx->walk_levels < 0 ? 0 : ctx->walk_levels;
     const bool all_levels = n_levels >= ctx->tree_max_depth + 2;
     if (all_levels) n_levels = ctx->tree_max_depth + 2;
@@ -1785,25 +1841,23 @@
         }
         ctx->w_net = net;
         ctx->w_fin_follows = early || !all_levels || net;
-        int rc = run_levels<NCH>(ctx, a, total_walks, n_levels, sized, early || net, &any_alive);
+        WalkCont *pause = nullptr;
+        if (ctx->walk_defer_req && !sized && !ctx->w_split && ctx->profile_every != 1 && !ctx->in_epoch_add) {
+            if (!ctx->walk_cont) ctx->walk_cont = new WalkCont();
+            pause = (WalkCont *)ctx->walk_cont;
+            pause->total_walks = total_walks;
+            pause->nch = NCH;
+            pause->n_levels = n_levels;
+            pause->early = early; pause->net = net; pause->all_levels = all_levels;
+        }
+        int rc = run_levels<NCH>(ctx, a, total_walks, n_levels, sized, early || net, &any_alive, nullptr, pause ? defer_head_levels() : -1, pause);
         if (rc != GG_OK) return rc;
         ctx->walk_used_speculation = !sized;
+        if (ctx->walk_cont_pending) return GG_OK;
         if (all_levels && !early && !net) any_alive = false;
         if (net) small_finisher = true;
     }
-    if (any_alive) {
-        a.level = n_levels;
-        int64_t blocks = (total_walks + WAVES_PER_BLOCK - 1) / WAVES_PER_BLOCK;
-        const int64_t max_blocks = small_finisher ? 256 : 256 * 8;
-        if (blocks > max_blocks) blocks = max_blocks;
-        if (blocks >= 8) blocks -= blocks % 8;
-        const int64_t need_stride = ctx->tree_max_list > SCORE_CAP ? ((ctx->tree_max_list + 63) / 64 * 64) : 0;
-        GG_HIP(ctx, ctx->w_scratch.reserve((size_t)need_stride * blocks * WAVES_PER_BLOCK * sizeof(float) + 16));
-        a.scratch = ctx->w_scratch.as<float>();
-        a.scratch_stride = need_stride;
-        if (a.lazy) hipLaunchKernelGGL((walk_sample_kernel<NCH, true>), dim3((unsigned)blocks), blk, 0, ctx->walk_stream, a);
-        else hipLaunchKernelGGL((walk_sample_kernel<NCH, false>), dim3((unsigned)blocks), blk, 0, ctx->walk_stream, a);
-    }
+    if (any_alive) return launch_finisher<NCH>(ctx, a, total_walks, n_levels, small_finisher);
     GG_HIP(ctx, hipGetLastError());
     return GG_OK;
 }
@@ -1924,6 +1978,7 @@
     else if (nch <= 8) rc = run_levels_and_finish<8>(ctx, a, total_walks);
     else return fail(ctx, GG_EINVAL, "n_emb %d not supported (max 512)", ctx->n_emb);
     if (rc != GG_OK) return rc;
+    if (ctx->walk_cont_pending) return GG_OK;
     if (ctx->walk_timed) GG_HIP(ctx, hipEventRecord(ctx->ev1, ctx->walk_stream));
     if (for_d)
         hipLaunchKernelGGL(walk_d_postpass_kernel, dim3(cdiv(total_walks, 256)), dim3(256), 0, ctx->walk_stream, a);
@@ -1931,4 +1986,25 @@
     return GG_OK;
 }
 
-}
+int walk_resume(gg_ctx *ctx) {
+    WalkCont *c = (WalkCont *)ctx->walk_cont;
+    GG_CHECK(ctx, c != nullptr, GG_EINVAL, "walk: no begun launch to resume");
+    WalkArgs a = c->a;
+    int rc;
+    if (c->nch == 1) rc = run_levels_and_finish<1>(ctx, a, c->total_walks, c);
+    else if (c->nch == 2) rc = run_levels_and_finish<2>(ctx, a, c->total_walks, c);
+    else if (c->nch == 4) rc = run_levels_and_finish<4>(ctx, a, c->total_walks, c);
+    else rc = run_levels_and_finish<8>(ctx, a, c->total_walks, c);
+    if (rc != GG_OK) return rc;
+    if (ctx->walk_timed) GG_HIP(ctx, hipEventRecord(ctx->ev1, ctx->walk_stream));
+    GG_HIP(ctx, hipGetLastError());
+    return GG_OK;
+}
+
+void walk_cont_release(gg_ctx *ctx) {
+    delete (WalkCont *)ctx->walk_cont;
+    ctx->walk_cont = nullptr;
+    ctx->walk_cont_pending = false;
+}
+
+}
```

New measurement: 639.7 million. 0.963x the previous value.
